# churchill-lab/gbrs

Hardware: AMD Instinct MI355X
Metric: EM iterations/s (EMASE Model 4, 40M reads x 8 haplotypes x 120k isoforms per GPU) (higher is better)
Workload: dtype f64

## Files before the change

### gbrs_amd/_lib.py

```python
from __future__ import annotations

import ctypes as C
import os

_HERE = os.path.dirname(os.path.abspath(__file__))
LIB_PATH = os.environ.get("GBRS_TUNING_LIB") or os.path.join(_HERE, "libgbrs_hip.so")

EXPORTS = [
    "gbrs_last_error", "gbrs_abi_version", "gbrs_device_count", "gbrs_warm_up",
    "gbrs_em_create", "gbrs_em_create_device", "gbrs_em_create_masked", "gbrs_em_create_masked_device", "gbrs_em_set_initial_values", "gbrs_em_prepare", "gbrs_em_step", "gbrs_em_run",
    "gbrs_em_set_groups", "gbrs_em_step_model", "gbrs_em_posterior",
    "gbrs_em_resample", "gbrs_em_weights", "gbrs_em_resample_info",
    "gbrs_em_bootstrap_begin", "gbrs_em_bootstrap_add", "gbrs_em_bootstrap_get",
    "gbrs_em_get", "gbrs_em_set_theta", "gbrs_em_group_sums", "gbrs_em_estep_partial",
    "gbrs_em_finish_step", "gbrs_em_prepare_partial", "gbrs_em_finish_prepare", "gbrs_em_stream",
    "gbrs_em_set_stream",
    "gbrs_em_sync", "gbrs_em_pair_begin", "gbrs_em_pair_check", "gbrs_em_pair_status", "gbrs_em_info", "gbrs_em_fold_counts", "gbrs_em_tile_cut", "gbrs_em_tile_shapes",
    "gbrs_alignment_counts",
    "gbrs_counts_create", "gbrs_counts_get", "gbrs_counts_destroy", "gbrs_em_destroy",
    "gbrs_shard_plan", "gbrs_shard_index", "gbrs_shard_gather",
    "gbrs_hmm_create", "gbrs_hmm_set_expression", "gbrs_hmm_set_eprob", "gbrs_hmm_run",
    "gbrs_hmm_get", "gbrs_hmm_info", "gbrs_hmm_destroy",
    "gbrs_grid_knots", "gbrs_hmm_set_grid", "gbrs_hmm_grid", "gbrs_hmm_grid_info", "gbrs_hmm_sample_paths", "gbrs_hmm_sample_info",
    "gbrs_hmm_diagnostics", "gbrs_hmm_pair_posterior", "gbrs_hmm_diagnostics_info",
    "gbrs_hmm_set_panel", "gbrs_hmm_match", "gbrs_hmm_match_info",
    "gbrs_hmm_set_snps", "gbrs_hmm_impute", "gbrs_hmm_impute_info", "gbrs_hmm_impute_times",
    "gbrs_hmm_loglik", "gbrs_hmm_loglik_tables", "gbrs_hmm_loglik_info", "gbrs_interpolate", "gbrs_genoprob_dosage",
    "gbrs_ri_transition_tables", "gbrs_alignment_spec",
    "gbrs_scan_create", "gbrs_scan_destroy", "gbrs_scan_append", "gbrs_scan_append_hmm", "gbrs_scan_prepare", "gbrs_scan_run",
    "gbrs_scan_info", "gbrs_scan_permute", "gbrs_scan_perm_info",
    "gbrs_scan_set_snps", "gbrs_scan_snp_dosage", "gbrs_scan_snps", "gbrs_scan_snp_info",
    "gbrs_compress_create", "gbrs_compress_get", "gbrs_compress_destroy",
    "gbrs_bam_open", "gbrs_bam_references", "gbrs_bam_set_reference_map", "gbrs_bam_convert", "gbrs_bam_get",
    "gbrs_bam_scan_records", "gbrs_bam_destroy",
    "gbrs_ecset_create", "gbrs_ecset_add_bam", "gbrs_ecset_add_bam_pair", "gbrs_ecset_sizes", "gbrs_ecset_get", "gbrs_ecset_destroy",
    "gbrs_matops_create", "gbrs_matops_intersect", "gbrs_matops_append_rows", "gbrs_matops_keep_unique_rows",
    "gbrs_matops_mask_columns", "gbrs_matops_sizes", "gbrs_matops_get", "gbrs_matops_destroy",
    "gbrs_matops_shared_counts", "gbrs_matops_shared_counts_get", "gbrs_matops_shared_counts_info",
    "gbrs_tensor_create", "gbrs_tensor_set_groups", "gbrs_tensor_reset", "gbrs_tensor_multiply",
    "gbrs_tensor_multiply_tensor", "gbrs_tensor_normalize", "gbrs_tensor_sum_reads", "gbrs_tensor_sum_loci",
    "gbrs_tensor_copy", "gbrs_tensor_values", "gbrs_tensor_set_values", "gbrs_tensor_nnz", "gbrs_tensor_destroy",
    "gbrs_format_double", "gbrs_write_locus_table", "gbrs_parse_length_table", "gbrs_parse_genotype_table",
    "gbrs_decode_chunks", "gbrs_inflate_backend", "gbrs_zip_directory", "gbrs_npz_stack", "gbrs_zip_read_members", "gbrs_parse_number_table",
]

GBRS_OK = 0
GBRS_ERR_INVALID = -1
GBRS_ERR_HIP = -2
GBRS_ERR_NO_DEVICE = -3
GBRS_ERR_FLOAT = -4
GBRS_ERR_UNSUPPORTED = -5
GBRS_ERR_STATE = -6

GBRS_EM_DEFAULT = 0
GBRS_EM_MERGE_IDENTICAL_ROWS = 1
GBRS_EM_LAYOUT_CSC = 2
GBRS_EM_NO_INTERLEAVE = 4
GBRS_EM_FORCE_INTERLEAVE = 8
GBRS_EM_NO_STREAMS = 16
GBRS_EM_DETERMINISTIC = 32
GBRS_EM_KEEP_CSC = 64
GBRS_EM_SIDE_BY_SIDE = 128
GBRS_EM_ONE_SHOT = 256
GBRS_EM_NO_LOCUS_SETS = 512
GBRS_EM_GROUPED_MODELS = 1024
GBRS_EM_POSTERIOR = 2048
GBRS_EM_RESAMPLE = 4096
GBRS_EM_NO_RUN_WORDS = 8192
GBRS_RESAMPLE_BASE = 0xFFFFFFFF


class EmInfo(C.Structure):
    _fields_ = [
        ("num_rows", C.c_uint64), ("num_entries", C.c_uint64), ("num_device_rows", C.c_uint64),
        ("num_device_words", C.c_uint64), ("bytes_per_iter", C.c_uint64),
        ("algorithmic_bytes", C.c_uint64), ("last_estep_ms", C.c_double),
        ("last_step_ms", C.c_double), ("num_loci", C.c_uint32), ("num_haps", C.c_uint32),
        ("layout", C.c_uint32), ("num_folded_rows", C.c_uint32),
        ("num_tiles", C.c_uint64), ("num_slots", C.c_uint64), ("num_long_rows", C.c_uint64),
        ("num_heavy_loci", C.c_uint64), ("num_light_loci", C.c_uint64), ("estep_bytes", C.c_uint64),
        ("retained_build_bytes", C.c_uint64),
        ("num_locus_sets", C.c_uint64),
    ]


class HmmInfo(C.Structure):
    _fields_ = [
        ("total_genes", C.c_uint64), ("algorithmic_bytes", C.c_uint64),
        ("last_emission_ms", C.c_double), ("last_forward_ms", C.c_double),
        ("last_backward_ms", C.c_double), ("last_backtrace_ms", C.c_double),
        ("num_states", C.c_int32), ("n_samples", C.c_int32),
        ("last_run_ms", C.c_double),
        ("last_delta_blocks", C.c_int32), ("last_delta_longest_fixup", C.c_int32),
        ("last_delta_fallbacks", C.c_int32), ("last_delta_tie_fallbacks", C.c_int32),
    ]


class ScanInfo(C.Structure):
    _fields_ = [
        ("n", C.c_int64), ("M", C.c_int64), ("H", C.c_int32), ("c", C.c_int32),
        ("last_prepare_ms", C.c_double), ("last_run_ms", C.c_double), ("last_product_ms", C.c_double),
        ("device_bytes", C.c_uint64),
    ]


class ScanPermInfo(C.Structure):
    _fields_ = [
        ("P", C.c_int64), ("B", C.c_int64), ("last_permute_ms", C.c_double), ("last_product_ms", C.c_double),
        ("peak_device_bytes", C.c_uint64),
    ]


class ScanSnpInfo(C.Structure):
    _fields_ = [
        ("M_snp", C.c_int64), ("chunk", C.c_int64), ("P", C.c_int64), ("last_pass_ms", C.c_double),
        ("last_row_ms", C.c_double), ("last_product_ms", C.c_double), ("device_bytes", C.c_uint64),
        ("peak_device_bytes", C.c_uint64), ("staged", C.c_int32), ("reserved", C.c_int32),
    ]


class GbrsHipError(RuntimeError):
    def __init__(self, status, message):
        super().__init__(message)
        self.status = status


_lib = None


def load():
    global _lib
    if _lib is not None:
        return _lib
    if not os.path.exists(LIB_PATH):
        raise ImportError(
            f"{LIB_PATH} is missing: the HIP library has not been built "
            "(run `python -c 'import __graft_entry__ as g; g.build()'`). "
            "gbrs_amd has no CPU fallback.")
    lib = C.CDLL(LIB_PATH)
    vp, i32, u32, u64, i64, dbl = C.c_void_p, C.c_int, C.c_uint32, C.c_uint64, C.c_int64, C.c_double
    pp = C.POINTER(C.c_void_p)
    lib.gbrs_last_error.restype = C.c_char_p
    lib.gbrs_last_error.argtypes = []
    lib.gbrs_abi_version.restype = i32
    lib.gbrs_device_count.restype = i32
    lib.gbrs_warm_up.restype = i32
    lib.gbrs_warm_up.argtypes = [i32]
    sigs = {
        "gbrs_em_create": [u64, u32, u32, pp, pp, vp, vp, i32, u32, pp],
        "gbrs_em_create_device": [u64, u32, u32, pp, pp, vp, vp, i32, u32, pp],
        "gbrs_em_create_masked": [u64, u32, u32, pp, pp, vp, vp, vp, i32, u32, pp],
        "gbrs_em_create_masked_device": [u64, u32, u32, pp, pp, vp, vp, vp, i32, u32, pp],
        "gbrs_em_set_initial_values": [vp, pp],
        "gbrs_em_prepare": [vp, dbl],
        "gbrs_em_step": [vp, i32, C.POINTER(dbl)],
        "gbrs_em_run": [vp, i32, dbl, i32, C.POINTER(i32), vp, i32, vp],
        "gbrs_em_set_groups": [vp, i64, vp, vp],
        "gbrs_em_step_model": [vp, i32, i32, C.POINTER(dbl)],
        "gbrs_em_posterior": [vp, u32, vp, u64],
        "gbrs_em_resample": [vp, u64, u32],
        "gbrs_em_weights": [vp, vp],
        "gbrs_em_resample_info": [vp, C.POINTER(u64), C.POINTER(u64), C.POINTER(u32)],
        "gbrs_em_bootstrap_begin": [vp, i64, vp, vp],
        "gbrs_em_bootstrap_add": [vp, vp, vp, vp, vp],
        "gbrs_em_bootstrap_get": [vp, i32, C.POINTER(u32), vp, vp, vp, vp, vp, vp, vp, vp],
        "gbrs_em_get": [vp, vp, vp],
        "gbrs_em_set_theta": [vp, vp],
        "gbrs_em_group_sums": [vp, i64, vp, vp, i32, vp],
        "gbrs_em_estep_partial": [vp, pp, C.POINTER(u64)],
        "gbrs_em_finish_step": [vp, C.POINTER(dbl)],
        "gbrs_em_prepare_partial": [vp, pp, C.POINTER(u64)],
        "gbrs_em_finish_prepare": [vp, dbl],
        "gbrs_em_sync": [vp],
        "gbrs_em_pair_begin": [vp, vp, i32],
        "gbrs_em_pair_check": [vp, vp, dbl],
        "gbrs_em_pair_status": [vp, vp, C.POINTER(i32), C.POINTER(i32), vp, i32],
        "gbrs_em_set_stream": [vp, vp],
        "gbrs_em_info": [vp, C.POINTER(EmInfo)],
        "gbrs_em_fold_counts": [vp, C.POINTER(u64), C.POINTER(u64)],
        "gbrs_em_tile_cut": [vp, C.POINTER(u32), C.POINTER(u32)],
        "gbrs_em_tile_shapes": [vp, vp, vp, u64],
        "gbrs_alignment_counts": [u64, u32, u32, pp, pp, vp, vp, u32, i32, vp, vp, vp],
        "gbrs_counts_create": [u64, u32, u32, pp, pp, vp, i32, pp],
        "gbrs_counts_get": [vp, vp, u32, vp, vp, vp],
        "gbrs_counts_destroy": [vp],
        "gbrs_em_destroy": [vp],
        "gbrs_shard_plan": [u64, u32, u32, pp, pp, i32, i32, vp],
        "gbrs_shard_index": [u64, u32, u32, pp, pp, u64, u64, i32, pp, vp],
        "gbrs_shard_gather": [u64, u32, u32, pp, pp, u64, u64, u32, pp, i32, vp, pp, pp, C.POINTER(u64)],
        "gbrs_hmm_create": [i32, i32, vp, vp, pp, i32, pp],
        "gbrs_hmm_set_expression": [vp, i32, pp, pp, pp, dbl, dbl],
        "gbrs_hmm_set_eprob": [vp, i32, pp],
        "gbrs_hmm_run": [vp],
        "gbrs_hmm_get": [vp, i32, i32, vp, vp, vp, vp, vp, vp, vp, vp],
        "gbrs_hmm_info": [vp, C.POINTER(HmmInfo)],
        "gbrs_hmm_destroy": [vp],
        "gbrs_grid_knots": [i32, vp, i32, vp, vp, vp],
        "gbrs_hmm_set_grid": [vp, vp, pp, vp, pp],
        "gbrs_hmm_grid": [vp, i32, vp, vp],
        "gbrs_hmm_grid_info": [vp, C.POINTER(i64), C.POINTER(dbl)],
        "gbrs_hmm_set_panel": [vp, i32, pp],
        "gbrs_hmm_match": [vp, i32, vp, vp],
        "gbrs_hmm_match_info": [vp, C.POINTER(i32), vp, C.POINTER(dbl), C.POINTER(u64)],
        "gbrs_hmm_set_snps": [vp, vp, pp, vp, pp, pp],
        "gbrs_hmm_impute": [vp, i32, i64, i64, vp],
        "gbrs_hmm_impute_info": [vp, C.POINTER(i64), C.POINTER(dbl), C.POINTER(u64)],
        "gbrs_hmm_impute_times": [vp, C.POINTER(dbl), C.POINTER(dbl), C.POINTER(dbl)],
        "gbrs_hmm_sample_paths": [vp, i32, i32, u64, vp, vp, vp, C.POINTER(u64)],
        "gbrs_hmm_sample_info": [vp, C.POINTER(dbl), C.POINTER(u64)],
        "gbrs_hmm_diagnostics": [vp, i32, vp, vp, vp, vp, vp],
        "gbrs_hmm_pair_posterior": [vp, i32, i32, vp],
        "gbrs_hmm_diagnostics_info": [vp, C.POINTER(dbl)],
        "gbrs_hmm_loglik": [vp, i32, vp],
        "gbrs_hmm_loglik_tables": [vp, i32, i32, vp, pp, i32, vp],
        "gbrs_hmm_loglik_info": [vp, C.POINTER(dbl), C.POINTER(u64)],
        "gbrs_interpolate": [i32, i32, vp, vp, i32, vp, vp, i32],
        "gbrs_genoprob_dosage": [i32, i64, vp, vp, i32],
        "gbrs_ri_transition_tables": [vp, vp, vp, i64, dbl, dbl, i32, vp],
        "gbrs_alignment_spec": [vp, vp, vp, i64, i32, dbl, i32, vp, vp, vp, vp],
        "gbrs_scan_create": [i32, i32, vp, i32, pp],
        "gbrs_scan_destroy": [vp],
        "gbrs_scan_append": [vp, i32, vp],
        "gbrs_scan_append_hmm": [vp, vp, i32],
        "gbrs_scan_prepare": [vp, i32, vp],
        "gbrs_scan_run": [vp, i64, vp, vp, vp, vp],
        "gbrs_scan_info": [vp, C.POINTER(ScanInfo), vp],
        "gbrs_scan_permute": [vp, i64, vp, i64, u64, vp, vp, vp],
        "gbrs_scan_perm_info": [vp, C.POINTER(ScanPermInfo)],
        "gbrs_scan_set_snps": [vp, pp, vp, pp, pp],
        "gbrs_scan_snp_dosage": [vp, i64, i64, vp],
        "gbrs_scan_snps": [vp, i64, vp, vp, vp, vp, vp],
        "gbrs_scan_snp_info": [vp, C.POINTER(ScanSnpInfo)],
        "gbrs_compress_create": [u64, u32, u32, pp, pp, vp, i32, pp, C.POINTER(u64), vp],
        "gbrs_compress_get": [vp, pp, pp, vp],
        "gbrs_compress_destroy": [vp],
        "gbrs_bam_convert": [vp, i32, C.POINTER(u64), C.POINTER(u32), vp, vp],
        "gbrs_bam_get": [vp, pp, pp, vp],
        "gbrs_ecset_create": [u32, u32, i32, C.POINTER(vp)],
        "gbrs_ecset_add_bam": [vp, vp, C.POINTER(u64), vp],
        "gbrs_ecset_add_bam_pair": [vp, vp, vp, C.POINTER(u64), vp],
        "gbrs_ecset_sizes": [vp, C.POINTER(u64), C.POINTER(u64), vp],
        "gbrs_ecset_get": [vp, pp, pp, vp],
        "gbrs_ecset_destroy": [vp],
        "gbrs_matops_create": [u64, u32, u32, pp, pp, i32, pp],
        "gbrs_matops_intersect": [vp, pp, pp],
        "gbrs_matops_append_rows": [vp, u64, pp, pp],
        "gbrs_matops_keep_unique_rows": [vp, vp, u32, i32, vp],
        "gbrs_matops_mask_columns": [vp, vp],
        "gbrs_matops_sizes": [vp, C.POINTER(u64), vp, C.POINTER(u32)],
        "gbrs_matops_get": [vp, pp, pp],
        "gbrs_matops_destroy": [vp],
        "gbrs_matops_shared_counts": [vp, vp, u32, C.POINTER(u64)],
        "gbrs_matops_shared_counts_get": [vp, vp, vp, vp],
        "gbrs_matops_shared_counts_info": [vp, C.POINTER(u64), C.POINTER(u64), C.POINTER(u64), C.POINTER(u32),
                                           C.POINTER(u64), C.POINTER(u64), C.POINTER(dbl)],
        "gbrs_tensor_create": [u64, u32, u32, pp, pp, pp, vp, i32, pp],
        "gbrs_tensor_set_groups": [vp, i64, vp, vp],
        "gbrs_tensor_reset": [vp],
        "gbrs_tensor_multiply": [vp, i32, vp, u64],
        "gbrs_tensor_multiply_tensor": [vp, vp],
        "gbrs_tensor_normalize": [vp, i32],
        "gbrs_tensor_sum_reads": [vp, vp],
        "gbrs_tensor_sum_loci": [vp, vp],
        "gbrs_tensor_copy": [vp, pp],
        "gbrs_tensor_values": [vp, u32, vp, vp, u64],
        "gbrs_tensor_set_values": [vp, u32, vp, u64],
        "gbrs_tensor_nnz": [vp, vp],
        "gbrs_tensor_destroy": [vp],
    }
    sigs.update(_host_signatures())
    for name, args in sigs.items():
        if name in ("gbrs_em_fold_counts", "gbrs_em_tile_cut", "gbrs_em_tile_shapes") and os.environ.get("GBRS_TUNING_LIB") and not hasattr(lib, name):
            continue
        fn = getattr(lib, name)
        fn.restype = i32
        fn.argtypes = args
    lib.gbrs_em_stream.restype = vp
    lib.gbrs_em_stream.argtypes = [vp]
    if lib.gbrs_abi_version() != 5:
        raise ImportError("libgbrs_hip.so ABI version mismatch")
    _lib = lib
    return lib


def _host_signatures():
    vp, i32, u32, u64, i64, dbl = C.c_void_p, C.c_int, C.c_uint32, C.c_uint64, C.c_int64, C.c_double
    return {
        "gbrs_format_double": [dbl, C.c_char_p],
        "gbrs_decode_chunks": [C.c_char_p, i64, vp, vp, vp, vp, u64, u32, u64, i32, i32, vp, i32],
        "gbrs_inflate_backend": [],
        "gbrs_zip_directory": [vp, u64, u64, vp, vp, vp, vp, vp, vp, u64, C.POINTER(u64), C.POINTER(u64)],
        "gbrs_npz_stack": [vp, u64, i64, vp, vp, vp, vp, vp, vp, u64, u64, vp, vp, i32],
        "gbrs_zip_read_members": [vp, u64, i64, vp, vp, vp, vp, vp, vp, i32],
        "gbrs_parse_number_table": [C.c_char_p, i64, i64, i32, vp],
        "gbrs_parse_length_table": [C.c_char_p, i64, C.c_char_p, vp, i64, C.c_char_p, vp, i32, dbl, vp],
        "gbrs_parse_genotype_table": [C.c_char_p, i64, C.c_char_p, vp, i64, C.c_char_p, vp, i32, vp, vp, i32, vp,
                                      C.POINTER(i64)],
        "gbrs_bam_open": [C.c_char_p, i32, C.POINTER(vp), C.POINTER(u64), C.POINTER(u64)],
        "gbrs_bam_references": [vp, vp, u64, vp, vp],
        "gbrs_bam_set_reference_map": [vp, u64, vp, vp, u32, u32],
        "gbrs_bam_scan_records": [vp, u64, vp, vp, vp, vp, u64, C.POINTER(u64), C.POINTER(u64)],
        "gbrs_bam_destroy": [vp],
        "gbrs_write_locus_table": [C.c_char_p, C.c_char_p, vp, i64, i32, i64, i64, vp, C.c_char_p, vp, C.c_char_p, vp, vp],
    }


def check(status):
    if status == GBRS_OK:
        return
    msg = load().gbrs_last_error().decode(errors="replace")
    if status == GBRS_ERR_FLOAT:
        raise FloatingPointError(msg)
    raise GbrsHipError(status, msg)


def ptr(a):
    if a is None:
        return None
    return a.ctypes.data_as(C.c_void_p)


def ptr_table(arrays):
    tab = (C.c_void_p * len(arrays))()
    for i, a in enumerate(arrays):
        tab[i] = None if a is None else a.ctypes.data
    return tab


def raw_table(addresses):
    tab = (C.c_void_p * len(addresses))()
    for i, a in enumerate(addresses):
        tab[i] = a
    return tab


def warm_up_device_async(device=0):
    import threading

    def _go():
        try:
            load().gbrs_warm_up(int(device))
        except Exception:
            pass
    t = threading.Thread(target=_go, name='gbrs-hip-init', daemon=True)
    t.start()
    return t
```

### gbrs_amd/csrc/em.hip

```cpp
#include "common.h"
#include "em_layout.h"
#include "em_step.h"

#include <algorithm>
#include <chrono>
#include <cmath>
#include <cstdlib>

namespace gbrs {


struct EmScalars {
    double s_prev, s_new;
    double err_sum;
    double pc_before, pc_after;
    int stop;
    int iters_done;
    int float_error;
    int ticket;
};

constexpr int RED_BLOCKS = 256;
constexpr int RED_THREADS = 256;

// ... 382 lines not shown
    else v = t * (fac[k] / (count ? count[r] : 1.0));
    out[k - k0] = v;
}

#include "em_tiles.inc"
#include "em_models.inc"
#include "em_resample.inc"

}

using namespace gbrs;


struct gbrs_em {
    int device = 0;
    hipStream_t stream = nullptr;
    bool own_stream = true;
    uint64_t R = 0, N = 0;
    uint32_t L = 0, H = 0;
    bool has_count = false, has_len = false, prepared = false;
    uint32_t flags = 0;

    int layout = 0;
    EmPlan plan;
    bool acc_external = false;
    TileLayout tl;

    DevBuf<uint32_t> ent_row;
    DevBuf<uint64_t> col_ptr;
    DevBuf<uint64_t> col_ptr_src;
    bool masked = false;
    DevBuf<double> den;

    DevBuf<double> count, eff_len;
    DevBuf<double> acc_init;
    bool has_init = false, keep_csc = false;
    bool stopped = false;
    DevBuf<double> theta, acc, counts;
    bool counts_stale = false;
    DevBuf<double> tot_prev, tot_new;
    DevBuf<double> partials;
    DevBuf<double> msums;
    uint32_t msum_cap = 0, msum_blocks = 0;
    DevBuf<double> scratch_hl;
    DevBuf<double> err_hist;
    DevBuf<EmScalars> scalars;
    int err_hist_cap = 0;
    double last_estep_ms = 0.0, last_step_ms = 0.0;
    bool time_steps = true;
    bool err_pending = false;
    double err_pending_target = -1.0;
    std::vector<hipEvent_t> ev_pool;

    struct PairScalars { int iters, stop; double err; };
    DevBuf<PairScalars> pair_sc;
    DevBuf<double> pair_hist;
    int pair_hist_cap = 0;
    hipEvent_t pair_ev_mstep = nullptr;
    hipEvent_t pair_ev_err = nullptr;

    bool grouped = false;
    uint32_t n_genes = 0;
    DevBuf<uint32_t> gene_ptr, gene_mem, locus_gene, row_ptr;
    DevBuf<uint32_t> rank_m1, inv_m1, rank_m23, inv_m23;
    GroupedOrder order_m1, order_m23;
    DevBuf<double> gene_tot, gene_hap_tot, locus_tot, fac;

    DevBuf<double> theta_kept, post_den, post_vals;
    int post_model = 0;
    bool post_den_valid = false;

    bool resample = false, has_base = false;
    DevBuf<uint32_t> base_count, big_rows;
    uint32_t n_big = 0;
    struct Stats {
        bool active = false;
        uint32_t n = 0;
        int64_t G = 0;
        DevBuf<int64_t> gptr, gmem;
        DevBuf<double> theta_sum;
        DevBuf<double> cur[2][2], mean[2][2], m2[2][2], tot_mean[2][2], tot_m2[2][2];
    } stats;

    int red_blocks() const { return (int)std::min<uint64_t>(RED_BLOCKS, (L + RED_THREADS - 1) / RED_THREADS); }
};

struct gbrs_counts {
    int device = 0;
    uint64_t R = 0, n = 0;
    uint32_t L = 0, H = 0;
    gbrs::DevBuf<uint32_t> ent_row;
    gbrs::DevBuf<uint64_t> col_ptr;
    gbrs::DevBuf<double> d_count;
    hipStream_t s = nullptr;
    gbrs::CountsWork *work = nullptr;
};

namespace {

ErrArgs em_err_args(gbrs_em *em, double target_err) {
    ErrArgs ea;
    ea.L = em->L;
    ea.nblocks = (int)em->msum_blocks;
    ea.cap = em->msum_cap;
    ea.tot_prev = em->tot_prev.p;
    ea.tot_new = em->tot_new.p;
    ea.partials = em->msums.p;
    ea.sc = em->scalars.p;
    ea.target_err = target_err;
    ea.err_hist = em->err_hist.p;
    ea.err_hist_cap = em->err_hist_cap;
    ea.n_err_blocks = (uint32_t)std::min<uint64_t>(ERR_BLOCKS, (em->L + RED_THREADS - 1) / RED_THREADS);
    return ea;
}

int em_launch_err(gbrs_em *em, double target_err) {
    const ErrArgs ea = em_err_args(em, target_err);
    hipLaunchKernelGGL(err_finish_kernel, dim3(ea.n_err_blocks), dim3(RED_THREADS), 0, em->stream, ea);
    GBRS_HIP_CHECK(hipGetLastError());
    return GBRS_OK;
}

int em_flush_err(gbrs_em *em) {
    if (!em->err_pending) return GBRS_OK;
    em->err_pending = false;
    return em_launch_err(em, em->err_pending_target);
}

int em_check_float(gbrs_em *em, EmScalars &host) {
    GBRS_TRY(em_flush_err(em));
    GBRS_HIP_CHECK(hipMemcpyAsync(&host, em->scalars.p, sizeof(EmScalars), hipMemcpyDeviceToHost, em->stream));
    GBRS_HIP_CHECK(hipStreamSynchronize(em->stream));
    em->stopped = host.stop != 0;
    if (host.float_error && !em->plan.no_float_check)
        return fail(GBRS_ERR_FLOAT, "invalid value encountered in divide (a read's alignments all have zero abundance)");
    return GBRS_OK;
}


EmStepRoute em_route(const gbrs_em *em, EmPass pass) {
    const TileLayout &tl = em->tl;
    EmStepShape s;
    s.tiled = em->layout == 1;
    s.H = em->H; s.tH = em->plan.tH; s.view = em->plan.view;
    s.no_tiles = tl.n_tiles == 0; s.no_long = tl.n_long == 0; s.no_entries = em->N == 0;
    s.weighted = tl.weighted; s.deterministic = tl.deterministic; s.all_one_word = tl.all_one_word;
    s.persist_groups = em->plan.persist_groups;
    s.acc_handed_out = em->acc_external;
    s.no_fused_mstep = em->plan.no_fused_mstep;
    return em_step_route(s, pass);
}

template <int HT, bool ONES>
int em_launch_tiles_h(gbrs_em *em, const EmStepRoute &r) {
    const TileLayout &tl = em->tl;
    const uint32_t tH = em->plan.tH;
    ErrArgs ea = em_err_args(em, em->err_pending_target);
    if (!r.err_rides || !em->err_pending) ea.n_err_blocks = 0;
    em->err_pending = false;
    const dim3 grid((unsigned)tl.n_tiles + ea.n_err_blocks), block(TILE_THREADS);
    const double *ww = tl.weighted ? tl.word_weight.p : (const double *)nullptr;
    const SetArgs sets{em->plan.tL, tl.n_sets ? tl.set_ptr.p : nullptr, tl.set_members.p, tl.dest_list.p, tl.dict_b.p, tl.dest_b.p,
                       em->resample ? 1u : 0u};
    const uint32_t lead_mask = em->plan.lead_mask;
#define GBRS_LAUNCH_TILES(W, D)                                                                                            \
    hipLaunchKernelGGL((tile_estep_kernel<HT, W, ONES, D>), grid, block, 0, em->stream, tH, tl.tiles.p, tl.words.p,        \
                       tl.dict.p, ww, em->theta.p, tl.partials.p, tl.slot_dest.p, em->acc.p, em->scalars.p,               \
                       (uint32_t)tl.n_tiles, ea, sets, lead_mask)
    switch (r.estep) {
        case EmEstep::Persistent:
        case EmEstep::PersistentOneWord: {
            const uint32_t G = std::min<uint32_t>(em->plan.persist_groups, (uint32_t)tl.n_tiles);
            const dim3 pgrid(G + ea.n_err_blocks);
#define GBRS_LAUNCH_PERSISTENT(HH, W, OW)                                                                                  \
            hipLaunchKernelGGL((tile_estep_persistent_kernel<HH, W, OW>), pgrid, block, 0, em->stream, tH, tl.tiles.p,     \
                               tl.words.p, tl.dict.p, ww, em->theta.p, tl.partials.p, tl.slot_dest.p,                      \
                               (int64_t)(em->acc.p - tl.partials.p), em->scalars.p, (uint32_t)tl.n_tiles, G, ea, sets)
            if (r.estep == EmEstep::PersistentOneWord) GBRS_LAUNCH_PERSISTENT(HT == 8 ? 8 : 1, false, HT == 8);
            else if (r.weighted) GBRS_LAUNCH_PERSISTENT(HT, true, false);
            else GBRS_LAUNCH_PERSISTENT(HT, false, false);
#undef GBRS_LAUNCH_PERSISTENT
            break;
        }
        case EmEstep::TilesDeterministic:
            if (r.weighted) GBRS_LAUNCH_TILES(true, true); else GBRS_LAUNCH_TILES(false, true);
            break;
#if !defined(GBRS_NO_ONEWORD)
        case EmEstep::TilesOneWord:
            hipLaunchKernelGGL((tile_estep_kernel<HT == 8 ? 8 : 1, false, ONES, false, HT == 8>), grid, block, 0, em->stream, tH,
                               tl.tiles.p, tl.words.p, tl.dict.p, ww, em->theta.p, tl.partials.p, tl.slot_dest.p, em->acc.p,
                               em->scalars.p, (uint32_t)tl.n_tiles, ea, sets, lead_mask);
            break;
#endif
        default:
            if (r.weighted) GBRS_LAUNCH_TILES(true, false); else GBRS_LAUNCH_TILES(false, false);
    }
#undef GBRS_LAUNCH_TILES
    return GBRS_OK;
}
int em_launch_tiles(gbrs_em *em, const EmStepRoute &r) {
#define GBRS_TILES_OF(HT) (r.pass == EmPass::Prepare ? em_launch_tiles_h<HT, true>(em, r) : em_launch_tiles_h<HT, false>(em, r))
    switch (r.width) {
        case 1: return GBRS_TILES_OF(1);
        case 2: return GBRS_TILES_OF(2);
        case 4: return GBRS_TILES_OF(4);
        case 8: return GBRS_TILES_OF(8);
        case 16: return GBRS_TILES_OF(16);
        default: return GBRS_TILES_OF(0);
    }
#undef GBRS_TILES_OF
}

int em_launch_long_rows(gbrs_em *em, const EmStepRoute &r) {
    const TileLayout &tl = em->tl;
    const bool ones = r.pass == EmPass::Prepare;
    GBRS_HIP_CHECK(hipMemsetAsync(tl.acc_extra.p, 0, tl.acc_extra.bytes(), em->stream));
#define GBRS_LAUNCH_LONG(KERNEL, GRID, BLOCK)                                                                              \
    hipLaunchKernelGGL(KERNEL, GRID, BLOCK, 0, em->stream, tl.n_long, em->plan.tH, tl.long_ptr.p, tl.long_loc.p,          \
                       tl.long_mask.p, tl.long_weight.p, em->theta.p, tl.acc_extra.p, em->scalars.p, em->resample ? 1u : 0u)
    const dim3 grid((unsigned)((tl.n_long + 3) / 4));
    if (r.long_rows == EmLongRows::Serial) {
        if (ones) GBRS_LAUNCH_LONG(long_rows_estep_serial_kernel<true>, dim3(1), dim3(64));
        else GBRS_LAUNCH_LONG(long_rows_estep_serial_kernel<false>, dim3(1), dim3(64));
    } else {
        if (ones) GBRS_LAUNCH_LONG(long_rows_estep_kernel<true>, grid, dim3(256));
        else GBRS_LAUNCH_LONG(long_rows_estep_kernel<false>, grid, dim3(256));
    }
#undef GBRS_LAUNCH_LONG
    return GBRS_OK;
}

int em_launch_gather(gbrs_em *em, const EmStepRoute &r) {
    const TileLayout &tl = em->tl;
    const uint32_t gH = em->plan.tH, gL = em->plan.tL;
    uint32_t HP = 1;
    while (HP < gH) HP <<= 1;
    const bool all = r.gather == EmGather::All;
    const uint64_t elems = all ? (uint64_t)gL * gH : (uint64_t)tl.n_light * gH;
    const unsigned light = (unsigned)((elems + 255) / 256);
    const unsigned heavy = (unsigned)((tl.n_heavy + 3) / 4);
    if (light + heavy > 0)
        hipLaunchKernelGGL(gather_kernel, dim3(light + heavy), dim3(256), 0, em->stream, gL, gH,
                           HP, light, heavy, (uint32_t)tl.n_heavy, all ? 1 : 0, (uint32_t)tl.n_light, tl.light_loci.p,
                           tl.slot_ptr.p, tl.heavy_loci.p, tl.locus_class.p, tl.partials.p,
                           (tl.n_long && all) ? tl.acc_extra.p : (const double *)nullptr, em->acc.p, em->scalars.p,
                           r.pass == EmPass::Prepare ? 0 : 1);
    return GBRS_OK;
}

template <bool ONES>
int em_launch_csc(gbrs_em *em, const EmStepRoute &r) {
    const uint64_t n = em->N;
    const uint32_t ncols = em->H * em->L;
    GBRS_HIP_CHECK(hipMemsetAsync(em->acc.p, 0, em->acc.bytes(), em->stream));
    if (r.estep != EmEstep::Csc) return GBRS_OK;
    GBRS_HIP_CHECK(hipMemsetAsync(em->den.p, 0, em->den.bytes(), em->stream));
    const unsigned grid = (unsigned)((n + 255) / 256);
    hipLaunchKernelGGL(csc_den_kernel<ONES>, dim3(grid), dim3(256), 0, em->stream, n, ncols, em->L,
                       em->H, em->col_ptr.p, em->ent_row.p, em->theta.p, em->den.p, em->scalars.p);
    hipLaunchKernelGGL(csc_acc_kernel<ONES>, dim3(grid), dim3(256), 0, em->stream, n, ncols, em->L,
                       em->H, em->col_ptr.p, em->ent_row.p, em->has_count ? em->count.p : nullptr,
                       em->den.p, em->acc.p, em->scalars.p, em->resample ? 1u : 0u);
    return GBRS_OK;
}

int em_launch_models(gbrs_em *em, int model) {
    const GroupedOrder &o = model == 1 ? em->order_m1 : em->order_m23;
    const uint32_t nt = std::max(em->L, em->n_genes);
    hipLaunchKernelGGL(model_totals_kernel, dim3((nt + 255) / 256), dim3(256), 0, em->stream, em->L, em->H, em->n_genes,
                       em->gene_ptr.p, em->gene_mem.p, em->theta.p, em->gene_tot.p, em->gene_hap_tot.p, em->locus_tot.p,
                       em->scalars.p);
    GBRS_HIP_CHECK(hipMemsetAsync(em->acc.p, 0, em->acc.bytes(), em->stream));
    if (em->N) {
        const dim3 rgrid((unsigned)((em->R + 255) / 256));
        const double *cnt = em->has_count ? em->count.p : (const double *)nullptr;
#define GBRS_LAUNCH_ROWS(M)                                                                                             \
        hipLaunchKernelGGL(model_row_kernel<M>, rgrid, dim3(256), 0, em->stream, em->R, em->H, em->row_ptr.p, o.lh.p,   \
                           o.src.p, em->locus_gene.p, em->theta.p, em->gene_tot.p, em->gene_hap_tot.p, em->locus_tot.p, \
                           cnt, em->fac.p, em->scalars.p)
        if (model == 1) GBRS_LAUNCH_ROWS(1);
        else if (model == 2) GBRS_LAUNCH_ROWS(2);
        else GBRS_LAUNCH_ROWS(3);
#undef GBRS_LAUNCH_ROWS
        hipLaunchKernelGGL(model_col_kernel, dim3((unsigned)((em->N + 255) / 256)), dim3(256), 0, em->stream, em->N,
                           em->H * em->L, em->L, em->H, em->col_ptr.p, em->fac.p, em->acc.p, em->scalars.p);
    }
    GBRS_HIP_CHECK(hipGetLastError());
    return GBRS_OK;
}

int em_estep(gbrs_em *em, const EmStepRoute &r, int model = 4, hipEvent_t after_kernels = nullptr) {
    if (!r.err_rides) GBRS_TRY(em_flush_err(em));
    if (r.estep == EmEstep::Models) GBRS_TRY(em_launch_models(em, model));
    else if (em->layout != 1) GBRS_TRY(r.pass == EmPass::Prepare ? em_launch_csc<true>(em, r) : em_launch_csc<false>(em, r));
    else if (r.estep != EmEstep::None) GBRS_TRY(em_launch_tiles(em, r));
    if (r.long_rows != EmLongRows::None) GBRS_TRY(em_launch_long_rows(em, r));
    if (after_kernels) GBRS_HIP_CHECK(hipEventRecord(after_kernels, em->stream));
    if (r.gather != EmGather::None) GBRS_TRY(em_launch_gather(em, r));
    GBRS_HIP_CHECK(hipGetLastError());
    return GBRS_OK;
}

template <int H, bool EXTRA, bool LEN>
void em_launch_mstep_gather_h(gbrs_em *em) {
    const TileLayout &tl = em->tl;
    const uint64_t npair = (uint64_t)em->L * MstepRow<H>::LANES, per = (uint64_t)RED_THREADS * MSTEP_EPT;
    const unsigned elem_blocks = (unsigned)((npair + per - 1) / per);
    const unsigned heavy_blocks = (unsigned)tl.n_heavy;
    const unsigned light_blocks = (unsigned)((tl.n_light * MstepRow<H>::LANES + RED_THREADS - 1) / RED_THREADS);
    em->msum_blocks = elem_blocks + heavy_blocks + light_blocks;
    hipLaunchKernelGGL((mstep_gather_kernel<H, EXTRA, LEN>), dim3(em->msum_blocks), dim3(RED_THREADS), 0, em->stream, em->L,
                       heavy_blocks, light_blocks, (uint32_t)tl.n_light, tl.heavy_range.p, tl.light_range.p,
                       tl.locus_class.p, tl.partials.p, em->acc.p, EXTRA ? tl.acc_extra.p : (const double *)nullptr,
                       em->theta.p, LEN ? em->eff_len.p : (const double *)nullptr, em->tot_prev.p, em->tot_new.p,
                       em->msums.p, em->msum_cap, em->scalars.p);
}
template <int H>
void em_launch_mstep_gather_opts(gbrs_em *em, bool extra) {
    if (extra) em->has_len ? em_launch_mstep_gather_h<H, true, true>(em) : em_launch_mstep_gather_h<H, true, false>(em);
    else em->has_len ? em_launch_mstep_gather_h<H, false, true>(em) : em_launch_mstep_gather_h<H, false, false>(em);
}
int em_launch_mstep_gather(gbrs_em *em, const EmStepRoute &r) {
    const bool extra = r.long_rows != EmLongRows::None;
    switch (em->H) {
    case 1: em_launch_mstep_gather_opts<1>(em, extra); break;
    case 2: em_launch_mstep_gather_opts<2>(em, extra); break;
    case 4: em_launch_mstep_gather_opts<4>(em, extra); break;
    case 8: em_launch_mstep_gather_opts<8>(em, extra); break;
    case 16: em_launch_mstep_gather_opts<16>(em, extra); break;
    default: return fail(GBRS_ERR_UNSUPPORTED, "the fused M-step has no instance for this haplotype count");
    }
    return GBRS_OK;
}

template <int MODE, int H>
void em_launch_mstep_elem(gbrs_em *em, const double *extra, const double *len) {
    const uint64_t npair = (uint64_t)em->L * MstepRow<H>::LANES;
    const unsigned nb = (unsigned)((npair + RED_THREADS - 1) / RED_THREADS);
    em->msum_blocks = nb;
    hipLaunchKernelGGL((mstep_elem_kernel<MODE, H>), dim3(nb), dim3(RED_THREADS), 0, em->stream, em->L, em->theta.p, em->acc.p,
                       extra, len, em->counts.p, em->tot_prev.p, em->tot_new.p, em->msums.p, em->msum_cap, em->scalars.p);
}
template <int MODE>
int em_launch_mstep_plain(gbrs_em *em, const EmStepRoute &r) {
    const double *len = em->has_len ? em->eff_len.p : nullptr;
    if (r.mstep == EmMstep::PerLocus) {
        const int nb = em->red_blocks();
        em->msum_blocks = nb;
        hipLaunchKernelGGL(mstep_kernel<MODE>, dim3(nb), dim3(RED_THREADS), 0, em->stream, em->L, em->H,
                           em->theta.p, em->acc.p, len, em->counts.p, em->tot_prev.p, em->tot_new.p,
                           em->msums.p, em->msum_cap, em->scalars.p);
        return GBRS_OK;
    }
    const double *extra = r.mstep_adds_extra ? em->tl.acc_extra.p : (const double *)nullptr;
    switch (em->H) {
    case 1: em_launch_mstep_elem<MODE, 1>(em, extra, len); break;
    case 2: em_launch_mstep_elem<MODE, 2>(em, extra, len); break;
    case 4: em_launch_mstep_elem<MODE, 4>(em, extra, len); break;
    case 8: em_launch_mstep_elem<MODE, 8>(em, extra, len); break;
    case 16: em_launch_mstep_elem<MODE, 16>(em, extra, len); break;
    case 32: em_launch_mstep_elem<MODE, 32>(em, extra, len); break;
    default: return fail(GBRS_ERR_UNSUPPORTED, "the element-parallel M-step has no instance for this haplotype count");
    }
    return GBRS_OK;
}
int em_launch_mstep(gbrs_em *em, const EmStepRoute &r) {
    if (r.mstep == EmMstep::Fused) return em_launch_mstep_gather(em, r);
    return r.pass == EmPass::Prepare ? em_launch_mstep_plain<1>(em, r) : em_launch_mstep_plain<0>(em, r);
}

__global__ void __launch_bounds__(256)
counts_from_theta_kernel(uint64_t n, const double *__restrict__ theta, const double *__restrict__ eff_len, double *__restrict__ counts) {
    const uint64_t i = (uint64_t)blockIdx.x * blockDim.x + threadIdx.x;
    if (i < n) counts[i] = eff_len ? theta[i] * eff_len[i] : theta[i];
}
int em_refresh_counts(gbrs_em *em) {
    if (!em->counts_stale) return GBRS_OK;
    const uint64_t n = (uint64_t)em->L * em->H;
    hipLaunchKernelGGL(counts_from_theta_kernel, dim3((unsigned)((n + 255) / 256)), dim3(256), 0, em->stream, n, em->theta.p,
                       em->has_len ? em->eff_len.p : (const double *)nullptr, em->counts.p);
    GBRS_HIP_CHECK(hipGetLastError());
    em->counts_stale = false;
    return GBRS_OK;
}

int em_finish_step(gbrs_em *em, const EmStepRoute &r, double target_err, bool defer_err) {
    GBRS_TRY(em_flush_err(em));
    GBRS_TRY(em_launch_mstep(em, r));
    em->counts_stale = r.counts_stale;
    if (defer_err && r.err_defer) {
        em->err_pending = true;
        em->err_pending_target = target_err;
        return GBRS_OK;
    }
    return em_launch_err(em, target_err);
}

int em_keep_theta(gbrs_em *em, int model) {
    if (!(em->flags & GBRS_EM_POSTERIOR)) return GBRS_OK;
    GBRS_TRY(em_flush_err(em));
    const uint64_t n = (uint64_t)em->L * em->H;
    hipLaunchKernelGGL(keep_theta_kernel, dim3((unsigned)((n + 255) / 256)), dim3(256), 0, em->stream, n, em->theta.p,
                       em->theta_kept.p, em->scalars.p);
    GBRS_HIP_CHECK(hipGetLastError());
    em->post_model = model;
    em->post_den_valid = false;
    return GBRS_OK;
}

constexpr int EM_TIME_STRIDE = 8, EM_TIME_SAMPLES = 16;
int em_one_step(gbrs_em *em, const EmStepRoute &r, int model, double target_err, hipEvent_t *ev, bool defer_err) {
    GBRS_TRY(em_keep_theta(em, model));
    if (!em->time_steps) ev = nullptr;
    if (ev) GBRS_HIP_CHECK(hipEventRecord(ev[0], em->stream));
    GBRS_TRY(em_estep(em, r, model, ev ? ev[1] : nullptr));
    GBRS_TRY(em_finish_step(em, r, target_err, defer_err));
    if (r.pass == EmPass::Model && em->layout == 1) GBRS_HIP_CHECK(hipMemsetAsync(em->acc.p, 0, em->acc.bytes(), em->stream));
    if (ev) GBRS_HIP_CHECK(hipEventRecord(ev[2], em->stream));
    return GBRS_OK;
}

void em_read_times(gbrs_em *em, int n) {
    if (!em->time_steps || n <= 0) return;
    double se = 0.0, ss = 0.0;
    for (int i = 0; i < n; ++i) {
        float a = 0.f, b = 0.f;
        if (hipEventElapsedTime(&a, em->ev_pool[3 * i], em->ev_pool[3 * i + 1]) != hipSuccess) return;
        if (hipEventElapsedTime(&b, em->ev_pool[3 * i], em->ev_pool[3 * i + 2]) != hipSuccess) return;
        se += a;
        ss += b;
    }
    em->last_estep_ms = se / n;
    em->last_step_ms = ss / n;
}

int em_finish_prepare(gbrs_em *em, double pseudocount) {
    GBRS_TRY(em_launch_mstep(em, em_route(em, EmPass::Prepare)));
    em->counts_stale = false;
    const int nb = em->red_blocks();
    if (pseudocount > 0.0) {
        hipLaunchKernelGGL(pseudo_add_kernel, dim3(nb), dim3(RED_THREADS), 0, em->stream, em->L,
                           em->H, pseudocount, em->theta.p, em->partials.p);
        hipLaunchKernelGGL(pseudo_scale_kernel, dim3(nb), dim3(RED_THREADS), 0, em->stream,
                           (uint64_t)em->L * em->H, nb, em->theta.p, em->partials.p, em->scalars.p);
    }
    GBRS_HIP_CHECK(hipMemsetAsync(em->partials.p, 0, em->partials.bytes(), em->stream));
    GBRS_HIP_CHECK(hipMemsetAsync(em->acc.p, 0, em->acc.bytes(), em->stream));
    GBRS_HIP_CHECK(hipGetLastError());
    em->prepared = true;
    return GBRS_OK;
}

int em_reset_scalars(gbrs_em *em, bool keep_iters) {
    GBRS_TRY(em_flush_err(em));
    EmScalars host;
    std::memset(&host, 0, sizeof(host));
    if (keep_iters) {
        EmScalars cur;
        GBRS_HIP_CHECK(hipMemcpyAsync(&cur, em->scalars.p, sizeof(cur), hipMemcpyDeviceToHost, em->stream));
        GBRS_HIP_CHECK(hipStreamSynchronize(em->stream));
        host.iters_done = cur.iters_done;
    }
    em->stopped = false;
    GBRS_HIP_CHECK(hipMemcpyAsync(em->scalars.p, &host, sizeof(host), hipMemcpyHostToDevice, em->stream));
    GBRS_HIP_CHECK(hipStreamSynchronize(em->stream));
    return GBRS_OK;
}

int em_ensure_hist(gbrs_em *em, int cap) {
    if (cap <= em->err_hist_cap) return GBRS_OK;
    GBRS_HIP_CHECK(hipStreamSynchronize(em->stream));
    GBRS_TRY(em->err_hist.alloc((size_t)cap));
    em->err_hist_cap = cap;
    return GBRS_OK;
}

int em_check_model(const gbrs_em *em, int model) {
    if (model < 1 || model > 4) return fail(GBRS_ERR_INVALID, "The read normalization model should be 1, 2, 3, or 4.");
    if (model == 4) return GBRS_OK;
    if (em->flags & GBRS_EM_DETERMINISTIC)
        return fail(GBRS_ERR_UNSUPPORTED, "multiread model %d has no bit-reproducible form (GBRS_EM_DETERMINISTIC)", model);
    if (!em->grouped)
        return fail(GBRS_ERR_UNSUPPORTED, "multiread model %d needs gene groups: create the handle with "
                                          "GBRS_EM_GROUPED_MODELS and call gbrs_em_set_groups", model);
    return GBRS_OK;
}

int em_ensure_order(gbrs_em *em, int model) {
    GroupedOrder &o = model == 1 ? em->order_m1 : em->order_m23;
    if (o.built) return GBRS_OK;
    GBRS_TRY(em_flush_err(em));
    return build_grouped_order(o, em->R, em->L, em->H, em->N, em->ent_row.p, em->col_ptr.p,
                               model == 1 ? em->rank_m1.p : em->rank_m23.p, model == 1 ? em->inv_m1.p : em->inv_m23.p,
                               em->stream);
}

int upload_csc(uint64_t R, uint32_t L, uint32_t H, const uint32_t *const *indptr,
               const uint32_t *const *indices, bool on_device, DevBuf<uint32_t> &ent_row,
               DevBuf<uint64_t> &col_ptr_dev, uint64_t &n_out, const uint32_t *allowed = nullptr,
               DevBuf<uint64_t> *src_ptr_dev = nullptr, hipStream_t stream = nullptr) {
    const hipMemcpyKind kind = on_device ? hipMemcpyDeviceToDevice : hipMemcpyHostToDevice;
    std::vector<uint64_t> col_ptr((size_t)H * L + 1), src_ptr;
    if (allowed) src_ptr.resize((size_t)H * L + 1);
    std::vector<uint32_t> tmp(L + 1);
    uint64_t n = 0, n_src = 0;
    std::vector<uint64_t> hap_off(H + 1);
    for (uint32_t h = 0; h < H; ++h) {
        if (!indptr[h]) return fail(GBRS_ERR_INVALID, "indptr[%u] is NULL", h);
        if (on_device) {
            GBRS_HIP_CHECK(hipMemcpy(tmp.data(), indptr[h], (L + 1) * sizeof(uint32_t), hipMemcpyDeviceToHost));
        } else {
            std::memcpy(tmp.data(), indptr[h], (L + 1) * sizeof(uint32_t));
        }
        if (tmp[0] != 0) return fail(GBRS_ERR_INVALID, "indptr[%u][0] != 0", h);
        hap_off[h] = n_src;
        for (uint32_t l = 0; l < L; ++l) {
            if (tmp[l + 1] < tmp[l]) return fail(GBRS_ERR_INVALID, "indptr[%u] is not non-decreasing at %u", h, l);
            col_ptr[(size_t)h * L + l] = n;
            if (allowed) {
                src_ptr[(size_t)h * L + l] = n_src + tmp[l];
                if ((allowed[l] >> h) & 1u) n += tmp[l + 1] - tmp[l];
            } else {
                n += tmp[l + 1] - tmp[l];
            }
        }
        n_src += tmp[L];
    }
    hap_off[H] = n_src;
    col_ptr[(size_t)H * L] = n;
    GBRS_TRY(col_ptr_dev.alloc(col_ptr.size()));
    GBRS_HIP_CHECK(hipMemcpy(col_ptr_dev.p, col_ptr.data(), col_ptr_dev.bytes(), hipMemcpyHostToDevice));
    GBRS_TRY(ent_row.alloc(std::max<uint64_t>(n, 1)));
// ... 333 lines not shown
        int hbad = 0;
        GBRS_HIP_CHECK(hipMemcpyAsync(&hbad, bad.p, sizeof(int), hipMemcpyDeviceToHost, em->stream));
        GBRS_HIP_CHECK(hipStreamSynchronize(em->stream));
        GBRS_HIP_CHECK(hipGetLastError());
        if (hbad) {
            em->acc_init.release();
            return fail(GBRS_ERR_FLOAT, "invalid value encountered in divide (a read's stored alignment values are "
                                        "negative or add up to zero)");
        }
    }
    em->has_init = true;
    if (em->layout == 1 && em->keep_csc) {
        if (!(em->flags & (GBRS_EM_GROUPED_MODELS | GBRS_EM_POSTERIOR))) em->ent_row.release();
        em->den.release();
        em->col_ptr_src.release();
        em->keep_csc = false;
    }
    return GBRS_OK;
}

int gbrs_em_prepare_partial(gbrs_em_t *em, void **partial_dev, uint64_t *n_elems) {
    if (!em) return fail(GBRS_ERR_INVALID, "handle is NULL");
    em->acc_external = true;
    GBRS_TRY(em_prepare_partial(em));
    if (partial_dev) *partial_dev = em->acc.p;
    if (n_elems) *n_elems = (uint64_t)em->L * em->H;
    return GBRS_OK;
}

int gbrs_em_finish_prepare(gbrs_em_t *em, double pseudocount) {
    if (!em) return fail(GBRS_ERR_INVALID, "handle is NULL");
    GBRS_TRY(select_device(em->device));
    GBRS_TRY(em_finish_prepare(em, pseudocount));
    EmScalars host;
    return em_check_float(em, host);
}

int gbrs_em_prepare(gbrs_em_t *em, double pseudocount) {
    RoctxRange roctx_range("gbrs_em_prepare");
    if (!em) return fail(GBRS_ERR_INVALID, "handle is NULL");
    GBRS_TRY(em_prepare_partial(em));
    return gbrs_em_finish_prepare(em, pseudocount);
}

int gbrs_em_estep_partial(gbrs_em_t *em, void **partial_dev, uint64_t *n_elems) {
    if (!em) return fail(GBRS_ERR_INVALID, "handle is NULL");
    if (!em->prepared) return fail(GBRS_ERR_STATE, "prepare() has not been called");
    GBRS_TRY(select_device(em->device));
    if (em->stopped) GBRS_TRY(em_reset_scalars(em, true));
    em->acc_external = true;
    GBRS_TRY(em_estep(em, em_route(em, EmPass::Partial)));
    if (partial_dev) *partial_dev = em->acc.p;
    if (n_elems) *n_elems = (uint64_t)em->L * em->H;
    return GBRS_OK;
}

int gbrs_em_finish_step(gbrs_em_t *em, double *err_sum_out) {
    if (!em) return fail(GBRS_ERR_INVALID, "handle is NULL");
    GBRS_TRY(select_device(em->device));
    GBRS_TRY(em_finish_step(em, em_route(em, EmPass::Partial), -1.0,  err_sum_out == nullptr));
    if (em->pair_ev_mstep) GBRS_HIP_CHECK(hipEventRecord(em->pair_ev_mstep, em->stream));
    if (err_sum_out) {
        EmScalars host;
        GBRS_TRY(em_check_float(em, host));
        *err_sum_out = host.err_sum;
    }
    return GBRS_OK;
}

int gbrs_em_step(gbrs_em_t *em, int n_iters, double *err_sum_out) {
    RoctxRange roctx_range("gbrs_em_step");
    if (!em) return fail(GBRS_ERR_INVALID, "handle is NULL");
    if (!em->prepared) return fail(GBRS_ERR_STATE, "prepare() has not been called");
    GBRS_TRY(select_device(em->device));
    if (em->stopped) GBRS_TRY(em_reset_scalars(em, true));
    const int stride = std::max(EM_TIME_STRIDE, (n_iters + EM_TIME_SAMPLES - 1) / EM_TIME_SAMPLES);
    const int timed = em->time_steps ? (n_iters + stride - 1) / stride : 0;
    while ((int)em->ev_pool.size() < 3 * timed) {
        hipEvent_t e;
        GBRS_HIP_CHECK(hipEventCreate(&e));
        em->ev_pool.push_back(e);
    }
    const EmStepRoute route = em_route(em, EmPass::Step);
    for (int i = 0; i < n_iters; ++i) {
        const int slot = i / stride;
        const bool t = i % stride == 0 && slot < timed;
        GBRS_TRY(em_one_step(em, route, 4, -1.0, t ? &em->ev_pool[3 * slot] : nullptr, i + 1 < n_iters));
    }
    EmScalars host;
    GBRS_TRY(em_check_float(em, host));
    em_read_times(em, timed);
    if (err_sum_out) *err_sum_out = host.err_sum;
    return GBRS_OK;
}

int gbrs_em_step_model(gbrs_em_t *em, int model, int n_iters, double *err_sum_out) {
    RoctxRange roctx_range("gbrs_em_step_model");
    if (!em) return fail(GBRS_ERR_INVALID, "handle is NULL");
    GBRS_TRY(em_check_model(em, model));
    if (model == 4) return gbrs_em_step(em, n_iters, err_sum_out);
    if (!em->prepared) return fail(GBRS_ERR_STATE, "prepare() has not been called");
    GBRS_TRY(select_device(em->device));
    if (em->stopped) GBRS_TRY(em_reset_scalars(em, true));
    GBRS_TRY(em_ensure_order(em, model));
    const EmStepRoute route = em_route(em, EmPass::Model);
    for (int i = 0; i < n_iters; ++i) GBRS_TRY(em_one_step(em, route, model, -1.0, i == 0 ? em->ev_pool.data() : nullptr, false));
    EmScalars host;
    GBRS_TRY(em_check_float(em, host));
    em_read_times(em, n_iters > 0 ? 1 : 0);
    if (err_sum_out) *err_sum_out = host.err_sum;
    return GBRS_OK;
}

int gbrs_em_set_groups(gbrs_em_t *em, int64_t G, const int64_t *group_ptr, const int64_t *members) {
    RoctxRange roctx_range("gbrs_em_set_groups");
    if (!em || G < 0 || (G > 0 && (!group_ptr || !members))) return fail(GBRS_ERR_INVALID, "bad argument");
    if (!(em->flags & GBRS_EM_GROUPED_MODELS))
        return fail(GBRS_ERR_STATE, "the handle was not created with GBRS_EM_GROUPED_MODELS");
    if (em->N && !em->ent_row.p) return fail(GBRS_ERR_STATE, "the handle no longer holds the CSC row ids");
    const uint32_t L = em->L, H = em->H;
    if (em->N >= 0xFFFFFFFFull || L >= (1u << 27))
        return fail(GBRS_ERR_UNSUPPORTED, "the grouped layout holds at most 2^32 - 1 entries of at most 2^27 loci");
    if (G > 0 && group_ptr[0] != 0) return fail(GBRS_ERR_INVALID, "group_ptr[0] != 0");
    for (int64_t g = 0; g < G; ++g)
        if (group_ptr[g + 1] < group_ptr[g]) return fail(GBRS_ERR_INVALID, "group_ptr not monotone");
    GBRS_TRY(select_device(em->device));
    std::vector<int64_t> gene(L, -1);
    std::vector<std::vector<uint32_t>> mem((size_t)G);
    for (int64_t g = 0; g < G; ++g)
        for (int64_t k = group_ptr[g]; k < group_ptr[g + 1]; ++k) {
            const int64_t l = members[k];
            if (l < 0 || l >= (int64_t)L) return fail(GBRS_ERR_INVALID, "group member %lld out of range", (long long)l);
            if (gene[l] == g) continue;
            if (gene[l] >= 0)
                return fail(GBRS_ERR_INVALID, "locus %lld is in two groups (%lld and %lld)", (long long)l,
                            (long long)gene[l], (long long)g);
            gene[l] = g;
            mem[g].push_back((uint32_t)l);
        }
    std::vector<uint32_t> gptr{0}, gmem, lgene(L), pos(L);
    gmem.reserve(L);
    for (int64_t g = 0; g < G; ++g) {
        std::sort(mem[g].begin(), mem[g].end());
        for (uint32_t l : mem[g]) { lgene[l] = (uint32_t)(gptr.size() - 1); pos[l] = (uint32_t)gmem.size(); gmem.push_back(l); }
        gptr.push_back((uint32_t)gmem.size());
    }
    for (uint32_t l = 0; l < L; ++l)
        if (gene[l] < 0) { lgene[l] = (uint32_t)(gptr.size() - 1); pos[l] = (uint32_t)gmem.size(); gmem.push_back(l); gptr.push_back((uint32_t)gmem.size()); }
    const uint32_t n_genes = (uint32_t)(gptr.size() - 1);
    const size_t HL = (size_t)H * L;
    std::vector<uint32_t> r23(HL), i23(HL), r1(HL), i1(HL);
    for (uint32_t l = 0; l < L; ++l) {
        const uint32_t g = lgene[l], start = gptr[g], size = gptr[g + 1] - start;
        for (uint32_t h = 0; h < H; ++h) {
            const uint32_t a = pos[l] * H + h, b = start * H + h * size + (pos[l] - start);
            r23[(size_t)h * L + l] = a;
            i23[a] = l * 32u + h;
            r1[(size_t)h * L + l] = b;
            i1[b] = l * 32u + h;
        }
    }
    em->grouped = false;
    em->order_m1.built = em->order_m23.built = false;
    auto up = [&](DevBuf<uint32_t> &d, const std::vector<uint32_t> &v) -> int {
        GBRS_TRY(d.alloc(std::max<size_t>(v.size(), 1)));
        if (!v.empty()) GBRS_HIP_CHECK(hipMemcpyAsync(d.p, v.data(), v.size() * 4, hipMemcpyHostToDevice, em->stream));
        return GBRS_OK;
    };
    GBRS_TRY(up(em->gene_ptr, gptr));
    GBRS_TRY(up(em->gene_mem, gmem));
    GBRS_TRY(up(em->locus_gene, lgene));
    GBRS_TRY(up(em->rank_m23, r23));
    GBRS_TRY(up(em->inv_m23, i23));
    GBRS_TRY(up(em->rank_m1, r1));
    GBRS_TRY(up(em->inv_m1, i1));
    GBRS_TRY(em->gene_tot.alloc(n_genes));
    GBRS_TRY(em->gene_hap_tot.alloc((size_t)n_genes * H));
    GBRS_TRY(em->locus_tot.alloc(L));
    GBRS_TRY(em->fac.alloc(std::max<uint64_t>(em->N, 1)));
    GBRS_HIP_CHECK(hipStreamSynchronize(em->stream));
    em->n_genes = n_genes;
    GBRS_TRY(build_row_ptr(em->row_ptr, em->R, em->N, em->ent_row.p, em->stream));
    GBRS_TRY(build_grouped_order(em->order_m23, em->R, L, H, em->N, em->ent_row.p, em->col_ptr.p, em->rank_m23.p,
                                 em->inv_m23.p, em->stream));
    em->grouped = true;
    return GBRS_OK;
}

int gbrs_em_run(gbrs_em_t *em, int model, double tol, int max_iters, int *n_iters_out,
                double *err_hist, int err_hist_cap, double *elapsed_s) {
    RoctxRange roctx_range("gbrs_em_run");
    if (!em) return fail(GBRS_ERR_INVALID, "handle is NULL");
    GBRS_TRY(em_check_model(em, model));
    if (!em->prepared) return fail(GBRS_ERR_STATE, "prepare() has not been called");
    GBRS_TRY(select_device(em->device));
    if (model != 4) GBRS_TRY(em_ensure_order(em, model));
    if (max_iters < 0) max_iters = 0;
    GBRS_TRY(em_ensure_hist(em, std::max(max_iters, 1)));
    GBRS_TRY(em_reset_scalars(em, false));
    const double target = 1000000.0 * tol;
    const EmStepRoute route = em_route(em, model == 4 ? EmPass::Step : EmPass::Model);
    int done = 0;
    EmScalars host;
    std::memset(&host, 0, sizeof(host));
    if (1000000.0 > target) {
        const int batch = 8;
        bool first = true;
        const auto t_start = std::chrono::steady_clock::now();
        while (done < max_iters) {
            const int nb = std::min(batch, max_iters - done);
            for (int i = 0; i < nb; ++i) {
                GBRS_TRY(em_one_step(em, route, model, target, first ? em->ev_pool.data() : nullptr, i + 1 < nb));
                first = false;
            }
            GBRS_TRY(em_check_float(em, host));
            if (elapsed_s) {
                const double t = std::chrono::duration<double>(std::chrono::steady_clock::now() - t_start).count();
                for (int i = done; i < host.iters_done && i < err_hist_cap; ++i) elapsed_s[i] = t;
            }
            done = host.iters_done;
            if (host.stop) break;
        }
    }
    em_read_times(em, 1);
    if (n_iters_out) *n_iters_out = done;
    if (err_hist && err_hist_cap > 0 && done > 0) {
        const int ncopy = std::min(done, err_hist_cap);
        GBRS_HIP_CHECK(hipMemcpy(err_hist, em->err_hist.p, ncopy * sizeof(double), hipMemcpyDeviceToHost));
    }
    return GBRS_OK;
}

int gbrs_em_get(gbrs_em_t *em, double *theta, double *expected_counts) {
    if (!em) return fail(GBRS_ERR_INVALID, "handle is NULL");
    GBRS_TRY(select_device(em->device));
    const size_t LH = (size_t)em->L * em->H;
    for (int which = 0; which < 2; ++which) {
        double *dst = which == 0 ? theta : expected_counts;
        if (!dst) continue;
        if (which == 1) GBRS_TRY(em_refresh_counts(em));
        hipLaunchKernelGGL(transpose_lh_to_hl, dim3(1024), dim3(256), 0, em->stream, em->L, em->H,
                           which == 0 ? em->theta.p : em->counts.p, em->scratch_hl.p);
        GBRS_HIP_CHECK(hipMemcpyAsync(dst, em->scratch_hl.p, LH * sizeof(double), hipMemcpyDeviceToHost, em->stream));
        GBRS_HIP_CHECK(hipStreamSynchronize(em->stream));
    }
    return GBRS_OK;
}

int gbrs_em_posterior(gbrs_em_t *em, uint32_t hap, double *out, uint64_t out_len) {
    RoctxRange roctx_range("gbrs_em_posterior");
    if (!em) return fail(GBRS_ERR_INVALID, "handle is NULL");
    if (!(em->flags & GBRS_EM_POSTERIOR))
        return fail(GBRS_ERR_STATE, "the handle was not created with GBRS_EM_POSTERIOR");
    if (em->post_model == 0) return fail(GBRS_ERR_STATE, "no EM step has run since prepare: there is no posterior yet");
    if (hap >= em->H) return fail(GBRS_ERR_INVALID, "haplotype %u >= num_haps %u", hap, em->H);
    GBRS_TRY(select_device(em->device));
    GBRS_TRY(em_flush_err(em));
    const uint32_t L = em->L, H = em->H, ncols = H * L;
    uint64_t k0 = 0, k1 = 0;
    GBRS_HIP_CHECK(hipMemcpyAsync(&k0, em->col_ptr.p + (size_t)hap * L, sizeof(k0), hipMemcpyDeviceToHost, em->stream));
    GBRS_HIP_CHECK(hipMemcpyAsync(&k1, em->col_ptr.p + (size_t)(hap + 1) * L, sizeof(k1), hipMemcpyDeviceToHost, em->stream));
    GBRS_HIP_CHECK(hipStreamSynchronize(em->stream));
    if (k1 < k0 || k1 > em->N) return fail(GBRS_ERR_STATE, "the kept column pointers are damaged");
    const uint64_t n_h = k1 - k0;
    if (out_len != n_h)
        return fail(GBRS_ERR_INVALID, "out_len is %llu, haplotype %u has %llu stored entries", (unsigned long long)out_len,
                    hap, (unsigned long long)n_h);
    if (n_h == 0) return GBRS_OK;
    if (!out) return fail(GBRS_ERR_INVALID, "out is NULL");
    if (!em->ent_row.p) return fail(GBRS_ERR_STATE, "the handle no longer holds the CSC row ids");
    const bool model4 = em->post_model == 4;
    if (!model4 && !em->fac.p) return fail(GBRS_ERR_STATE, "the handle holds no factors of a model %d step", em->post_model);
    if (model4 && !em->post_den_valid) {
        GBRS_HIP_CHECK(hipMemsetAsync(em->post_den.p, 0, em->post_den.bytes(), em->stream));
        hipLaunchKernelGGL(post_den_kernel, dim3((unsigned)((em->N + 255) / 256)), dim3(256), 0, em->stream, em->N, ncols,
                           L, H, em->col_ptr.p, em->ent_row.p, em->theta_kept.p, em->post_den.p);
        GBRS_HIP_CHECK(hipGetLastError());
        em->post_den_valid = true;
    }
    if (em->post_vals.n < n_h) {
        std::vector<uint64_t> cp((size_t)ncols + 1);
        GBRS_HIP_CHECK(hipMemcpy(cp.data(), em->col_ptr.p, cp.size() * 8, hipMemcpyDeviceToHost));
        uint64_t longest = 0;
        for (uint32_t h = 0; h < H; ++h) longest = std::max(longest, cp[(size_t)(h + 1) * L] - cp[(size_t)h * L]);
        GBRS_HIP_CHECK(hipStreamSynchronize(em->stream));
        GBRS_TRY(em->post_vals.alloc(longest));
    }
    const dim3 grid((unsigned)((n_h + 255) / 256));
    const double *cnt = em->has_count ? em->count.p : (const double *)nullptr;
    if (model4)
        hipLaunchKernelGGL(post_value_kernel<true>, grid, dim3(256), 0, em->stream, k0, k1, ncols, L, H, hap, em->col_ptr.p,
                           em->ent_row.p, em->theta_kept.p, em->post_den.p, (const double *)nullptr, cnt, em->post_vals.p);
    else
        hipLaunchKernelGGL(post_value_kernel<false>, grid, dim3(256), 0, em->stream, k0, k1, ncols, L, H, hap, em->col_ptr.p,
                           em->ent_row.p, em->theta_kept.p, (const double *)nullptr, em->fac.p, cnt, em->post_vals.p);
    GBRS_HIP_CHECK(hipGetLastError());
    GBRS_HIP_CHECK(hipMemcpyAsync(out, em->post_vals.p, n_h * sizeof(double), hipMemcpyDeviceToHost, em->stream));
    GBRS_HIP_CHECK(hipStreamSynchronize(em->stream));
    return GBRS_OK;
}

int gbrs_em_set_theta(gbrs_em_t *em, const double *theta) {
    if (!em || !theta) return fail(GBRS_ERR_INVALID, "NULL argument");
    GBRS_TRY(select_device(em->device));
    const size_t LH = (size_t)em->L * em->H;
    GBRS_TRY(em_refresh_counts(em));
    GBRS_HIP_CHECK(hipMemcpyAsync(em->scratch_hl.p, theta, LH * sizeof(double), hipMemcpyHostToDevice, em->stream));
    hipLaunchKernelGGL(transpose_hl_to_lh, dim3(1024), dim3(256), 0, em->stream, em->L, em->H,
                       em->scratch_hl.p, em->theta.p);
    GBRS_HIP_CHECK(hipStreamSynchronize(em->stream));
    em->prepared = true;
    return GBRS_OK;
}

int gbrs_em_group_sums(gbrs_em_t *em, int64_t G, const int64_t *group_ptr, const int64_t *members,
                       int which, double *out) {
    if (!em || !group_ptr || !out || G < 0) return fail(GBRS_ERR_INVALID, "bad argument");
    if (G == 0) return GBRS_OK;
    GBRS_TRY(select_device(em->device));
    const int64_t nm = group_ptr[G];
    for (int64_t g = 0; g < G; ++g)
        if (group_ptr[g + 1] < group_ptr[g]) return fail(GBRS_ERR_INVALID, "group_ptr not monotone");
    for (int64_t k = 0; k < nm; ++k)
        if (members[k] < 0 || members[k] >= (int64_t)em->L)
            return fail(GBRS_ERR_INVALID, "group member %lld out of range", (long long)members[k]);
    DevBuf<int64_t> d_ptr, d_mem;
    DevBuf<double> d_out;
    GBRS_TRY(d_ptr.alloc(G + 1));
    GBRS_TRY(d_mem.alloc(std::max<int64_t>(nm, 1)));
    GBRS_TRY(d_out.alloc((size_t)G * em->H));
    GBRS_HIP_CHECK(hipMemcpyAsync(d_ptr.p, group_ptr, (G + 1) * sizeof(int64_t), hipMemcpyHostToDevice, em->stream));
    if (nm) GBRS_HIP_CHECK(hipMemcpyAsync(d_mem.p, members, nm * sizeof(int64_t), hipMemcpyHostToDevice, em->stream));
    const int64_t total = G * (int64_t)em->H;
    if (which != 0) GBRS_TRY(em_refresh_counts(em));
    hipLaunchKernelGGL(group_sum_kernel, dim3((unsigned)((total + 255) / 256)), dim3(256), 0, em->stream,
                       em->H, G, d_ptr.p, d_mem.p, which == 0 ? em->theta.p : em->counts.p, d_out.p);
    GBRS_HIP_CHECK(hipMemcpyAsync(out, d_out.p, (size_t)G * em->H * sizeof(double), hipMemcpyDeviceToHost, em->stream));
    GBRS_HIP_CHECK(hipStreamSynchronize(em->stream));
    return GBRS_OK;
}

void *gbrs_em_stream(gbrs_em_t *em) { return em ? (void *)em->stream : nullptr; }

#if defined(GBRS_DIAG_TILE_TIMES)
int gbrs_debug_set_tile_stamps(void *device_ptr) {
    unsigned long long *p = static_cast<unsigned long long *>(device_ptr);
    GBRS_HIP_CHECK(hipMemcpyToSymbol(HIP_SYMBOL(g_tile_stamps), &p, sizeof(p)));
    return GBRS_OK;
}
#endif

int gbrs_em_set_stream(gbrs_em_t *em, void *stream) {
    if (!em) return fail(GBRS_ERR_INVALID, "handle is NULL");
    GBRS_TRY(select_device(em->device));
    GBRS_HIP_CHECK(hipStreamSynchronize(em->stream));
    if (em->own_stream && em->stream) (void)hipStreamDestroy(em->stream);
    em->stream = (hipStream_t)stream;
    em->own_stream = false;
    return GBRS_OK;
}

int gbrs_em_sync(gbrs_em_t *em) {
    if (!em) return fail(GBRS_ERR_INVALID, "handle is NULL");
    GBRS_TRY(em_flush_err(em));
    GBRS_HIP_CHECK(hipStreamSynchronize(em->stream));
    return GBRS_OK;
}

int gbrs_em_pair_begin(gbrs_em_t *a, gbrs_em_t *b, int max_iters) {
    if (!a || !b || a == b) return fail(GBRS_ERR_INVALID, "two distinct handles are needed");
    if (a->device != b->device) return fail(GBRS_ERR_INVALID, "the two handles of a pair live on one device");
    GBRS_TRY(select_device(a->device));
    for (gbrs_em *em : {a, b}) {
        GBRS_TRY(em_reset_scalars(em, false));
        if (!em->pair_ev_mstep) GBRS_HIP_CHECK(hipEventCreateWithFlags(&em->pair_ev_mstep, hipEventDisableTiming));
    }
    if (!a->pair_ev_err) GBRS_HIP_CHECK(hipEventCreateWithFlags(&a->pair_ev_err, hipEventDisableTiming));
    const int cap = std::max(max_iters, 1);
    if (!a->pair_sc.p) GBRS_TRY(a->pair_sc.alloc(1));
    if (cap > a->pair_hist_cap) {
        GBRS_TRY(a->pair_hist.alloc((size_t)cap));
        a->pair_hist_cap = cap;
    }
    GBRS_HIP_CHECK(hipMemset(a->pair_sc.p, 0, sizeof(gbrs_em::PairScalars)));
    return GBRS_OK;
}

int gbrs_em_pair_check(gbrs_em_t *a, gbrs_em_t *b, double tol) {
    if (!a || !b || !a->pair_sc.p || !a->pair_ev_err || !a->pair_ev_mstep || !b->pair_ev_mstep)
        return fail(GBRS_ERR_STATE, "gbrs_em_pair_begin has not been called on this pair");
    GBRS_TRY(select_device(a->device));
    GBRS_HIP_CHECK(hipStreamWaitEvent(b->stream, a->pair_ev_mstep, 0));
    static_assert(sizeof(PairState) == sizeof(gbrs_em::PairScalars), "one struct, two names");
    const PairSide sa{a->L, (int)a->msum_blocks, a->msum_cap, a->tot_prev.p, a->tot_new.p, a->msums.p, a->scalars.p};
    const PairSide sb{b->L, (int)b->msum_blocks, b->msum_cap, b->tot_prev.p, b->tot_new.p, b->msums.p, b->scalars.p};
    hipLaunchKernelGGL(pair_err_kernel, dim3(1), dim3(1024), 0, b->stream, sa, sb, 1000000.0 * tol,
                       reinterpret_cast<PairState *>(a->pair_sc.p), a->pair_hist.p, a->pair_hist_cap);
    GBRS_HIP_CHECK(hipGetLastError());
    GBRS_HIP_CHECK(hipEventRecord(a->pair_ev_err, b->stream));
    GBRS_HIP_CHECK(hipStreamWaitEvent(a->stream, a->pair_ev_err, 0));
    return GBRS_OK;
}

int gbrs_em_pair_status(gbrs_em_t *a, gbrs_em_t *b, int *iters_done, int *stopped, double *err_hist, int err_hist_cap) {
    if (!a || !b || !a->pair_sc.p) return fail(GBRS_ERR_STATE, "gbrs_em_pair_begin has not been called on this pair");
    GBRS_TRY(select_device(a->device));
    EmScalars ha, hb;
    GBRS_TRY(em_check_float(a, ha));
    GBRS_TRY(em_check_float(b, hb));
    gbrs_em::PairScalars ps;
    GBRS_HIP_CHECK(hipMemcpy(&ps, a->pair_sc.p, sizeof(ps), hipMemcpyDeviceToHost));
    if (iters_done) *iters_done = ps.iters;
    if (stopped) *stopped = ps.stop;
    if (err_hist && err_hist_cap > 0 && ps.iters > 0)
        GBRS_HIP_CHECK(hipMemcpy(err_hist, a->pair_hist.p, std::min(ps.iters, std::min(err_hist_cap, a->pair_hist_cap)) * sizeof(double),
                                 hipMemcpyDeviceToHost));
    return GBRS_OK;
}

int gbrs_em_info(gbrs_em_t *em, gbrs_em_info_t *info) {
    if (!em || !info) return fail(GBRS_ERR_INVALID, "NULL argument");
    std::memset(info, 0, sizeof(*info));
    const uint64_t HL = (uint64_t)em->H * em->L;
    info->num_rows = em->R;
    info->num_entries = em->N;
    info->num_device_rows = em->R;
    info->num_device_words = em->N;
    info->algorithmic_bytes = 4 * em->N + 4 * (em->R + 1) + (em->has_count ? 8 * em->R : 0) +
                              16 * HL + (em->has_len ? 8 * HL : 0);
    info->bytes_per_iter = 8 * em->N + 8 * em->R * 3 + 8 * HL * 4;
    info->estep_bytes = 8 * em->N + 8 * em->R * 3 + 8 * HL * 2;
    if (em->layout == 1) {
        const TileLayout &tl = em->tl;
        info->num_device_rows = tl.n_rows + tl.n_folded + tl.n_folded_two + tl.n_long;
        info->num_folded_rows = (uint32_t)tl.n_folded;
        info->num_tiles = tl.n_tiles;
        info->num_slots = tl.n_slots;
        info->num_long_rows = tl.n_long;
        info->num_device_words = tl.n_batches * 64;
        const uint64_t rows = tl.n_dest_rows ? tl.n_dest_rows : tl.n_slots;
        info->bytes_per_iter = 4 * tl.n_batches * 64 + 16 * tl.n_tiles + 4 * tl.n_slots +
                               8 * rows * em->plan.tH * 3 + 4 * rows + 4 * ((uint64_t)em->plan.tL + 1) +
                               (tl.weighted ? 8 * tl.n_batches * 64 : 0) + 8 * HL * 6;
        info->num_heavy_loci = tl.n_heavy;
        info->num_light_loci = tl.n_light;
        info->estep_bytes = 4 * tl.n_batches * 64 + 16 * tl.n_tiles + 4 * tl.n_slots + 4 * rows +
                            8 * rows * em->plan.tH * 2 + (tl.weighted ? 8 * tl.n_batches * 64 : 0) +
                            (tl.n_sets ? 8 * tl.n_slots : 0);
        if (tl.n_sets) info->bytes_per_iter += 8 * tl.n_slots;
    }
    info->last_estep_ms = em->last_estep_ms;
    info->last_step_ms = em->last_step_ms;
    info->num_loci = em->L;
    info->num_haps = em->H;
    info->layout = em->layout;
    info->retained_build_bytes = em->tl.retired_bytes;
    info->num_locus_sets = em->layout == 1 ? em->tl.n_sets : 0;
    return GBRS_OK;
}

int gbrs_em_fold_counts(gbrs_em_t *em, uint64_t *one_word_reads, uint64_t *two_word_reads) {
    if (!em || !one_word_reads || !two_word_reads) return fail(GBRS_ERR_INVALID, "NULL argument");
    *one_word_reads = em->layout == 1 ? em->tl.n_folded : 0;
    *two_word_reads = em->layout == 1 ? em->tl.n_folded_two : 0;
    return GBRS_OK;
}

int gbrs_em_tile_cut(gbrs_em_t *em, uint32_t *passes, uint32_t *tile_words) {
    if (!em || !passes || !tile_words) return fail(GBRS_ERR_INVALID, "NULL argument");
    *passes = em->layout == 1 ? em->tl.cut_passes : 0;
    *tile_words = em->layout == 1 ? em->tl.cut_tile_words : 0;
    return GBRS_OK;
}

int gbrs_em_tile_shapes(gbrs_em_t *em, uint32_t *n_batches, uint32_t *dict_entries, uint64_t n) {
    if (!em || !n_batches || !dict_entries) return fail(GBRS_ERR_INVALID, "NULL argument");
    if (em->layout != 1 || n != em->tl.n_tiles) return fail(GBRS_ERR_INVALID, "n is not the handle's number of tiles");
    (void)hipSetDevice(em->device);
    std::vector<TileHdr> hdr(n);
    if (n) GBRS_HIP_CHECK(hipMemcpy(hdr.data(), em->tl.tiles.p, n * sizeof(TileHdr), hipMemcpyDeviceToHost));
    for (uint64_t t = 0; t < n; ++t) {
        n_batches[t] = hdr[t].n_batches;
        dict_entries[t] = hdr[t].dict_count();
    }
    return GBRS_OK;
}

int gbrs_counts_create(uint64_t R, uint32_t L, uint32_t H, const uint32_t *const *indptr,
                       const uint32_t *const *indices, const double *count, int device, gbrs_counts_t **out) {
    if (!out) return fail(GBRS_ERR_INVALID, "out is NULL");
    *out = nullptr;
    if (H < 1 || H > 32 || L < 1 || R < 1 || R > 0xFFFFFFFFull || !indptr || !indices)
        return fail(GBRS_ERR_INVALID, "The shape must be a tuple of three positive integers (H <= 32, R < 2^32).");
    GBRS_TRY(select_device(device));
    gbrs_counts *c = new gbrs_counts();
    struct Guard { gbrs_counts *p; ~Guard() { if (p) gbrs_counts_destroy(p); } } guard{c};
    c->device = device;
    c->R = R; c->L = L; c->H = H;
    GBRS_HIP_CHECK(hipStreamCreateWithFlags(&c->s, hipStreamDefault));
    GBRS_TRY(upload_csc(R, L, H, indptr, indices, false, c->ent_row, c->col_ptr, c->n));
    if (count) {
        GBRS_TRY(c->d_count.alloc(R));
        GBRS_HIP_CHECK(hipMemcpy(c->d_count.p, count, R * sizeof(double), hipMemcpyHostToDevice));
    }
    GBRS_HIP_CHECK(hipDeviceSynchronize());
    GBRS_TRY(check_row_ids(c->n, c->ent_row.p, R, c->s));
    c->work = counts_work_new();
    guard.p = nullptr;
    *out = c;
    return GBRS_OK;
}

int gbrs_counts_get(gbrs_counts_t *c, const int32_t *locus_group, uint32_t num_out_loci, double *aln_counts,
                    double *allele_unique, double *locus_unique) {
    RoctxRange roctx_range("gbrs_counts_get");
    if (!c) return fail(GBRS_ERR_INVALID, "handle is NULL");
    const uint32_t L = c->L, H = c->H;
    const uint32_t Lout = locus_group ? num_out_loci : L;
    if (Lout < 1 || Lout >= (1u << 27)) return fail(GBRS_ERR_INVALID, "bad number of output loci");
    if (locus_group)
        for (uint32_t l = 0; l < L; ++l)
            if (locus_group[l] < -1 || (locus_group[l] >= 0 && (uint32_t)locus_group[l] >= Lout))
                return fail(GBRS_ERR_INVALID, "locus_group[%u] out of range", l);
    GBRS_TRY(select_device(c->device));
    DevBuf<double> d_aln, d_uniq, d_lu;
    DevBuf<int32_t> d_group;
    if (locus_group) {
        GBRS_TRY(d_group.alloc(L));
        GBRS_HIP_CHECK(hipMemcpy(d_group.p, locus_group, L * sizeof(int32_t), hipMemcpyHostToDevice));
    }
    GBRS_TRY(d_aln.alloc((size_t)H * Lout));
    GBRS_TRY(d_uniq.alloc((size_t)H * Lout));
    GBRS_TRY(d_lu.alloc(Lout));
    GBRS_TRY(alignment_counts_device(c->R, L, H, c->n, c->ent_row.p, c->col_ptr.p, c->d_count.p,
                                     locus_group ? d_group.p : nullptr, Lout, d_aln.p, d_uniq.p, d_lu.p, c->s, c->work));
    if (aln_counts) GBRS_HIP_CHECK(hipMemcpy(aln_counts, d_aln.p, d_aln.bytes(), hipMemcpyDeviceToHost));
    if (allele_unique) GBRS_HIP_CHECK(hipMemcpy(allele_unique, d_uniq.p, d_uniq.bytes(), hipMemcpyDeviceToHost));
    if (locus_unique) GBRS_HIP_CHECK(hipMemcpy(locus_unique, d_lu.p, d_lu.bytes(), hipMemcpyDeviceToHost));
    return GBRS_OK;
}

int gbrs_counts_destroy(gbrs_counts_t *c) {
    if (!c) return GBRS_OK;
    (void)hipSetDevice(c->device);
    if (c->s) {
        (void)hipStreamSynchronize(c->s);
        (void)hipStreamDestroy(c->s);
    }
    if (c->work) counts_work_free(c->work);
    delete c;
    return GBRS_OK;
}

int gbrs_alignment_counts(uint64_t R, uint32_t L, uint32_t H, const uint32_t *const *indptr,
// ... 182 lines not shown
```

### gbrs_amd/csrc/em_layout.h

```cpp
#pragma once
#include "common.h"
#include "em_plan.h"

#include <vector>

namespace gbrs {

#ifndef GBRS_TILE_THREADS
#define GBRS_TILE_THREADS 512
#endif
constexpr int TILE_THREADS = GBRS_TILE_THREADS;
constexpr int TILE_WAVES = TILE_THREADS / 64;
#ifndef GBRS_TILE_CAP
#define GBRS_TILE_CAP 32768
#endif
#ifndef GBRS_TILE_WORDS
#define GBRS_TILE_WORDS 2048
#endif
constexpr int TILE_WORDS = GBRS_TILE_WORDS, TILE_WORDS_MAX = GBRS_TILE_CAP - 64, TILE_ROUNDS_MIN = 1;
static_assert(TILE_WORDS <= TILE_WORDS_MAX, "a tile's padded words must fit the dictionary sort");
__host__ __device__ constexpr int pos_bits(int H) { return H <= 8 ? 5 : 3; }
__host__ __device__ constexpr int max_row_words(int H) { return 1 << pos_bits(H); }
#ifndef GBRS_LDS_DOUBLES
#define GBRS_LDS_DOUBLES 3072
#endif
#ifndef GBRS_LDS_DOUBLES_WEIGHTED
#define GBRS_LDS_DOUBLES_WEIGHTED 4608
#endif
#ifndef GBRS_LDS_DOUBLES_H16
#define GBRS_LDS_DOUBLES_H16 4800
#endif
__host__ __device__ constexpr uint32_t dict_index_limit(int H) { return 1u << (32 - H - 2 * pos_bits(H)); }
__host__ __device__ constexpr int lds_theta_doubles(bool weighted, int H) {
    return weighted ? GBRS_LDS_DOUBLES_WEIGHTED : (H == 16 ? GBRS_LDS_DOUBLES_H16 : GBRS_LDS_DOUBLES);
}
__host__ __device__ constexpr int lds_acc_doubles(bool weighted, int H) { return lds_theta_doubles(weighted, H) + 64; }
__host__ __device__ constexpr uint32_t det_dict_cap(int H, bool weighted) { return (lds_acc_doubles(weighted, H) / TILE_WAVES - 1) / H; }
constexpr uint32_t SLOT_DIRECT = 0x80000000u;
constexpr uint32_t SLOT_SET = 0x40000000u;
constexpr uint32_t SLOT_PAIR = 0x20000000u;
constexpr uint32_t DICT_PAIR = 0x80000000u, DICT_SET = 0x40000000u;
constexpr int HEAVY_SLOTS = 16;

struct TileHdr {
    uint32_t batch_base;
    uint16_t n_batches;
    uint16_t n_one;
    uint32_t dict_base;
    uint32_t dict_n_two;
    __host__ __device__ uint32_t dict_count() const { return dict_n_two & 0xFFFFu; }
    __host__ __device__ uint32_t n_two() const { return dict_n_two >> 16; }
    template <bool COUNTED> __host__ __device__ uint32_t dict_count_of() const { return COUNTED ? dict_count() : dict_n_two; }
};
static_assert(sizeof(TileHdr) == 16, "a tile header is one 16-byte scalar load");
static_assert(GBRS_LDS_DOUBLES < 65536 && GBRS_LDS_DOUBLES_WEIGHTED < 65536 && GBRS_LDS_DOUBLES_H16 < 65536,
              "TileHdr::dict_count is 16 bits");
static_assert(2 * (GBRS_TILE_CAP / 64) < 65536, "TileHdr::n_batches is 16 bits");

struct SetArgs {
    uint32_t n_loci;
    const uint32_t *set_ptr, *set_members, *dest_list;
    const uint32_t *dict_b, *dest_b;
    uint32_t relax_zero_weight;
};

struct TileLayout {
    uint64_t n_pairs = 0;
    uint64_t n_rows_in = 0;
    uint64_t n_rows = 0;
    uint64_t n_folded = 0;
    uint64_t n_folded_two = 0;
    uint64_t n_long = 0;
    uint64_t n_tiles = 0, n_batches = 0, n_slots = 0, n_heavy = 0, n_light = 0;
    uint32_t d_max = 0;
    uint32_t cut_passes = 0;
    uint32_t cut_tile_words = 0;
    bool weighted = false;
    bool deterministic = false;
    bool all_one_word = false;

    DevBuf<uint32_t> words;
    DevBuf<TileHdr> tiles;
    DevBuf<uint32_t> dict;
    DevBuf<double> word_weight;
    DevBuf<double> row_weight;
    DevBuf<uint32_t> slot_ptr;
    DevBuf<uint32_t> slot_list;
    DevBuf<uint32_t> heavy_loci;
    DevBuf<uint32_t> light_loci;
    DevBuf<uint32_t> heavy_range, light_range;
    DevBuf<uint32_t> slot_dest;
    DevBuf<uint8_t> locus_class;
    DevBuf<double> partials;
    DevBuf<uint64_t> long_ptr;
    DevBuf<uint32_t> long_loc, long_mask;
    DevBuf<double> long_weight;
    DevBuf<double> acc_extra;
    bool keep_row_ids = false;
    DevBuf<uint32_t> word_row;
    DevBuf<uint32_t> long_row;
    uint32_t n_sets = 0;
    uint64_t n_dest_rows = 0;
    DevBuf<uint32_t> set_ptr, set_members;
    DevBuf<uint32_t> dest_list;
    DevBuf<uint32_t> dict_b, dest_b;
    bool retain_temporaries = false;
    std::vector<void *> retired;
    size_t retired_bytes = 0;
    TileLayout() = default;
    TileLayout(const TileLayout &) = delete;
    TileLayout &operator=(const TileLayout &) = delete;
    ~TileLayout() {
        for (void *p : retired) (void)hipFree(p);
    }
};

inline EmDictLimits dict_limits(bool weighted, int H) {
    return {(uint32_t)max_row_words(H), dict_index_limit(H), (uint32_t)lds_theta_doubles(weighted, H), det_dict_cap(H, weighted)};
}

int build_tile_layout(TileLayout &out, uint64_t R, uint64_t N, const uint32_t *ent_row, const uint64_t *col_ptr,
                      const double *count, hipStream_t stream, const EmPlan &plan);

struct GroupedOrder {
    DevBuf<uint32_t> lh;
    DevBuf<uint32_t> src;
    bool built = false;
};
int build_row_ptr(DevBuf<uint32_t> &row_ptr, uint64_t R, uint64_t N, const uint32_t *ent_row, hipStream_t s);
int build_grouped_order(GroupedOrder &out, uint64_t R, uint32_t L, uint32_t H, uint64_t N, const uint32_t *ent_row,
                        const uint64_t *col_ptr, const uint32_t *rank, const uint32_t *rank_lh, hipStream_t s);

struct CompressResult {
    uint64_t num_ecs = 0, n_entries = 0;
    DevBuf<uint64_t> col_ptr;
    DevBuf<uint32_t> indices;
    DevBuf<double> count;
};
int compress_device(CompressResult &out, uint64_t R, uint32_t L, uint32_t H, uint64_t N, const uint32_t *ent_row,
                    const uint64_t *col_ptr, const double *count, hipStream_t s);

struct CountsWork;
CountsWork *counts_work_new();
void counts_work_free(CountsWork *w);
int alignment_counts_device(uint64_t R, uint32_t L, uint32_t H, uint64_t N, const uint32_t *ent_row,
                            const uint64_t *col_ptr, const double *count, const int32_t *locus_group,
                            uint32_t Lout, double *aln, double *uniq, double *locus_uniq, hipStream_t s,
                            CountsWork *work = nullptr);

__device__ __forceinline__ uint32_t find_column(const uint64_t *__restrict__ col_ptr, uint32_t lo,
                                                uint32_t hi, uint64_t k) {
    while (lo < hi) {
        const uint32_t mid = lo + ((hi - lo + 1) >> 1);
        if (col_ptr[mid] <= k) lo = mid; else hi = mid - 1;
    }
    return lo;
}

__device__ __forceinline__ uint32_t find_column_from(const uint64_t *__restrict__ col_ptr, uint32_t c0,
                                                     uint32_t ncols, uint64_t k) {
    uint32_t lo = c0, step = 1;
    while (lo + step < ncols && col_ptr[lo + step] <= k) {
        lo += step;
        step <<= 1;
    }
    const uint32_t hi = min(lo + step, ncols) - 1;
    return find_column(col_ptr, lo, hi, k);
}

__device__ __forceinline__ uint32_t entry_column(const uint64_t *__restrict__ col_ptr, uint32_t ncols,
                                                 uint64_t k, uint64_t n) {
    const uint64_t kbase = k - (threadIdx.x & 63);
    const uint64_t klast = min(kbase + 63, n - 1);
    uint32_t c_first = 0, c_last = 0;
    if ((threadIdx.x & 63) == 0) {
        c_first = find_column(col_ptr, 0, ncols - 1, kbase);
        c_last = find_column(col_ptr, c_first, ncols - 1, klast);
    }
    c_first = __shfl(c_first, 0, WAVE);
    c_last = __shfl(c_last, 0, WAVE);
    if (c_first == c_last) return c_first;
    return find_column(col_ptr, c_first, c_last, k);
}

}
```

### gbrs_amd/csrc/em_layout.hip

```cpp
#include "em_layout.h"
#include "prim.h"

#include <algorithm>

namespace gbrs {
namespace {



struct BuildFlags {
    unsigned int duplicate;
    unsigned int dict_overflow;
    unsigned int bad_row;
    unsigned int n_long;
    unsigned int long_pairs;
};

constexpr int KEY_ITERS = 32, KEY_SPAN = 64 * KEY_ITERS;
__global__ void __launch_bounds__(256)
make_keys_kernel(uint64_t n, uint32_t ncols, uint32_t L, uint64_t R, unsigned row_shift,
                 const uint64_t *__restrict__ col_ptr, const uint32_t *__restrict__ ent_row,
                 uint64_t *__restrict__ keys, BuildFlags *flags, uint32_t view_h = 0) {
    const int lane = threadIdx.x & 63;
    const uint64_t base = ((uint64_t)blockIdx.x * 4 + (threadIdx.x >> 6)) * KEY_SPAN;
// ... 1642 lines not shown
    std::vector<TileHdr> hdr(T);
    GBRS_HIP_CHECK(hipMemcpy(hdr.data(), out.tiles.p, T * sizeof(TileHdr), hipMemcpyDeviceToHost));
    std::stable_sort(hdr.begin(), hdr.end(), [](const TileHdr &a, const TileHdr &b) { return a.n_batches > b.n_batches; });
    GBRS_HIP_CHECK(hipMemcpy(out.tiles.p, hdr.data(), T * sizeof(TileHdr), hipMemcpyHostToDevice));
    return GBRS_OK;
}

int inverted_index(Build &b, TileLayout &out, uint32_t NS, uint32_t L_in, uint32_t H) {
    hipStream_t s = b.s;
    GBRS_TRY(out.slot_dest.alloc(std::max<uint32_t>(NS, 1)));
    uint32_t NE = 0, n_rows_real = 0;
    if (NS) {
        DevBuf<uint32_t> ecnt, eoff;
        GBRS_TRY(ecnt.alloc(NS)); GBRS_TRY(eoff.alloc(NS));
        hipLaunchKernelGGL(dest_count_kernel, dim3(grid_for(NS)), dim3(256), 0, s, (uint64_t)NS, L_in, out.dict.p,
                           out.n_sets ? out.set_ptr.p : (const uint32_t *)nullptr, ecnt.p);
        GBRS_TRY(scan_total(b.sc, ecnt.p, eoff.p, NS, NE, s));
        if (NE >= SLOT_PAIR) return fail(GBRS_ERR_INVALID, "the tiled layout needs fewer than 2^29 destination rows");
        DevBuf<uint32_t> eloc, eidx, sloc;
        GBRS_TRY(eloc.alloc(NE)); GBRS_TRY(eidx.alloc(NE)); GBRS_TRY(sloc.alloc(NE));
        GBRS_TRY(out.slot_list.alloc(NE));
        GBRS_TRY(out.dest_list.alloc(NE));
        hipLaunchKernelGGL(dest_emit_kernel, dim3(grid_for(NS)), dim3(256), 0, s, (uint64_t)NS, L_in, out.dict.p,
                           out.n_sets ? out.set_ptr.p : (const uint32_t *)nullptr, out.set_members.p, eoff.p, eloc.p, eidx.p,
                           out.slot_dest.p, out.dest_list.p);
        GBRS_TRY(sort_pairs<uint32_t>(b.sc, eloc.p, sloc.p, eidx.p, out.slot_list.p, NE, bits_for(L_in), s));
        hipLaunchKernelGGL(slot_ptr_kernel, dim3(grid_for((uint64_t)L_in + 1)), dim3(256), 0, s, L_in, (uint64_t)NE, sloc.p,
                           out.slot_ptr.p);
        GBRS_HIP_CHECK(hipMemcpyAsync(&n_rows_real, out.slot_ptr.p + L_in, 4, hipMemcpyDeviceToHost, s));
        GBRS_HIP_CHECK(hipStreamSynchronize(s));
    } else {
        GBRS_TRY(out.slot_list.alloc(1));
        GBRS_TRY(out.dest_list.alloc(1));
    }
    out.n_dest_rows = n_rows_real;
    GBRS_TRY(out.partials.alloc(std::max<size_t>((size_t)n_rows_real * H, 1)));
    hipLaunchKernelGGL(locus_class_kernel, dim3(grid_for(L_in)), dim3(256), 0, s, L_in, out.slot_ptr.p, out.slot_list.p,
                       out.locus_class.p, out.dest_list.p);
    if (NS) hipLaunchKernelGGL(dest_route_kernel, dim3(grid_for(NS)), dim3(256), 0, s, (uint64_t)NS, out.dest_list.p, out.slot_dest.p);
    if (out.n_sets && NS) {
        GBRS_TRY(out.dict_b.alloc(NS));
        GBRS_TRY(out.dest_b.alloc(NS));
        hipLaunchKernelGGL(encode_sets_kernel, dim3(grid_for(NS)), dim3(256), 0, s, (uint64_t)NS, L_in, out.set_ptr.p,
                           out.set_members.p, out.dest_list.p, out.dict.p, out.dict_b.p, out.slot_dest.p, out.dest_b.p);
    }
    return GBRS_OK;
}

int heavy_light_lists(TileLayout &out, uint32_t L_in, hipStream_t s) {
    std::vector<uint32_t> sp((size_t)L_in + 1), heavy, lightv;
    GBRS_HIP_CHECK(hipMemcpyAsync(sp.data(), out.slot_ptr.p, sp.size() * 4, hipMemcpyDeviceToHost, s));
    GBRS_HIP_CHECK(hipStreamSynchronize(s));
    for (uint32_t l = 0; l < L_in; ++l)
        if (sp[l + 1] - sp[l] > (uint32_t)HEAVY_SLOTS) heavy.push_back(l);
        else if (sp[l + 1] - sp[l] >= 2) lightv.push_back(l);
    out.n_heavy = heavy.size();
    out.n_light = lightv.size();
    for (int which = 0; which < 2; ++which) {
        const std::vector<uint32_t> &loci = which == 0 ? heavy : lightv;
        DevBuf<uint32_t> &dst = which == 0 ? out.heavy_range : out.light_range;
        std::vector<uint32_t> rng;
        rng.reserve(loci.size() * 3);
        for (uint32_t l : loci) {
            rng.push_back(l);
            rng.push_back(sp[l]);
            rng.push_back(sp[l + 1]);
        }
        GBRS_TRY(dst.alloc(std::max<size_t>(rng.size(), 3)));
        if (!rng.empty()) GBRS_HIP_CHECK(hipMemcpyAsync(dst.p, rng.data(), rng.size() * 4, hipMemcpyHostToDevice, s));
        GBRS_HIP_CHECK(hipStreamSynchronize(s));
    }
    GBRS_TRY(out.light_loci.alloc(std::max<size_t>(lightv.size(), 1)));
    if (!lightv.empty())
        GBRS_HIP_CHECK(hipMemcpyAsync(out.light_loci.p, lightv.data(), lightv.size() * 4, hipMemcpyHostToDevice, s));
    GBRS_TRY(out.heavy_loci.alloc(std::max<size_t>(heavy.size(), 1)));
    if (!heavy.empty())
        GBRS_HIP_CHECK(hipMemcpyAsync(out.heavy_loci.p, heavy.data(), heavy.size() * 4, hipMemcpyHostToDevice, s));
    GBRS_HIP_CHECK(hipStreamSynchronize(s));
    return GBRS_OK;
}

}

int build_tile_layout(TileLayout &out, uint64_t R, uint64_t N, const uint32_t *ent_row, const uint64_t *col_ptr,
                      const double *count, hipStream_t s, const EmPlan &plan) {
    const uint32_t L_in = plan.tL, H = plan.tH;
    out.n_sets = 0;
    out.n_dest_rows = 0;
    const bool keep_row_ids = out.keep_row_ids && !plan.merge;
    if (H > 16) return fail(GBRS_ERR_INVALID, "the tiled layout packs the haplotype mask in 16 bits (H <= 16)");
    if (N >= 0xFFFFFFFFull || L_in >= (1u << 27))
        return fail(GBRS_ERR_INVALID, "the tiled layout needs N < 2^32 entries and L < 2^27 loci per handle");
    DeferFrees park_temporaries(out.retain_temporaries ? &out.retired : nullptr, &out.retired_bytes);
    StageTimer stg("layout");
    Build b(s, &stg);
    GBRS_TRY(b.init());
    out.d_max = plan.d_max;
    out.deterministic = plan.deterministic;
    if (!plan.dict_room)
        return fail(GBRS_ERR_UNSUPPORTED, "the deterministic tile layout has no room for a row's loci at H = %u", H);
    out.weighted = plan.weighted;
    out.n_pairs = out.n_rows = out.n_rows_in = out.n_long = out.n_tiles = out.n_batches = out.n_slots = out.n_folded = out.n_folded_two = 0;
    GBRS_TRY(out.slot_ptr.alloc((size_t)L_in + 1));
    GBRS_HIP_CHECK(hipMemsetAsync(out.slot_ptr.p, 0, out.slot_ptr.bytes(), s));
    GBRS_TRY(out.locus_class.alloc(L_in));
    GBRS_HIP_CHECK(hipMemsetAsync(out.locus_class.p, 0, out.locus_class.bytes(), s));
    if (N == 0) { GBRS_HIP_CHECK(hipStreamSynchronize(s)); return GBRS_OK; }

    RowPairs rp;
    stg.mark("0 setup");
    GBRS_TRY(build_row_pairs(b, rp, R, L_in, H, N, ent_row, col_ptr, 5 + bits_for(L_in - 1) , plan.view));
    out.n_pairs = rp.P;
    out.n_rows_in = rp.R1;
    stg.mark("3 rows");
    if (plan.whole_row_sets && rp.R1 > 0) {
        GBRS_TRY(whole_row_sets(b, out, rp, plan));
        stg.mark("3b locus sets");
    }
    if (plan.locus_sets && rp.R1 > 0 && out.n_sets == 0) {
        if (plan.group_sets) GBRS_TRY(mask_group_sets(b, out, rp, plan));
        stg.mark("3c mask-group sets");
    }
    SortedRows rows;
    LayoutRows lr;
    GBRS_TRY(order_rows(b, out, rp, rows, L_in + out.n_sets, H));
    stg.mark("4 order rows");
    GBRS_TRY(merge_rows(b, out, rp, rows, lr, count, plan));
    out.all_one_word = false;
    stg.mark("5 merge");
    if (rows.n_long) GBRS_TRY(long_rows(b, out, rp, rows, count, keep_row_ids, plan));
    rows.srow.release();
    if (!keep_row_ids) rp.row_orig.release();
    if (lr.M == 0) { GBRS_HIP_CHECK(hipStreamSynchronize(s)); return GBRS_OK; }
    stg.mark("6 long rows");
    Tiles tiles;
    TileParts parts;
    GBRS_TRY(cut_tiles(b, out, rp, lr, tiles, plan));
    stg.mark("7 tiles");
    if (plan.row_order != 0) GBRS_TRY(order_rows_in_tiles(b, out, lr, tiles, plan.row_order == 1));
    tiles.dnew.release();
    tiles.tflag.release();
    stg.mark("7b row order");
    GBRS_TRY(pad_rows(b, out, tiles, parts, lr.M, plan));
    stg.mark("8 padding");
    GBRS_TRY(tile_dictionaries(b, out, rp, lr, tiles, parts));
    stg.mark("9 dictionaries");
    GBRS_TRY(emit_words(b, out, rp, lr, tiles, parts, keep_row_ids, plan));
    parts.release(); tiles.release(); lr.release(); rp.release();
    out.row_weight.release();
    if (plan.reorder_tiles && tiles.T > 1) GBRS_TRY(reorder_tiles(out, tiles.T));
    stg.mark("10 words");
    GBRS_TRY(inverted_index(b, out, parts.NS, L_in, H));
    stg.mark("11 inverted index");
    GBRS_TRY(heavy_light_lists(out, L_in, s));
    stg.mark("12 heavy / light lists");
    GBRS_HIP_CHECK(hipGetLastError());
    return GBRS_OK;
}

}

namespace gbrs {
namespace {

__global__ void __launch_bounds__(256)
row_hist_kernel(uint64_t n, const uint32_t *__restrict__ ent_row, uint32_t *__restrict__ cnt) {
// ... 78 lines not shown
```

### gbrs_amd/csrc/em_plan.h

```cpp
#pragma once

#include <algorithm>
#include <cstdint>
#include <cstdlib>

#include "../../include/gbrs_hip.h"

namespace gbrs {


struct EmTuning {
    struct Int {
        bool set = false;
        int v = 0;
        bool is(int x) const { return set && v == x; }
        bool nonzero() const { return set && v != 0; }
    };
    int dict_cap = 0;
    Int locus_sets;
    Int group_sets;
    uint32_t set_min_rows = 192;
    Int run_words;
    int tile_words = 0;
    bool tile_cut = true;
    int tile_target = 0;
    bool tile_order = true;
    bool half_loci = false;
    bool persistent = false;
    unsigned persistent_groups = 0;
    bool no_phase_split = false;
    uint32_t resample_cut = 256;
    bool no_fused_mstep = false;
    bool no_float_check = false;
};

namespace em_env {
inline EmTuning::Int integer(const char *name) {
    EmTuning::Int i;
    if (const char *e = std::getenv(name); e) { i.set = true; i.v = std::atoi(e); }
    return i;
}
template <typename T>
inline void at_least(const char *name, int lo, T &v) {
    if (const char *e = std::getenv(name); e && std::atoi(e) >= lo) v = (T)std::atoi(e);
}
}

inline EmTuning em_tuning_from_env() {
    using namespace em_env;
    EmTuning t;
    at_least("GBRS_TUNING_DICT_CAP", 1, t.dict_cap);
    t.locus_sets = integer("GBRS_TUNING_LOCUS_SETS");
    t.group_sets = integer("GBRS_TUNING_GROUP_SETS");
    at_least("GBRS_TUNING_SET_MIN_ROWS", 1, t.set_min_rows);
    t.run_words = integer("GBRS_TUNING_RUN_WORDS");
    at_least("GBRS_TUNING_TILE_WORDS", 64, t.tile_words);
    t.tile_cut = !integer("GBRS_TUNING_TILE_CUT").is(0);
    at_least("GBRS_TUNING_TILE_TARGET", 1, t.tile_target);
    t.tile_order = !integer("GBRS_TUNING_TILE_ORDER").is(0);
    t.half_loci = integer("GBRS_TUNING_HALF_LOCI").nonzero();
    t.persistent = integer("GBRS_TUNING_PERSISTENT").nonzero();
    at_least("GBRS_TUNING_PERSISTENT_GROUPS", 1, t.persistent_groups);
    t.no_phase_split = integer("GBRS_TUNING_NO_PHASE_SPLIT").nonzero();
    at_least("GBRS_TUNING_RESAMPLE_CUT", 1, t.resample_cut);
    t.no_fused_mstep = integer("GBRS_TUNING_NO_FUSED_MSTEP").nonzero();
    t.no_float_check = integer("GBRS_TUNING_NO_FLOAT_CHECK").set;
    return t;
}


struct EmDictLimits {
    uint32_t max_row_words = 0;
    uint32_t index_limit = 0;
    uint32_t lds_doubles = 0;
    uint32_t det_cap = 0;
};

struct EmShape {
    uint32_t H = 0, L = 0;
    uint64_t R = 0, N = 0;
    uint32_t flags = 0;
    bool counts_given = false;
    int n_cu = 0;
    uint32_t tile_words = 0, tile_words_max = 0, tile_rounds_min = 1;
    uint32_t err_blocks = 0;
    EmDictLimits dict;
    EmDictLimits dict_half;
};

inline bool em_weighted(uint32_t flags, bool counts_given) {
    return counts_given || (flags & (GBRS_EM_RESAMPLE | GBRS_EM_MERGE_IDENTICAL_ROWS)) != 0;
}


struct EmPlan {
    bool tiled = false;
    uint32_t view = 1;
    uint32_t tH = 0, tL = 0;
    int row_order = 2;
    bool merge = false, deterministic = false, weighted = false;
    unsigned side_by_side = 1;
    bool locus_sets = false;
    bool whole_row_sets = false;
    bool group_sets = false;
    bool group_sets_forced = false;
    int sets_forced = -1;
    uint32_t set_min_rows = 192;
    bool counted_pairs = false;
    bool fold = false;
    int fold_mode = 3;
    bool fold_forced = false;
    unsigned per_cu = 3;
    uint64_t places = 0;
    uint32_t tile_words = 0, tile_words_cap = 0;
    uint32_t tile_words_forced = 0;
    bool exact_cut = false;
    uint64_t tile_target = 0;
    bool tile_target_forced = false;
    bool reorder_tiles = true;
    uint32_t d_max = 0, dseg = 0;
    bool dict_room = false;
    uint32_t persist_groups = 0;
    uint32_t lead_mask = ~0u;
    uint32_t resample_cut = 256;
    bool no_fused_mstep = false, no_float_check = false;
};

inline uint64_t em_tile_target(uint64_t places, unsigned side_by_side, uint32_t err_blocks, int forced) {
    if (forced > 0) return (uint64_t)forced;
    const uint64_t n = std::max<uint64_t>(places / std::max(side_by_side, 1u), 1);
    return n > err_blocks ? n - err_blocks : n;
}

inline EmPlan em_plan(const EmShape &s, const EmTuning &t) {
    EmPlan p;
    const uint32_t f = s.flags;
    p.merge = (f & GBRS_EM_MERGE_IDENTICAL_ROWS) != 0;
    p.deterministic = (f & GBRS_EM_DETERMINISTIC) != 0;
    p.weighted = em_weighted(f, s.counts_given);
    p.side_by_side = (f & GBRS_EM_SIDE_BY_SIDE) ? 2u : 1u;
    p.no_fused_mstep = t.no_fused_mstep;
    p.no_float_check = t.no_float_check;
    if ((f & GBRS_EM_RESAMPLE) && s.counts_given) p.resample_cut = t.resample_cut;
    p.tiled = !(f & GBRS_EM_LAYOUT_CSC) && s.H <= 16 && s.N < 0xFFFFFFFFull;
    p.tH = s.H;
    p.tL = s.L;
    if (!p.tiled) return p;

    if (f & GBRS_EM_FORCE_INTERLEAVE) p.row_order = 1;
    else if (f & GBRS_EM_NO_STREAMS) p.row_order = (p.weighted && !(f & GBRS_EM_NO_INTERLEAVE)) ? 1 : 0;
    if (s.H == 16 && t.half_loci && !p.weighted && !p.deterministic && (uint64_t)s.L * 2 < (1u << 27)) p.view = 2;
    p.tH = s.H / p.view;
    p.tL = s.L * p.view;
    const EmDictLimits &d = p.view == 2 ? s.dict_half : s.dict;

    p.locus_sets = !(f & GBRS_EM_NO_LOCUS_SETS) && !p.weighted;
    p.whole_row_sets = p.locus_sets && t.locus_sets.is(1);
    if (t.locus_sets.set) p.sets_forced = t.locus_sets.v != 0;
    p.group_sets = p.locus_sets && !t.group_sets.is(0);
    p.group_sets_forced = t.group_sets.is(1);
    p.set_min_rows = t.set_min_rows;

    p.counted_pairs = p.row_order == 2 && !p.weighted && !p.deterministic && p.view == 1 &&
                      (p.tH == 1 || p.tH == 2 || p.tH == 4 || p.tH == 8);
    p.fold = !(f & GBRS_EM_NO_RUN_WORDS) && p.counted_pairs && !t.run_words.is(0);
    p.fold_mode = t.run_words.is(1) ? 2 : 3;
    p.fold_forced = t.run_words.set;

    p.per_cu = (p.weighted || p.tH > 8) ? 2u : 3u;
    const unsigned n_cu = (unsigned)std::max(s.n_cu, 1);
    p.places = (uint64_t)s.tile_rounds_min * p.per_cu * n_cu;
    p.tile_words = s.tile_words;
    p.tile_words_cap = p.weighted ? std::min<uint32_t>(s.tile_words_max, 16320) : s.tile_words_max;
    if (t.tile_words) p.tile_words_forced = std::min<uint32_t>((uint32_t)t.tile_words, s.tile_words_max);
    p.exact_cut = t.tile_cut && !p.tile_words_forced;
    p.tile_target = em_tile_target(p.places, p.side_by_side, s.err_blocks, t.tile_target);
    p.tile_target_forced = t.tile_target > 0;
    p.reorder_tiles = t.tile_order;

    p.d_max = std::min<uint32_t>(1024, d.lds_doubles / p.tH);
    p.d_max = std::min(p.d_max, d.index_limit);
    if (p.deterministic) p.d_max = std::min(p.d_max, d.det_cap);
    if (t.dict_cap > (int)d.max_row_words) p.d_max = std::min(p.d_max, (uint32_t)t.dict_cap);
    p.dict_room = p.d_max > d.max_row_words;
    p.dseg = p.dict_room ? p.d_max - d.max_row_words : 0;

    unsigned groups = p.per_cu * n_cu / p.side_by_side;
    if (t.persistent_groups) groups = t.persistent_groups;
    p.persist_groups = t.persistent ? std::max(groups, 1u) : 0u;
    p.lead_mask = t.no_phase_split ? 0u : ~0u;
    return p;
}


inline uint32_t em_tile_words(const EmPlan &p, uint64_t total_words) {
    if (p.tile_words_forced) return p.tile_words_forced;
    const uint64_t fit = total_words * p.side_by_side / p.places;
    return (uint32_t)std::min<uint64_t>(std::max<uint64_t>(fit, p.tile_words), p.tile_words_cap) & ~63u;
}

constexpr int TILE_CUT_PASSES = 3;
inline bool em_take_exact_cut(const EmPlan &p, uint64_t total_words) {
    if (!p.exact_cut) return false;
    return p.tile_target_forced || (total_words + p.tile_target - 1) / p.tile_target <= p.tile_words_cap;
}
inline uint32_t em_cut_clamp(const EmPlan &p, uint64_t words) {
    return (uint32_t)std::min<uint64_t>(std::max<uint64_t>((words + 63) & ~63ull, p.tile_words), p.tile_words_cap);
}
inline uint32_t em_cut_tile_words(const EmPlan &p, uint64_t total_words) {
    return em_cut_clamp(p, (total_words + p.tile_target - 1) / p.tile_target);
}
inline uint32_t em_cut_rescale(const EmPlan &p, uint32_t tile_words, uint64_t tiles) {
    if (tiles <= p.tile_target) return tile_words;
    return std::max(tile_words, em_cut_clamp(p, ((uint64_t)tile_words * tiles + p.tile_target - 1) / p.tile_target));
}

inline bool em_take_fold(const EmPlan &p, uint64_t words_in, uint64_t folded) {
    if (p.fold_forced) return true;
    return folded * 100 >= words_in * 15 && (words_in - folded) * p.side_by_side / p.places >= (uint64_t)p.tile_words;
}

inline bool em_use_whole_row_sets(const EmPlan &p, uint64_t P, uint64_t P2, uint64_t L, uint64_t V) {
    if (p.sets_forced >= 0) return p.sets_forced != 0;
    return P2 * 100 <= P * 85 && P2 >= 100 * (L + V) && V <= 2 * L;
}
// ... 6 lines not shown
```

### gbrs_amd/csrc/em_step.h

```cpp
#pragma once

#include "em_plan.h"

namespace gbrs {

struct EmStepShape {
    bool tiled = false;
    uint32_t H = 0;
    uint32_t tH = 0, view = 1;
    bool no_tiles = true, no_long = true, no_entries = true;
    bool weighted = false, deterministic = false, all_one_word = false;
    uint32_t persist_groups = 0;
    bool acc_handed_out = false;
    bool no_fused_mstep = false;
};

enum class EmPass {
    Prepare,
    Step,
    Partial,
    Model,
};
enum class EmEstep { None, Csc, Tiles, TilesOneWord, TilesDeterministic, Persistent, PersistentOneWord, Models };
enum class EmLongRows { None, Atomic, Serial };
enum class EmGather { None, Written, All };
enum class EmMstep { Fused, Elem, PerLocus };

struct EmStepRoute {
    EmPass pass = EmPass::Step;
    EmEstep estep = EmEstep::None;
    int width = 0;
    bool weighted = false;
    EmLongRows long_rows = EmLongRows::None;
    EmGather gather = EmGather::None;
    EmMstep mstep = EmMstep::PerLocus;
    bool mstep_adds_extra = false;
    bool counts_stale = false;
    bool err_rides = false;
    bool err_defer = false;
};

#if defined(GBRS_NO_ONEWORD)
constexpr bool EM_ONEWORD_TILES = false;
#else
constexpr bool EM_ONEWORD_TILES = true;
#endif

inline EmStepRoute em_step_route(const EmStepShape &s, EmPass pass) {
    EmStepRoute r;
    r.pass = pass;
    const bool ones = pass == EmPass::Prepare;
    r.mstep = (s.H & (s.H - 1)) == 0 ? EmMstep::Elem : EmMstep::PerLocus;
    if (pass == EmPass::Model) {
        r.estep = EmEstep::Models;
        return r;
    }
    if (!s.tiled) {
        r.estep = s.no_entries ? EmEstep::None : EmEstep::Csc;
        return r;
    }
    const uint32_t tH = s.tH;
    r.width = (tH == 1 || tH == 2 || tH == 4 || tH == 8 || tH == 16) ? (int)tH : 0;
    r.weighted = s.weighted;
    const bool one_word = r.width == 8 && !s.weighted && s.all_one_word;
    if (s.no_tiles) r.estep = EmEstep::None;
    else if (!ones && !s.deterministic && s.persist_groups > 0 && r.width >= 1 && r.width <= 8)
        r.estep = one_word ? EmEstep::PersistentOneWord : EmEstep::Persistent;
    else if (s.deterministic) r.estep = EmEstep::TilesDeterministic;
    else if (EM_ONEWORD_TILES && one_word) r.estep = EmEstep::TilesOneWord;
    else r.estep = EmEstep::Tiles;
    r.err_rides = !ones && !s.no_tiles;
    if (!s.no_long) r.long_rows = s.deterministic ? EmLongRows::Serial : EmLongRows::Atomic;
    const bool fused = pass == EmPass::Step && r.mstep == EmMstep::Elem && !s.acc_handed_out && s.view == 1 && !s.no_fused_mstep;
    const bool all = pass != EmPass::Step || s.acc_handed_out || (tH & (tH - 1)) != 0 || s.view > 1;
    r.gather = fused ? EmGather::None : all ? EmGather::All : EmGather::Written;
    if (fused) r.mstep = EmMstep::Fused;
    r.mstep_adds_extra = r.gather == EmGather::Written && !s.no_long;
    r.counts_stale = fused;
    r.err_defer = !ones;
    return r;
}

}
```

### gbrs_amd/csrc/em_tiles.inc

```


#ifndef GBRS_ESTEP_WAVES16
#define GBRS_ESTEP_WAVES16 4
#endif
#ifndef GBRS_ESTEP_WAVES
#define GBRS_ESTEP_WAVES 6
#endif
#if !defined(GBRS_NO_MASK_ZLO) && !defined(GBRS_MASK_ZLO)
#define GBRS_MASK_ZLO 1
#endif
__host__ __device__ constexpr int estep_batches(bool weighted, int ht) { return (weighted && ht <= 8) ? 2 : 1; }
#ifndef GBRS_FTAB
#define GBRS_FTAB 1
#endif
__host__ __device__ constexpr bool estep_uses_ftab(int ub, int ht) { return GBRS_FTAB && ub == 1 && ht == 8; }
#ifndef GBRS_THETA_REGS
#define GBRS_THETA_REGS 1
#endif
__host__ __device__ constexpr bool estep_theta_regs(int ub, int ht, bool det) { return GBRS_THETA_REGS && ub == 1 && ht == 8 && !det; }
#ifndef GBRS_THETA_PLANES
#define GBRS_THETA_PLANES 1
#endif
__host__ __device__ constexpr bool theta_planar(int ht) { return GBRS_THETA_PLANES && (ht == 8 || ht == 16); }
__host__ __device__ constexpr bool estep_uses_zlo(int ub) {
// ... 298 lines not shown
#pragma unroll
                    for (int h = 0; h < HC; ++h)
                        if (h < H) atomicAdd(ap + h, st.pc[h]);
                    st.pidx = 0xFFFFFFFFu;
                }
            }
            if (miss) {
#pragma unroll
                for (int h = 0; h < HC; ++h) {
                    asm volatile("v_mov_b64 %0, %1" : "+v"(st.pc[h]) : "v"(st.c[h]));
                    asm volatile("v_mov_b64 %0, 0" : "+v"(st.c[h]));
                }
                st.pidx = st.cidx;
                st.cidx = idx[u];
            }
        }
#else
        if (miss) st.cidx = idx[u];
#endif
        if (HT > 0) {
#pragma unroll
            for (int h = 0; h < HT; ++h) {
                if ((ZLO || FTAB) && HT == 8) { st.c[h] = fma(f8[u][h & 7], v[u], st.c[h]); continue; }
                if (ZLO && HT == 16) { st.c[h] = fma(f16[u][h & 15], v[u], st.c[h]); continue; }
                st.c[h] = fma(bit_as_double(mask[u], h), v[u], st.c[h]);
            }
        } else {
#pragma unroll
            for (int h = 0; h < HC; ++h)
                if (h < H) st.c[h] = fma(bit_as_double(mask[u], h), v[u], st.c[h]);
        }
    }
}

template <bool ZERO>
__device__ __forceinline__ double sum_copies(double *__restrict__ s_acc, uint32_t i, uint32_t K, uint32_t stride) {
    double a = 0.0;
    if (K >= 8) {
        for (uint32_t c = 0; c < K; c += 8) {
            double v[8];
#pragma unroll
            for (int q = 0; q < 8; ++q) v[q] = s_acc[(c + q) * stride + i];
            if (ZERO) {
#pragma unroll
                for (int q = 0; q < 8; ++q) s_acc[(c + q) * stride + i] = 0.0;
            }
#pragma unroll
            for (int q = 0; q < 8; ++q) a += v[q];
        }
    } else {
        double v[4];
#pragma unroll
        for (int q = 0; q < 4; ++q) v[q] = s_acc[min((uint32_t)q, K - 1u) * stride + i];
        if (ZERO) {
#pragma unroll
            for (int q = 0; q < 4; ++q)
                if ((uint32_t)q < K) s_acc[q * stride + i] = 0.0;
        }
#pragma unroll
        for (int q = 0; q < 4; ++q) a += (uint32_t)q < K ? v[q] : 0.0;
    }
    return a;
}

#if defined(GBRS_DIAG_TILE_TIMES)
__device__ unsigned long long *g_tile_stamps = nullptr;
__device__ __forceinline__ void diag_stamp(int slot, unsigned long long extra = 0) {
    if (g_tile_stamps && threadIdx.x == 0) {
        g_tile_stamps[(size_t)blockIdx.x * 8 + slot] = __builtin_amdgcn_s_memrealtime();
        if (slot == 0) {
            g_tile_stamps[(size_t)blockIdx.x * 8 + 4] = __builtin_amdgcn_s_getreg((31 << 11) | (0 << 6) | 4);
            g_tile_stamps[(size_t)blockIdx.x * 8 + 5] = __builtin_amdgcn_s_getreg((3 << 11) | (0 << 6) | 20);
            g_tile_stamps[(size_t)blockIdx.x * 8 + 5] |= extra << 8;
        }
    }
}
#define GBRS_DIAG_STAMP(...) do { if (!ONES) diag_stamp(__VA_ARGS__); } while (0)
#define GBRS_DIAG_PSTAMP(t, slot) do { if (g_tile_stamps && threadIdx.x == 0) g_tile_stamps[(size_t)(t) * 8 + (slot)] = __builtin_amdgcn_s_memrealtime(); } while (0)
#else
#define GBRS_DIAG_STAMP(...) do { } while (0)
#define GBRS_DIAG_PSTAMP(t, slot) do { } while (0)
#endif

template <int HT, bool WEIGHTED, bool ONES, bool DET = false, bool ONEWORD = false>
#if defined(GBRS_ESTEP_VGPR_CAP)
__attribute__((amdgpu_num_vgpr(GBRS_ESTEP_VGPR_CAP)))
#endif
__global__ void __launch_bounds__(TILE_THREADS, (HT > 0 && HT <= 8) ? (WEIGHTED ? 4 : GBRS_ESTEP_WAVES) : (WEIGHTED ? 3 : GBRS_ESTEP_WAVES16))
tile_estep_kernel(uint32_t Hrt, const TileHdr *__restrict__ tiles, const uint32_t *__restrict__ words,
                  const uint32_t *__restrict__ dict, const double *__restrict__ word_weight,
                  const double *__restrict__ theta, double *__restrict__ partials,
                  const uint32_t *__restrict__ slot_dest, double *__restrict__ acc_direct,
                  EmScalars *__restrict__ sc, uint32_t n_tiles, ErrArgs ea, SetArgs sets,
                  uint32_t lead_mask ) {
    constexpr int LDS_ACC_DOUBLES = lds_acc_doubles(WEIGHTED, HT);
    __shared__ __attribute__((aligned(16))) double s_theta[lds_theta_doubles(WEIGHTED, HT)];
    __shared__ __attribute__((aligned(16))) double2 s_ftab[32];
    if (estep_uses_ftab(estep_batches(WEIGHTED, HT), HT) && threadIdx.x < 32) {
        const uint32_t k = threadIdx.x & 15u, sh = (threadIdx.x >> 4) * 2;
        s_ftab[threadIdx.x] = make_double2((double)((k >> sh) & 1u), (double)((k >> (sh + 1)) & 1u));
    }
    __shared__ __attribute__((aligned(16))) double s_acc[LDS_ACC_DOUBLES];
    __shared__ uint32_t s_stop;
    if (blockIdx.x >= n_tiles) {
        if (!ONES) err_finish_body(ea, blockIdx.x - n_tiles);
        return;
    }
    const uint32_t stop_flag = ONES ? 0u : sc->stop;
    const int H = HT > 0 ? HT : (int)Hrt;
    const int PB = pos_bits(H);
#if defined(GBRS_ESTEP_PRIO)
    __builtin_amdgcn_s_setprio(GBRS_ESTEP_PRIO);
#endif
    const TileHdr th = tiles[blockIdx.x];
    GBRS_DIAG_STAMP(0, th.n_batches);
    const int lane = threadIdx.x & 63, wave = __builtin_amdgcn_readfirstlane(threadIdx.x >> 6);
#ifndef GBRS_WEIGHTED_PD
#define GBRS_WEIGHTED_PD 4
#endif
#ifndef GBRS_RAW_PD
#define GBRS_RAW_PD 4
#endif
#ifndef GBRS_H16_PD
#define GBRS_H16_PD 8
#endif
    constexpr int UB = estep_batches(WEIGHTED, HT), PD = WEIGHTED ? GBRS_WEIGHTED_PD : (HT == 16 ? GBRS_H16_PD : GBRS_RAW_PD);
    const uint32_t b0 = (uint32_t)(((uint64_t)th.n_batches * wave) / TILE_WAVES);
    const uint32_t b1 = (uint32_t)(((uint64_t)th.n_batches * (wave + 1)) / TILE_WAVES);
    constexpr bool SPLIT = HT > 0 && HT <= 8 && !WEIGHTED && !DET;
    const uint32_t n_one = SPLIT ? (uint32_t)th.n_one : 0u;
    const uint32_t n_lead = SPLIT ? ((n_one + (ONEWORD ? 0u : th.n_two())) & lead_mask) : 0u;
    uint32_t bm = b0;
    if (SPLIT && n_lead > b0) bm = b0 + ((min(b1, n_lead) - b0) / PD) * PD;
    const uint32_t *wp = words + (size_t)th.batch_base * 64;
    const double *wtp = WEIGHTED ? word_weight + (size_t)th.batch_base * 64 : nullptr;
    const __amdgpu_buffer_rsrc_t wres = __builtin_amdgcn_make_buffer_rsrc(const_cast<uint32_t *>(wp), 0, (int)(b1 * 256u), 0x00020000);
    const __amdgpu_buffer_rsrc_t wtres = __builtin_amdgcn_make_buffer_rsrc(const_cast<double *>(WEIGHTED ? wtp : (const double *)wp), 0,
                                                                          WEIGHTED ? (int)(b1 * 512u) : 0, 0x00020000);
    int voff = (int)(b0 * 256u) + lane * 4;
    auto load_word = [&](int ahead) -> uint32_t {
        return (uint32_t)__builtin_amdgcn_raw_buffer_load_b32(wres, voff + ahead * 256, 0, 0);
    };
    auto load_weight = [&](int ahead) -> double {
        const auto q = __builtin_amdgcn_raw_buffer_load_b64(wtres, 2 * voff + ahead * 512, 0, 0);
        return __hiloint2double((int)q[1], (int)q[0]);
    };
    uint32_t ring[PD];
    double wring[WEIGHTED ? PD : 1];
#pragma unroll
    for (int u = 0; u < PD; ++u) {
        ring[u] = load_word(u);
        if (WEIGHTED) wring[u] = load_weight(u);
    }
    const uint32_t DH = th.template dict_count_of<SPLIT>() * H;
    const uint32_t stride = DH | 1u;
    uint32_t K = LDS_ACC_DOUBLES / stride;
    K = K >= 64 ? 64u : (1u << (31 - __clz((int)K)));
#if defined(GBRS_ABLATE_PROLOGUE)
    constexpr bool gather_ones = true;
#else
    constexpr bool gather_ones = ONES;
#endif
    for (uint32_t i = threadIdx.x; i < K * stride; i += TILE_THREADS) s_acc[i] = 0.0;
    GBRS_DIAG_STAMP(7);
    for (uint32_t i = threadIdx.x; i < DH; i += TILE_THREADS) {
        const uint32_t j = i / H, h = i - j * H;
        constexpr uint32_t DP = theta_planar(HT) ? lds_theta_doubles(WEIGHTED, HT) / (HT > 0 ? HT : 1) : 0;
        const uint32_t at = theta_planar(HT) ? (((h >> 1) * DP + j) << 1) + (h & 1u) : i;
        double tv;
#if defined(GBRS_ABLATE_PROLOGUE_FULL)
        if (true) {
            tv = 1.0;
        } else
#endif
        if (sets.set_ptr == nullptr) {
            tv = gather_ones ? 1.0 : theta[(size_t)dict[th.dict_base + j] * H + h];
        } else {
            const uint32_t e = dict[th.dict_base + j], e2 = sets.dict_b[th.dict_base + j];
            if (!(e & (DICT_PAIR | DICT_SET))) {
                tv = gather_ones ? 1.0 : theta[(size_t)e * H + h];
            } else if (e & DICT_PAIR) {
                if (gather_ones) {
                    tv = 2.0;
                } else {
                    const double t0 = theta[(size_t)(e & ~DICT_PAIR) * H + h], t1 = theta[(size_t)e2 * H + h];
                    tv = t0 + t1;
                }
            } else {
                const uint32_t k = e & ~DICT_SET;
                const uint32_t m0 = sets.set_ptr[k], m1 = sets.set_ptr[k + 1];
                tv = 0.0;
                if (gather_ones) {
                    tv = (double)(m1 - m0);
                } else {
                    constexpr int SETB = (HT == 16 && !WEIGHTED) ? 1 : 4;
                    for (uint32_t m = m0; m < m1; m += SETB) {
                        uint32_t mem[SETB];
                        double tm[SETB];
#pragma unroll
                        for (int q = 0; q < SETB; ++q) mem[q] = sets.set_members[min(m + q, m1 - 1)];
#pragma unroll
                        for (int q = 0; q < SETB; ++q) tm[q] = theta[(size_t)mem[q] * H + h];
#pragma unroll
                        for (int q = 0; q < SETB; ++q) tv += m + q < m1 ? tm[q] : 0.0;
                    }
                }
            }
        }
        s_theta[at] = tv;
    }
    GBRS_DIAG_STAMP(6);
    if (threadIdx.x == 0) s_stop = stop_flag;
    __syncthreads();
    if (s_stop) return;
    GBRS_DIAG_STAMP(1);
#if defined(GBRS_ESTEP_PRIO)
    __builtin_amdgcn_s_setprio(0);
#endif
    double *my_acc = s_acc + (DET ? (uint32_t)wave : (lane & (K - 1))) * stride;
    constexpr int HC = HT > 0 ? HT : 16;
    int zlo[32];
#pragma unroll
    for (int k = 0; k < 32; ++k) {
        if constexpr (estep_uses_zlo(estep_batches(WEIGHTED, HT))) asm volatile("v_mov_b32 %0, 0" : "=v"(zlo[k]));
        else zlo[k] = 0;
    }
    LaneAcc<HC> st;
#pragma unroll
    for (int h = 0; h < HC; ++h) st.c[h] = st.pc[h] = 0.0;
    if constexpr (estep_theta_regs(UB, HT, DET)) {
#pragma unroll
        for (int h = 0; h < HC / 2; ++h) st.th[h] = theta_pair_t{0.0, 0.0};
    }
    st.cidx = st.pidx = 0xFFFFFFFFu;
    st.bad = 0;
    if constexpr (SPLIT) {
        for (uint32_t b = b0; b < bm; b += PD) {
#pragma unroll
            for (int tt = 0; tt < PD; ++tt) {
                const uint32_t w[1] = {ring[tt]};
                const double wt[1] = {1.0};
                ring[tt] = load_word(PD + tt);
                tile_batches<HT, false, HC, false, 1, ONEWORD, true>(w, wt, H, PB, lane, s_theta, my_acc, st, zlo, s_ftab, 0u, 0u, 0,
                                                                     !ONEWORD && b + tt >= n_one);
            }
            voff += PD * 256;
            asm volatile("" : "+v"(voff));
        }
        if constexpr (estep_theta_regs(UB, HT, DET)) {
#pragma unroll
            for (int h = 0; h < HC / 2; ++h) asm volatile("" : "+v"(st.th[h]));
        }
    }
    int lane_g = lane;
    if constexpr (SPLIT) asm volatile("" : "+v"(lane_g));
    const uint32_t misfit_bits = pair_misfit_bits(H, PB, lane_g);
#if defined(GBRS_ABLATE_BATCHES)
    for (uint32_t b = bm; b < bm; b += PD) {
#else
    for (uint32_t b = bm; b < b1; b += PD) {
#endif
#pragma unroll
        for (int tt = 0; tt < PD / UB; ++tt) {
            uint32_t w[UB];
            double wt[UB];
#pragma unroll
            for (int u = 0; u < UB; ++u) {
                const int slot = tt * UB + u;
                w[u] = ring[slot];
                wt[u] = WEIGHTED ? wring[slot] : 1.0;
                ring[slot] = load_word(PD + slot);
                if (WEIGHTED) wring[slot] = load_weight(PD + slot);
            }
            if (b + tt * UB < b1) tile_batches<HT, WEIGHTED, HC, DET, UB, ONEWORD>(w, wt, H, PB, lane, s_theta, my_acc, st, zlo, s_ftab, misfit_bits, WEIGHTED ? sets.relax_zero_weight : 0u,
                                                                                   !SPLIT ? 0 : (b + tt * UB < n_one ? 1 : (!ONEWORD && b + tt * UB < n_one + th.n_two() ? 2 : 0)));
        }
        voff += PD * 256;
        asm volatile("" : "+v"(voff));
    }
#if defined(GBRS_ABLATE_ATOMICS)
    asm volatile("" ::"v"(st.c[0]), "v"(st.pc[0]));
    st.cidx = st.pidx = 0xFFFFFFFFu;
#endif
    if (DET) {
        if (K < (uint32_t)TILE_WAVES) sc->float_error = 1;
        det_flush<HC>(my_acc, H, lane, st.pidx, st.pc);
        det_flush<HC>(my_acc, H, lane, st.cidx, st.c);
    }
    constexpr int FIRST_FLUSH = 0;
#if defined(GBRS_ABLATE_FLUSH)
    asm volatile("" ::"v"(st.c[0]), "v"(st.pc[0]));
    for (int which = 2; which < 2; ++which) {
#else
    for (int which = FIRST_FLUSH; which < 2 && !DET; ++which) {
#endif
        const uint32_t fidx = which == 0 ? st.pidx : st.cidx;
        if (fidx != 0xFFFFFFFFu) {
            double *ap = my_acc + fidx * H;
#pragma unroll
            for (int h = 0; h < HC; ++h)
                if (h < H) atomicAdd(ap + h, which == 0 ? st.pc[h] : st.c[h]);
        }
    }
    if (st.bad != 0) sc->float_error = 1;
#if defined(GBRS_ESTEP_PRIO)
    __builtin_amdgcn_s_setprio(GBRS_ESTEP_PRIO);
#endif
    __syncthreads();
    GBRS_DIAG_STAMP(2);
    uint32_t tix = threadIdx.x;
    asm volatile("" : "+v"(tix));
    for (uint32_t i = tix; i < DH; i += TILE_THREADS) {
        double a = sum_copies<false>(s_acc, i, K, stride);
        if (SPLIT && estep_theta_regs(UB, HT, DET) && n_lead != 0 && !(a < 4e307)) sc->float_error = 1;
#if defined(GBRS_ABLATE_ATOMICS) || defined(GBRS_ABLATE_BATCHES)
        a = 1.0;
#endif
        const uint32_t j = i / H, h = i - j * H;
        const uint32_t d = slot_dest[th.dict_base + j];
        const uint32_t d2 = sets.set_ptr ? sets.dest_b[th.dict_base + j] : 0u;
        auto put = [&](uint32_t dq) {
            if (dq & SLOT_DIRECT) acc_direct[(size_t)(dq & ~SLOT_DIRECT) * H + h] = a;
            else partials[(size_t)dq * H + h] = a;
        };
        if (sets.set_ptr == nullptr || !(d & (SLOT_SET | SLOT_PAIR))) {
            put(d);
        } else if (d & SLOT_PAIR) {
            put(d & ~SLOT_PAIR);
            put(d2);
        } else {
            const uint32_t *dl = sets.dest_list + (d & ~SLOT_SET);
            const uint32_t n = dl[0];
            for (uint32_t q = 1; q <= n; ++q) put(dl[q]);
        }
    }
    GBRS_DIAG_STAMP(3);
}

template <int HT, bool WEIGHTED>
__device__ __forceinline__ double dict_entry_theta(const double *__restrict__ theta, const SetArgs &sets, uint32_t e, uint32_t e2,
                                                   uint32_t H, uint32_t h) {
    if (sets.set_ptr == nullptr || !(e & (DICT_PAIR | DICT_SET))) return theta[(size_t)e * H + h];
    if (e & DICT_PAIR) {
        const double t0 = theta[(size_t)(e & ~DICT_PAIR) * H + h], t1 = theta[(size_t)e2 * H + h];
        return t0 + t1;
    }
    const uint32_t k = e & ~DICT_SET;
    const uint32_t m0 = sets.set_ptr[k], m1 = sets.set_ptr[k + 1];
    double tv = 0.0;
    constexpr int SETB = (HT == 16 && !WEIGHTED) ? 1 : 4;
    for (uint32_t m = m0; m < m1; m += SETB) {
        uint32_t mem[SETB];
        double tm[SETB];
#pragma unroll
        for (int q = 0; q < SETB; ++q) mem[q] = sets.set_members[min(m + q, m1 - 1)];
#pragma unroll
        for (int q = 0; q < SETB; ++q) tm[q] = theta[(size_t)mem[q] * H + h];
#pragma unroll
        for (int q = 0; q < SETB; ++q) tv += m + q < m1 ? tm[q] : 0.0;
    }
    return tv;
}

template <int HT, bool WEIGHTED>
__device__ __forceinline__ uint32_t theta_lds_index(uint32_t i, uint32_t j, uint32_t h) {
    constexpr uint32_t DP = theta_planar(HT) ? lds_theta_doubles(WEIGHTED, HT) / (HT > 0 ? HT : 1) : 0;
    return theta_planar(HT) ? (((h >> 1) * DP + j) << 1) + (h & 1u) : i;
}

template <int HT, bool WEIGHTED, bool ONEWORD = false>
__global__ void __launch_bounds__(TILE_THREADS, (HT > 0 && HT <= 8) ? (WEIGHTED ? 4 : GBRS_ESTEP_WAVES) : (WEIGHTED ? 3 : GBRS_ESTEP_WAVES16))
tile_estep_persistent_kernel(uint32_t Hrt, const TileHdr *__restrict__ tiles, const uint32_t *__restrict__ words,
                             const uint32_t *__restrict__ dict, const double *__restrict__ word_weight,
                             const double *__restrict__ theta, double *__restrict__ partials,
                             const uint32_t *__restrict__ slot_dest, int64_t direct_delta ,
                             EmScalars *__restrict__ sc, uint32_t n_tiles, uint32_t n_groups, ErrArgs ea, SetArgs sets) {
    constexpr int LDS_ACC_DOUBLES = lds_acc_doubles(WEIGHTED, HT);
    constexpr bool PF = HT > 0 && HT <= 8;
    constexpr bool EPF = PF && !(HT == 8 && !WEIGHTED && !ONEWORD);
    __shared__ __attribute__((aligned(16))) double s_theta[lds_theta_doubles(WEIGHTED, HT)];
    __shared__ __attribute__((aligned(16))) double2 s_ftab[32];
    __shared__ __attribute__((aligned(16))) double s_acc[LDS_ACC_DOUBLES];
    __shared__ uint32_t s_stop;
    if (estep_uses_ftab(estep_batches(WEIGHTED, HT), HT) && threadIdx.x < 32) {
        const uint32_t k = threadIdx.x & 15u, sh = (threadIdx.x >> 4) * 2;
        s_ftab[threadIdx.x] = make_double2((double)((k >> sh) & 1u), (double)((k >> (sh + 1)) & 1u));
    }
    if (blockIdx.x >= n_groups) {
        err_finish_body(ea, blockIdx.x - n_groups);
        return;
    }
    const uint32_t stop_flag = sc->stop;
    const int H = HT > 0 ? HT : (int)Hrt;
    const int PB = pos_bits(H);
    const int lane = threadIdx.x & 63, wave = __builtin_amdgcn_readfirstlane(threadIdx.x >> 6);
    constexpr int UB = estep_batches(WEIGHTED, HT), PD = WEIGHTED ? GBRS_WEIGHTED_PD : (HT == 16 ? GBRS_H16_PD : GBRS_RAW_PD);
    constexpr int HC = HT > 0 ? HT : 16;
    const uint32_t G = n_groups, me = blockIdx.x;
    uint32_t round = 0, t = me;
    TileHdr th = tiles[t];
    uint32_t b0, b1;
    __amdgpu_buffer_rsrc_t wres, wtres;
    int voff;
// ... 323 lines not shown
```

### gbrs_amd/engine.py

```python
from __future__ import annotations

import ctypes as C

import numpy as np

from . import _lib


def _allowed_array(allowed, L):
    al = np.ascontiguousarray(allowed, dtype=np.uint32)
    if al.shape != (L,):
        raise RuntimeError('allowed must hold one haplotype bit mask per locus')
    return al


class EmEngine:
    def __init__(self, handle, shape, keepalive=None):
        self._h = handle
        self.shape = shape
        self._keep = keepalive

    @classmethod
    def from_host(cls, R, L, H, indptr, indices, count=None, eff_len=None, device=0, flags=0, allowed=None):
        lib = _lib.load()
# ... 26 lines not shown
        if allowed is not None:
            al = _allowed_array(allowed, L)
            _lib.check(lib.gbrs_em_create_masked_device(R, L, H, _lib.raw_table(indptr_ptrs),
                                                        _lib.raw_table(indices_ptrs), count_ptr, eff_len_ptr,
                                                        _lib.ptr(al), device, flags, C.byref(h)))
        else:
            _lib.check(lib.gbrs_em_create_device(R, L, H, _lib.raw_table(indptr_ptrs),
                                                 _lib.raw_table(indices_ptrs), count_ptr, eff_len_ptr,
                                                 device, flags, C.byref(h)))
        return cls(h, (L, H, R))

    def set_initial_values(self, values):
        vals = [np.ascontiguousarray(v, dtype=np.float64) for v in values]
        _lib.check(_lib.load().gbrs_em_set_initial_values(self._h, _lib.ptr_table(vals)))

    def close(self):
        if self._h is not None:
            _lib.load().gbrs_em_destroy(self._h)
            self._h = None

    def __del__(self):
        try:
            self.close()
        except Exception:
            pass

    def prepare(self, pseudocount=0.0):
        _lib.check(_lib.load().gbrs_em_prepare(self._h, float(pseudocount)))

    def step(self, n=1, want_err=False):
        err = C.c_double(0.0)
        _lib.check(_lib.load().gbrs_em_step(self._h, int(n), C.byref(err) if want_err else None))
        return err.value

    def run(self, model=4, tol=0.001, max_iters=999):
        n_it = C.c_int(0)
        cap = max(int(max_iters), 1)
        hist = np.zeros(cap, dtype=np.float64)
        _lib.check(_lib.load().gbrs_em_run(self._h, int(model), float(tol), int(max_iters), C.byref(n_it),
                                           _lib.ptr(hist), cap, None))
        return int(n_it.value), hist[:n_it.value].copy()

    def theta(self):
        L, H, R = self.shape
        out = np.empty((H, L), dtype=np.float64)
        _lib.check(_lib.load().gbrs_em_get(self._h, _lib.ptr(out), None))
        return out

    def expected_counts(self):
        L, H, R = self.shape
        out = np.empty((H, L), dtype=np.float64)
        _lib.check(_lib.load().gbrs_em_get(self._h, None, _lib.ptr(out)))
        return out

    def set_theta(self, theta):
        L, H, R = self.shape
        t = np.ascontiguousarray(theta, dtype=np.float64).reshape(H, L)
        _lib.check(_lib.load().gbrs_em_set_theta(self._h, _lib.ptr(t)))

    def group_sums(self, group_ptr, members, which=0):
        L, H, R = self.shape
        gp = np.ascontiguousarray(group_ptr, dtype=np.int64)
        mem = np.ascontiguousarray(members, dtype=np.int64)
        G = len(gp) - 1
        out = np.empty((H, G), dtype=np.float64)
        _lib.check(_lib.load().gbrs_em_group_sums(self._h, G, _lib.ptr(gp), _lib.ptr(mem), which, _lib.ptr(out)))
        return out

    def info(self):
        inf = _lib.EmInfo()
        _lib.check(_lib.load().gbrs_em_info(self._h, C.byref(inf)))
        return inf

    def fold_counts(self):
        one, two = C.c_uint64(0), C.c_uint64(0)
        _lib.check(_lib.load().gbrs_em_fold_counts(self._h, C.byref(one), C.byref(two)))
        return int(one.value), int(two.value)

    def tile_cut(self):
        passes, words = C.c_uint32(0), C.c_uint32(0)
        _lib.check(_lib.load().gbrs_em_tile_cut(self._h, C.byref(passes), C.byref(words)))
        return int(passes.value), int(words.value)

    def tile_shapes(self):
        n = int(self.info().num_tiles)
        batches, entries = np.zeros(n, np.uint32), np.zeros(n, np.uint32)
        _lib.check(_lib.load().gbrs_em_tile_shapes(self._h, batches.ctypes.data, entries.ctypes.data, n))
        return batches, entries

    def _partial(self, fn):
        p = C.c_void_p()
        n = C.c_uint64(0)
        _lib.check(fn(self._h, C.byref(p), C.byref(n)))
        return p.value, int(n.value)

    def estep_partial(self):
        return self._partial(_lib.load().gbrs_em_estep_partial)

    def prepare_partial(self):
        return self._partial(_lib.load().gbrs_em_prepare_partial)

    def finish_step(self, want_err=True):
        err = C.c_double(0.0)
        _lib.check(_lib.load().gbrs_em_finish_step(self._h, C.byref(err) if want_err else None))
        return err.value

    def finish_prepare(self, pseudocount=0.0):
        _lib.check(_lib.load().gbrs_em_finish_prepare(self._h, float(pseudocount)))

    def sync(self):
        _lib.check(_lib.load().gbrs_em_sync(self._h))

    def pair_begin(self, other, max_iters):
        _lib.check(_lib.load().gbrs_em_pair_begin(self._h, other._h, int(max_iters)))

    def pair_check(self, other, tol):
        _lib.check(_lib.load().gbrs_em_pair_check(self._h, other._h, float(tol)))

    def pair_status(self, other, cap):
        it, st = C.c_int(0), C.c_int(0)
        hist = np.zeros(max(int(cap), 1), dtype=np.float64)
        _lib.check(_lib.load().gbrs_em_pair_status(self._h, other._h, C.byref(it), C.byref(st), _lib.ptr(hist), len(hist)))
        return int(it.value), bool(st.value), hist[:min(int(it.value), len(hist))].copy()

    def stream(self):
        return _lib.load().gbrs_em_stream(self._h)

    def set_stream(self, stream_ptr):
        _lib.check(_lib.load().gbrs_em_set_stream(self._h, stream_ptr))
```

### include/gbrs_hip.h

```cpp
#ifndef GBRS_HIP_H
#define GBRS_HIP_H

#include <stdint.h>

#ifdef __cplusplus
extern "C" {
#endif

#define GBRS_ABI_VERSION 5

enum gbrs_status {
    GBRS_OK = 0,
    GBRS_ERR_INVALID = -1,
    GBRS_ERR_HIP = -2,
    GBRS_ERR_NO_DEVICE = -3,
    GBRS_ERR_FLOAT = -4,
    GBRS_ERR_UNSUPPORTED = -5,
    GBRS_ERR_STATE = -6
};

const char *gbrs_last_error(void);
int gbrs_abi_version(void);
int gbrs_device_count(void);
int gbrs_warm_up(int device);
// ... 25 lines not shown

int gbrs_em_create_device(uint64_t num_rows, uint32_t num_loci, uint32_t num_haps,
                          const uint32_t *const *indptr, const uint32_t *const *indices,
                          const double *count, const double *eff_len,
                          int device, uint32_t flags, gbrs_em_t **out);

int gbrs_em_create_masked(uint64_t num_rows, uint32_t num_loci, uint32_t num_haps,
                          const uint32_t *const *indptr, const uint32_t *const *indices,
                          const double *count, const double *eff_len, const uint32_t *allowed,
                          int device, uint32_t flags, gbrs_em_t **out);
int gbrs_em_create_masked_device(uint64_t num_rows, uint32_t num_loci, uint32_t num_haps,
                                 const uint32_t *const *indptr, const uint32_t *const *indices,
                                 const double *count, const double *eff_len, const uint32_t *allowed,
                                 int device, uint32_t flags, gbrs_em_t **out);

int gbrs_em_set_initial_values(gbrs_em_t *em, const double *const *values);

int gbrs_em_prepare(gbrs_em_t *em, double pseudocount);

int gbrs_em_step(gbrs_em_t *em, int n_iters, double *err_sum_out);

int gbrs_em_set_groups(gbrs_em_t *em, int64_t num_groups, const int64_t *group_ptr, const int64_t *members);

int gbrs_em_step_model(gbrs_em_t *em, int model, int n_iters, double *err_sum_out);

int gbrs_em_run(gbrs_em_t *em, int model, double tol, int max_iters,
                int *n_iters_out, double *err_hist, int err_hist_cap, double *elapsed_s);

int gbrs_em_get(gbrs_em_t *em, double *theta, double *expected_counts);

int gbrs_em_posterior(gbrs_em_t *em, uint32_t hap, double *out, uint64_t out_len);

int gbrs_em_resample(gbrs_em_t *em, uint64_t seed, uint32_t replicate);
int gbrs_em_weights(gbrs_em_t *em, double *out);
int gbrs_em_resample_info(gbrs_em_t *em, uint64_t *extra_device_bytes, uint64_t *num_big_rows, uint32_t *cut);

int gbrs_em_bootstrap_begin(gbrs_em_t *em, int64_t num_groups, const int64_t *group_ptr, const int64_t *members);
int gbrs_em_bootstrap_add(gbrs_em_t *em, double *tpm, double *counts, double *gene_tpm, double *gene_counts);
int gbrs_em_bootstrap_get(gbrs_em_t *em, int level, uint32_t *num_replicates, double *tpm_mean, double *tpm_sd,
                          double *count_mean, double *count_sd, double *tpm_total_mean, double *tpm_total_sd,
                          double *count_total_mean, double *count_total_sd);

int gbrs_em_set_theta(gbrs_em_t *em, const double *theta);

int gbrs_em_group_sums(gbrs_em_t *em, int64_t num_groups, const int64_t *group_ptr,
                       const int64_t *members, int which, double *out);

int gbrs_em_estep_partial(gbrs_em_t *em, void **partial_dev, uint64_t *n_elems);
int gbrs_em_finish_step(gbrs_em_t *em, double *err_sum_out);
int gbrs_em_prepare_partial(gbrs_em_t *em, void **partial_dev, uint64_t *n_elems);
int gbrs_em_finish_prepare(gbrs_em_t *em, double pseudocount);
void *gbrs_em_stream(gbrs_em_t *em);
int gbrs_em_set_stream(gbrs_em_t *em, void *stream);
int gbrs_em_sync(gbrs_em_t *em);

int gbrs_em_pair_begin(gbrs_em_t *a, gbrs_em_t *b, int max_iters);
int gbrs_em_pair_check(gbrs_em_t *a, gbrs_em_t *b, double tol);
int gbrs_em_pair_status(gbrs_em_t *a, gbrs_em_t *b, int *iters_done, int *stopped, double *err_hist, int err_hist_cap);

typedef struct gbrs_em_info {
    uint64_t num_rows;
    uint64_t num_entries;
    uint64_t num_device_rows;
    uint64_t num_device_words;
    uint64_t bytes_per_iter;
    uint64_t algorithmic_bytes;
    double   last_estep_ms;
    double   last_step_ms;
    uint32_t num_loci, num_haps;
    uint32_t layout;
    uint32_t num_folded_rows;
    uint64_t num_tiles;
    uint64_t num_slots;
    uint64_t num_long_rows;
    uint64_t num_heavy_loci;
    uint64_t num_light_loci;
    uint64_t estep_bytes;
    uint64_t retained_build_bytes;
    uint64_t num_locus_sets;
} gbrs_em_info_t;
int gbrs_em_info(gbrs_em_t *em, gbrs_em_info_t *info);
int gbrs_em_fold_counts(gbrs_em_t *em, uint64_t *one_word_reads, uint64_t *two_word_reads);
int gbrs_em_tile_cut(gbrs_em_t *em, uint32_t *passes, uint32_t *tile_words);
int gbrs_em_tile_shapes(gbrs_em_t *em, uint32_t *n_batches, uint32_t *dict_entries, uint64_t n);

int gbrs_alignment_counts(uint64_t num_rows, uint32_t num_loci, uint32_t num_haps,
                          const uint32_t *const *indptr, const uint32_t *const *indices,
                          const double *count, const int32_t *locus_group, uint32_t num_out_loci,
                          int device, double *aln_counts, double *allele_unique, double *locus_unique);

typedef struct gbrs_counts gbrs_counts_t;
int gbrs_counts_create(uint64_t num_rows, uint32_t num_loci, uint32_t num_haps,
                       const uint32_t *const *indptr, const uint32_t *const *indices,
                       const double *count, int device, gbrs_counts_t **out);
int gbrs_counts_get(gbrs_counts_t *c, const int32_t *locus_group, uint32_t num_out_loci,
                    double *aln_counts, double *allele_unique, double *locus_unique);
int gbrs_counts_destroy(gbrs_counts_t *c);

int gbrs_shard_plan(uint64_t num_rows, uint32_t num_loci, uint32_t num_haps,
                    const uint32_t *const *indptr, const uint32_t *const *indices,
                    int world, int device, uint64_t *bounds);
int gbrs_shard_index(uint64_t num_rows, uint32_t num_loci, uint32_t num_haps,
                     const uint32_t *const *indptr, const uint32_t *const *indices,
                     uint64_t r0, uint64_t r1, int device,
                     uint32_t *const *indptr_out, uint64_t *nnz_out);
int gbrs_shard_gather(uint64_t num_rows, uint32_t num_loci, uint32_t num_haps,
                      const uint32_t *const *indptr, const uint32_t *const *indices,
                      uint64_t r0, uint64_t r1, uint32_t l_split, const double *const *values,
                      int device, const uint64_t *nnz_local, uint32_t *const *indices_out,
                      double *const *values_out, uint64_t *straddling);

int gbrs_em_destroy(gbrs_em_t *em);

typedef struct gbrs_compress gbrs_compress_t;
int gbrs_compress_create(uint64_t num_rows, uint32_t num_loci, uint32_t num_haps,
                         const uint32_t *const *indptr, const uint32_t *const *indices,
                         const double *count, int device, gbrs_compress_t **out,
                         uint64_t *num_ecs, uint64_t *nnz_per_hap);
int gbrs_compress_get(gbrs_compress_t *c, uint32_t *const *indptr_out, uint32_t *const *indices_out,
                      double *count_out);
int gbrs_compress_destroy(gbrs_compress_t *c);

typedef struct gbrs_matops gbrs_matops_t;
int gbrs_matops_create(uint64_t num_rows, uint32_t num_loci, uint32_t num_haps, const uint32_t *const *indptr,
                       const uint32_t *const *indices, int device, gbrs_matops_t **out);
int gbrs_matops_intersect(gbrs_matops_t *m, const uint32_t *const *indptr_b, const uint32_t *const *indices_b);
int gbrs_matops_append_rows(gbrs_matops_t *m, uint64_t num_rows_b, const uint32_t *const *indptr_b,
                            const uint32_t *const *indices_b);
int gbrs_matops_keep_unique_rows(gbrs_matops_t *m, const int32_t *locus_group, uint32_t num_groups,
                                 int ignore_haplotype, uint8_t *keep_out);
int gbrs_matops_mask_columns(gbrs_matops_t *m, const uint32_t *allowed);
int gbrs_matops_sizes(gbrs_matops_t *m, uint64_t *num_rows, uint64_t *nnz_per_hap, uint32_t *sorted_inputs);
int gbrs_matops_get(gbrs_matops_t *m, uint32_t *const *indptr_out, uint32_t *const *indices_out);
int gbrs_matops_shared_counts(gbrs_matops_t *m, const int32_t *locus_group, uint32_t num_groups, uint64_t *nnz_out);
int gbrs_matops_shared_counts_get(gbrs_matops_t *m, uint64_t *indptr_out, uint32_t *indices_out, double *data_out);
int gbrs_matops_shared_counts_info(gbrs_matops_t *m, uint64_t *num_columns, uint64_t *pattern_entries,
                                   uint64_t *pairs_emitted, uint32_t *batches, uint64_t *pair_budget,
                                   uint64_t *peak_device_bytes, double *device_ms);
int gbrs_matops_destroy(gbrs_matops_t *m);

typedef struct gbrs_tensor gbrs_tensor_t;
int gbrs_tensor_create(uint64_t num_rows, uint32_t num_loci, uint32_t num_haps, const uint32_t *const *indptr,
                       const uint32_t *const *indices, const double *const *values ,
                       const double *count , int device, gbrs_tensor_t **out);
int gbrs_tensor_set_groups(gbrs_tensor_t *t, int64_t num_groups, const int64_t *group_ptr, const int64_t *members);
int gbrs_tensor_reset(gbrs_tensor_t *t);
int gbrs_tensor_multiply(gbrs_tensor_t *t, int form, const double *m, uint64_t m_len);
int gbrs_tensor_multiply_tensor(gbrs_tensor_t *t, const gbrs_tensor_t *other);
int gbrs_tensor_normalize(gbrs_tensor_t *t, int axis);
int gbrs_tensor_sum_reads(gbrs_tensor_t *t, double *out_HxL);
int gbrs_tensor_sum_loci(gbrs_tensor_t *t, double *out_RxH);
int gbrs_tensor_copy(gbrs_tensor_t *t, gbrs_tensor_t **out);
int gbrs_tensor_values(gbrs_tensor_t *t, uint32_t hap, double *out, uint8_t *live , uint64_t len);
int gbrs_tensor_set_values(gbrs_tensor_t *t, uint32_t hap, const double *v, uint64_t len);
int gbrs_tensor_nnz(gbrs_tensor_t *t, uint64_t *per_hap);
int gbrs_tensor_destroy(gbrs_tensor_t *t);

typedef struct gbrs_bam gbrs_bam_t;
int gbrs_bam_open(const char *path, int32_t threads, gbrs_bam_t **out, uint64_t *n_ref, uint64_t *ref_names_len);
int gbrs_bam_references(gbrs_bam_t *b, char *names, uint64_t names_cap, uint64_t *name_off, uint32_t *ref_len);
int gbrs_bam_set_reference_map(gbrs_bam_t *b, uint64_t n_ref, const uint32_t *hap, const uint32_t *locus,
                               uint32_t num_haps, uint32_t num_loci);
int gbrs_bam_convert(gbrs_bam_t *b, int device, uint64_t *num_reads, uint32_t *name_width, uint64_t *nnz_per_hap,
                     double *stage_seconds);
int gbrs_bam_get(gbrs_bam_t *b, uint32_t *const *indptr_out, uint32_t *const *indices_out, char *rname_out);
int gbrs_bam_scan_records(gbrs_bam_t *b, uint64_t cap, int32_t *refid, uint32_t *flag, uint64_t *name_off, char *names,
// ... 196 lines not shown
```

Before: 24300.

## Fuse the model-4 M-step into the next E-step tile prologue via gather slots

For unweighted tiled layouts with 1-8 haplotypes, each E-step tile now applies the previous iteration's M-step (theta*acc/len, per-locus totals, error partial sums) while loading theta into LDS. It accumulates directly into a triple-rotated acc buffer through new gather slots instead of writing partials for a separate reduction. This removes the standalone M-step kernel, the partial-reduction pass and the acc memset from each iteration, at the cost of extra buffers and rotated state. It also needs settle logic to recover the right theta when convergence stops mid-batch. Owner-only writes keep duplicated loci consistent, but atomics on acc may change reduction order.

```diff
diff --git a/gbrs_amd/_lib.py b/gbrs_amd/_lib.py
--- a/gbrs_amd/_lib.py
+++ b/gbrs_amd/_lib.py
@@ -15,7 +15,7 @@
     "gbrs_em_get", "gbrs_em_set_theta", "gbrs_em_group_sums", "gbrs_em_estep_partial",
     "gbrs_em_finish_step", "gbrs_em_prepare_partial", "gbrs_em_finish_prepare", "gbrs_em_stream",
     "gbrs_em_set_stream",
-    "gbrs_em_sync", "gbrs_em_pair_begin", "gbrs_em_pair_check", "gbrs_em_pair_status", "gbrs_em_info", "gbrs_em_fold_counts", "gbrs_em_tile_cut", "gbrs_em_tile_shapes",
+    "gbrs_em_sync", "gbrs_em_pair_begin", "gbrs_em_pair_check", "gbrs_em_pair_status", "gbrs_em_info", "gbrs_em_fold_counts", "gbrs_em_tile_cut", "gbrs_em_gather_mstep", "gbrs_em_tile_shapes",
     "gbrs_alignment_counts",
     "gbrs_counts_create", "gbrs_counts_get", "gbrs_counts_destroy", "gbrs_em_destroy",
     "gbrs_shard_plan", "gbrs_shard_index", "gbrs_shard_gather",
@@ -179,6 +179,7 @@
         "gbrs_em_info": [vp, C.POINTER(EmInfo)],
         "gbrs_em_fold_counts": [vp, C.POINTER(u64), C.POINTER(u64)],
         "gbrs_em_tile_cut": [vp, C.POINTER(u32), C.POINTER(u32)],
+        "gbrs_em_gather_mstep": [vp, C.POINTER(u32)],
         "gbrs_em_tile_shapes": [vp, vp, vp, u64],
         "gbrs_alignment_counts": [u64, u32, u32, pp, pp, vp, vp, u32, i32, vp, vp, vp],
         "gbrs_counts_create": [u64, u32, u32, pp, pp, vp, i32, pp],
@@ -270,7 +271,7 @@
     }
     sigs.update(_host_signatures())
     for name, args in sigs.items():
-        if name in ("gbrs_em_fold_counts", "gbrs_em_tile_cut", "gbrs_em_tile_shapes") and os.environ.get("GBRS_TUNING_LIB") and not hasattr(lib, name):
+        if name in ("gbrs_em_fold_counts", "gbrs_em_tile_cut", "gbrs_em_gather_mstep", "gbrs_em_tile_shapes") and os.environ.get("GBRS_TUNING_LIB") and not hasattr(lib, name):
             continue
         fn = getattr(lib, name)
         fn.restype = i32
diff --git a/gbrs_amd/csrc/em.hip b/gbrs_amd/csrc/em.hip
--- a/gbrs_amd/csrc/em.hip
+++ b/gbrs_amd/csrc/em.hip
@@ -488,6 +488,15 @@
         DevBuf<double> cur[2][2], mean[2][2], m2[2][2], tot_mean[2][2], tot_m2[2][2];
     } stats;
 
+    struct Gather {
+        bool ready = false;
+        DevBuf<double> acc_b[2], theta_b, tot_prev_b, tot_new_b, msums_b;
+        int rot = 0;
+        bool clean = false;
+        bool primed = false;
+        std::vector<const double *> wrote;
+    } gm;
+
     int red_blocks() const { return (int)std::min<uint64_t>(RED_BLOCKS, (L + RED_THREADS - 1) / RED_THREADS); }
 };
 
@@ -544,7 +553,7 @@
 }
 
 
-EmStepRoute em_route(const gbrs_em *em, EmPass pass) {
+EmStepShape em_step_shape(const gbrs_em *em) {
     const TileLayout &tl = em->tl;
     EmStepShape s;
     s.tiled = em->layout == 1;
@@ -554,8 +563,9 @@
     s.persist_groups = em->plan.persist_groups;
     s.acc_handed_out = em->acc_external;
     s.no_fused_mstep = em->plan.no_fused_mstep;
-    return em_step_route(s, pass);
-}
+    return s;
+}
+EmStepRoute em_route(const gbrs_em *em, EmPass pass) { return em_step_route(em_step_shape(em), pass); }
 
 template <int HT, bool ONES>
 int em_launch_tiles_h(gbrs_em *em, const EmStepRoute &r) {
@@ -572,7 +582,7 @@
 #define GBRS_LAUNCH_TILES(W, D)                                                                                            \
     hipLaunchKernelGGL((tile_estep_kernel<HT, W, ONES, D>), grid, block, 0, em->stream, tH, tl.tiles.p, tl.words.p,        \
                        tl.dict.p, ww, em->theta.p, tl.partials.p, tl.slot_dest.p, em->acc.p, em->scalars.p,               \
-                       (uint32_t)tl.n_tiles, ea, sets, lead_mask)
+                       (uint32_t)tl.n_tiles, ea, sets, lead_mask, GatherArgs{})
     switch (r.estep) {
         case EmEstep::Persistent:
         case EmEstep::PersistentOneWord: {
@@ -595,7 +605,7 @@
         case EmEstep::TilesOneWord:
             hipLaunchKernelGGL((tile_estep_kernel<HT == 8 ? 8 : 1, false, ONES, false, HT == 8>), grid, block, 0, em->stream, tH,
                                tl.tiles.p, tl.words.p, tl.dict.p, ww, em->theta.p, tl.partials.p, tl.slot_dest.p, em->acc.p,
-                               em->scalars.p, (uint32_t)tl.n_tiles, ea, sets, lead_mask);
+                               em->scalars.p, (uint32_t)tl.n_tiles, ea, sets, lead_mask, GatherArgs{});
             break;
 #endif
         default:
@@ -740,11 +750,11 @@
 }
 
 template <int MODE, int H>
-void em_launch_mstep_elem(gbrs_em *em, const double *extra, const double *len) {
+void em_launch_mstep_elem(gbrs_em *em, double *theta, const double *acc, const double *extra, const double *len) {
     const uint64_t npair = (uint64_t)em->L * MstepRow<H>::LANES;
     const unsigned nb = (unsigned)((npair + RED_THREADS - 1) / RED_THREADS);
     em->msum_blocks = nb;
-    hipLaunchKernelGGL((mstep_elem_kernel<MODE, H>), dim3(nb), dim3(RED_THREADS), 0, em->stream, em->L, em->theta.p, em->acc.p,
+    hipLaunchKernelGGL((mstep_elem_kernel<MODE, H>), dim3(nb), dim3(RED_THREADS), 0, em->stream, em->L, theta, acc,
                        extra, len, em->counts.p, em->tot_prev.p, em->tot_new.p, em->msums.p, em->msum_cap, em->scalars.p);
 }
 template <int MODE>
@@ -760,12 +770,12 @@
     }
     const double *extra = r.mstep_adds_extra ? em->tl.acc_extra.p : (const double *)nullptr;
     switch (em->H) {
-    case 1: em_launch_mstep_elem<MODE, 1>(em, extra, len); break;
-    case 2: em_launch_mstep_elem<MODE, 2>(em, extra, len); break;
-    case 4: em_launch_mstep_elem<MODE, 4>(em, extra, len); break;
-    case 8: em_launch_mstep_elem<MODE, 8>(em, extra, len); break;
-    case 16: em_launch_mstep_elem<MODE, 16>(em, extra, len); break;
-    case 32: em_launch_mstep_elem<MODE, 32>(em, extra, len); break;
+    case 1: em_launch_mstep_elem<MODE, 1>(em, em->theta.p, em->acc.p, extra, len); break;
+    case 2: em_launch_mstep_elem<MODE, 2>(em, em->theta.p, em->acc.p, extra, len); break;
+    case 4: em_launch_mstep_elem<MODE, 4>(em, em->theta.p, em->acc.p, extra, len); break;
+    case 8: em_launch_mstep_elem<MODE, 8>(em, em->theta.p, em->acc.p, extra, len); break;
+    case 16: em_launch_mstep_elem<MODE, 16>(em, em->theta.p, em->acc.p, extra, len); break;
+    case 32: em_launch_mstep_elem<MODE, 32>(em, em->theta.p, em->acc.p, extra, len); break;
     default: return fail(GBRS_ERR_UNSUPPORTED, "the element-parallel M-step has no instance for this haplotype count");
     }
     return GBRS_OK;
@@ -794,6 +804,8 @@
     GBRS_TRY(em_flush_err(em));
     GBRS_TRY(em_launch_mstep(em, r));
     em->counts_stale = r.counts_stale;
+    em->gm.primed = true;
+    em->gm.clean = false;
     if (defer_err && r.err_defer) {
         em->err_pending = true;
         em->err_pending_target = target_err;
@@ -840,6 +852,149 @@
     em->last_step_ms = ss / n;
 }
 
+
+bool em_gather_route(const gbrs_em *em) {
+    if (em->layout != 1 || em->N == 0) return false;
+    const TileLayout &tl = em->tl;
+    const EmStepShape s = em_step_shape(em);
+    EmGatherShape g;
+    g.no_heavy = tl.n_heavy == 0;
+    g.n_tiles = (uint32_t)tl.n_tiles; g.tile_waves = TILE_WAVES; g.msum_cap = em->msum_cap;
+    g.posterior = (em->flags & GBRS_EM_POSTERIOR) != 0;
+    g.resample = em->resample;
+    g.pair_mode = em->pair_ev_mstep != nullptr;
+    EmTuning t;
+    t.no_gather_mstep = em->plan.no_gather_mstep;
+    return em_gather_mstep(s, g, EmPass::Step, t);
+}
+
+int em_gather_setup(gbrs_em *em) {
+    gbrs_em::Gather &gm = em->gm;
+    const size_t LH = (size_t)em->L * em->H;
+    if (!gm.ready) {
+        GBRS_TRY(build_gather_slots(em->tl, em->plan.tL, em->stream));
+        for (DevBuf<double> *b : {&gm.acc_b[0], &gm.acc_b[1], &gm.theta_b}) {
+            GBRS_TRY(b->alloc(LH));
+            GBRS_HIP_CHECK(hipMemsetAsync(b->p, 0, b->bytes(), em->stream));
+        }
+        GBRS_TRY(gm.tot_prev_b.alloc(em->L));
+        GBRS_TRY(gm.tot_new_b.alloc(em->L));
+        GBRS_TRY(gm.msums_b.alloc(em->msums.n));
+        GBRS_HIP_CHECK(hipMemsetAsync(gm.msums_b.p, 0, gm.msums_b.bytes(), em->stream));
+        gm.ready = true;
+        gm.clean = false;
+    }
+    if (!gm.clean) {
+        for (double *p : {em->acc.p, gm.acc_b[0].p, gm.acc_b[1].p}) GBRS_HIP_CHECK(hipMemsetAsync(p, 0, LH * sizeof(double), em->stream));
+        for (double *p : {em->tot_prev.p, em->tot_new.p, gm.tot_prev_b.p, gm.tot_new_b.p})
+            GBRS_HIP_CHECK(hipMemsetAsync(p, 0, (size_t)em->L * sizeof(double), em->stream));
+        gm.rot = 0;
+        gm.clean = true;
+    }
+    return GBRS_OK;
+}
+
+template <int HT>
+void em_launch_gather_tiles(gbrs_em *em, bool one_word, const double *theta, const ErrArgs &ea, const GatherArgs &ga) {
+    const TileLayout &tl = em->tl;
+    const dim3 grid((unsigned)tl.n_tiles + ea.n_err_blocks), block(TILE_THREADS);
+    const SetArgs sets{em->plan.tL, tl.n_sets ? tl.set_ptr.p : nullptr, tl.set_members.p, tl.dest_list.p, tl.dict_b.p, tl.dest_b.p, 0u};
+#define GBRS_LAUNCH_GATHER(OW)                                                                                             \
+    hipLaunchKernelGGL((tile_estep_kernel<HT, false, false, false, OW, true>), grid, block, 0, em->stream, em->plan.tH,    \
+                       tl.tiles.p, tl.words.p, tl.dict.p, (const double *)nullptr, theta, (double *)nullptr, tl.slot_dest.p, \
+                       (double *)nullptr, em->scalars.p, (uint32_t)tl.n_tiles, ea, sets, em->plan.lead_mask, ga)
+    if constexpr (HT == 8) {
+        if (one_word) { GBRS_LAUNCH_GATHER(true); return; }
+    }
+    GBRS_LAUNCH_GATHER(false);
+#undef GBRS_LAUNCH_GATHER
+}
+
+int em_gather_steps(gbrs_em *em, int k, double target_err, int stride, int timed) {
+    GBRS_TRY(em_flush_err(em));
+    GBRS_TRY(em_gather_setup(em));
+    gbrs_em::Gather &gm = em->gm;
+    const TileLayout &tl = em->tl;
+    const EmStepRoute route = em_route(em, EmPass::Step);
+    const bool one_word = route.estep == EmEstep::TilesOneWord;
+    double *accs[3] = {em->acc.p, gm.acc_b[0].p, gm.acc_b[1].p};
+    double *thetas[2] = {em->theta.p, gm.theta_b.p};
+    double *tps[2] = {em->tot_prev.p, gm.tot_prev_b.p}, *tns[2] = {em->tot_new.p, gm.tot_new_b.p}, *mss[2] = {em->msums.p, gm.msums_b.p};
+    gm.wrote.assign((size_t)k + 1, nullptr);
+    gm.wrote[0] = em->theta.p;
+    ErrArgs waiting = em_err_args(em, target_err);
+    waiting.nblocks = (int)(tl.n_tiles * TILE_WAVES);
+    const uint32_t n_err = waiting.n_err_blocks;
+    bool have_waiting = false;
+    int src = 0;
+    if (!em->time_steps) timed = 0;
+    for (int j = 1; j <= k; ++j) {
+        const bool pending = j > 1;
+        const int set = j & 1, dst = src ^ 1;
+        GatherArgs ga;
+        ga.acc_old = accs[(gm.rot + 2) % 3];
+        ga.eff_len = em->has_len ? em->eff_len.p : nullptr;
+        ga.theta_new = thetas[dst];
+        ga.tot_prev = tps[set]; ga.tot_new = tns[set]; ga.msums = mss[set]; ga.cap = em->msum_cap;
+        ga.acc_cur = accs[gm.rot]; ga.acc_next = accs[(gm.rot + 1) % 3];
+        ga.gdest = tl.gdest.p; ga.gdest_b = tl.gdest_b.p; ga.gdest_list = tl.gdest_list.p;
+        ga.pending = pending ? 1u : 0u;
+        ErrArgs ea = waiting;
+        ea.n_err_blocks = have_waiting ? n_err : 0u;
+        const int slot = (j - 1) / stride;
+        hipEvent_t *ev = ((j - 1) % stride == 0 && slot < timed) ? &em->ev_pool[3 * slot] : nullptr;
+        if (ev) GBRS_HIP_CHECK(hipEventRecord(ev[0], em->stream));
+        switch (em->H) {
+        case 1: em_launch_gather_tiles<1>(em, one_word, thetas[src], ea, ga); break;
+        case 2: em_launch_gather_tiles<2>(em, one_word, thetas[src], ea, ga); break;
+        case 4: em_launch_gather_tiles<4>(em, one_word, thetas[src], ea, ga); break;
+        case 8: em_launch_gather_tiles<8>(em, one_word, thetas[src], ea, ga); break;
+        default: return fail(GBRS_ERR_UNSUPPORTED, "the gather-side M-step has no instance for this haplotype count");
+        }
+        if (ev) {
+            GBRS_HIP_CHECK(hipEventRecord(ev[1], em->stream));
+            GBRS_HIP_CHECK(hipEventRecord(ev[2], em->stream));
+        }
+        if (pending) {
+            gm.wrote[j - 1] = thetas[dst];
+            waiting.tot_prev = tps[set]; waiting.tot_new = tns[set]; waiting.partials = mss[set];
+            have_waiting = true;
+            src = dst;
+        }
+        gm.rot = (gm.rot + 1) % 3;
+    }
+    GBRS_HIP_CHECK(hipGetLastError());
+    if (have_waiting) {
+        waiting.n_err_blocks = n_err;
+        hipLaunchKernelGGL(err_finish_kernel, dim3(n_err), dim3(RED_THREADS), 0, em->stream, waiting);
+    }
+    {
+        double *theta = thetas[src];
+        const double *acc = accs[(gm.rot + 2) % 3], *len = em->has_len ? em->eff_len.p : nullptr;
+        switch (em->H) {
+        case 1: em_launch_mstep_elem<0, 1>(em, theta, acc, nullptr, len); break;
+        case 2: em_launch_mstep_elem<0, 2>(em, theta, acc, nullptr, len); break;
+        case 4: em_launch_mstep_elem<0, 4>(em, theta, acc, nullptr, len); break;
+        default: em_launch_mstep_elem<0, 8>(em, theta, acc, nullptr, len); break;
+        }
+    }
+    gm.wrote[k] = thetas[src];
+    if (src == 1) em->theta.swap(gm.theta_b);
+    em->counts_stale = false;
+    GBRS_TRY(em_launch_err(em, target_err));
+    GBRS_HIP_CHECK(hipGetLastError());
+    return GBRS_OK;
+}
+
+void em_gather_settle(gbrs_em *em, int it0, int done) {
+    gbrs_em::Gather &gm = em->gm;
+    const int k = (int)gm.wrote.size() - 1, m = done - it0;
+    if (k < 1 || m < 0 || m >= k) return;
+    if (gm.wrote[m] != em->theta.p) em->theta.swap(gm.theta_b);
+    em->counts_stale = true;
+    gm.clean = false;
+}
+
 int em_finish_prepare(gbrs_em *em, double pseudocount) {
     GBRS_TRY(em_launch_mstep(em, em_route(em, EmPass::Prepare)));
     em->counts_stale = false;
@@ -854,6 +1009,7 @@
     GBRS_HIP_CHECK(hipMemsetAsync(em->acc.p, 0, em->acc.bytes(), em->stream));
     GBRS_HIP_CHECK(hipGetLastError());
     em->prepared = true;
+    em->gm.primed = em->gm.clean = false;
     return GBRS_OK;
 }
 
@@ -1353,6 +1509,23 @@
         em->ev_pool.push_back(e);
     }
     const EmStepRoute route = em_route(em, EmPass::Step);
+    if (em_gather_route(em) && n_iters > 0) {
+        int left = n_iters;
+        if (!em->gm.primed) {
+            GBRS_TRY(em_one_step(em, route, 4, -1.0, left == 1 ? em->ev_pool.data() : nullptr, false));
+            --left;
+        }
+        const int gtimed = left == 0 ? 1 : std::min(timed, (left + stride - 1) / stride);
+        if (left > 0) GBRS_TRY(em_gather_steps(em, left, -1.0, stride, gtimed));
+        EmScalars host;
+        std::memset(&host, 0, sizeof(host));
+        const int float_rc = em_check_float(em, host);
+        if (host.stop || float_rc != GBRS_OK) em->gm.clean = em->gm.primed = false;
+        GBRS_TRY(float_rc);
+        em_read_times(em, gtimed);
+        if (err_sum_out) *err_sum_out = host.err_sum;
+        return GBRS_OK;
+    }
     for (int i = 0; i < n_iters; ++i) {
         const int slot = i / stride;
         const bool t = i % stride == 0 && slot < timed;
@@ -1480,11 +1653,26 @@
         const auto t_start = std::chrono::steady_clock::now();
         while (done < max_iters) {
             const int nb = std::min(batch, max_iters - done);
-            for (int i = 0; i < nb; ++i) {
+            const bool gather = model == 4 && em_gather_route(em);
+            int left = nb;
+            if (gather && !em->gm.primed) {
+                GBRS_TRY(em_one_step(em, route, model, target, first ? em->ev_pool.data() : nullptr, false));
+                first = false;
+                --left;
+            }
+            const int gk = gather ? left : 0, g_it0 = done + (nb - left);
+            if (gk > 0) {
+                GBRS_TRY(em_gather_steps(em, gk, target, gk, first ? 1 : 0));
+                first = false;
+                left = 0;
+            }
+            for (int i = 0; i < left; ++i) {
                 GBRS_TRY(em_one_step(em, route, model, target, first ? em->ev_pool.data() : nullptr, i + 1 < nb));
                 first = false;
             }
-            GBRS_TRY(em_check_float(em, host));
+            const int float_rc = em_check_float(em, host);
+            if (gk > 0 && host.stop) em_gather_settle(em, g_it0, host.iters_done);
+            GBRS_TRY(float_rc);
             if (elapsed_s) {
                 const double t = std::chrono::duration<double>(std::chrono::steady_clock::now() - t_start).count();
                 for (int i = done; i < host.iters_done && i < err_hist_cap; ++i) elapsed_s[i] = t;
@@ -1581,6 +1769,7 @@
                        em->scratch_hl.p, em->theta.p);
     GBRS_HIP_CHECK(hipStreamSynchronize(em->stream));
     em->prepared = true;
+    em->gm.primed = false;
     return GBRS_OK;
 }
 
@@ -1719,6 +1908,15 @@
                             8 * rows * em->plan.tH * 2 + (tl.weighted ? 8 * tl.n_batches * 64 : 0) +
                             (tl.n_sets ? 8 * tl.n_slots : 0);
         if (tl.n_sets) info->bytes_per_iter += 8 * tl.n_slots;
+        if (em_gather_route(em)) {
+            const uint64_t tH = em->plan.tH;
+            const uint64_t with_slot = tl.n_dest_rows ? std::min<uint64_t>(rows, em->L) : std::min<uint64_t>(tl.n_slots, em->L);
+            info->estep_bytes = 4 * tl.n_batches * 64 + 16 * tl.n_tiles + 4 * tl.n_slots * 3 + 4 * rows * 2 +
+                                8 * rows * tH * ((em->has_len ? 3 : 2) + 1) + 8 * with_slot * tH + 16 * with_slot +
+                                8 * (tl.n_light) * tH + 16 * tl.n_tiles * TILE_WAVES +
+                                (tl.n_sets ? 8 * tl.n_slots : 0);
+            info->bytes_per_iter = info->estep_bytes;
+        }
     }
     info->last_estep_ms = em->last_estep_ms;
     info->last_step_ms = em->last_step_ms;
@@ -1741,6 +1939,12 @@
     if (!em || !passes || !tile_words) return fail(GBRS_ERR_INVALID, "NULL argument");
     *passes = em->layout == 1 ? em->tl.cut_passes : 0;
     *tile_words = em->layout == 1 ? em->tl.cut_tile_words : 0;
+    return GBRS_OK;
+}
+
+int gbrs_em_gather_mstep(gbrs_em_t *em, uint32_t *taken) {
+    if (!em || !taken) return fail(GBRS_ERR_INVALID, "NULL argument");
+    *taken = em_gather_route(em) ? 1u : 0u;
     return GBRS_OK;
 }
 
diff --git a/gbrs_amd/csrc/em_layout.h b/gbrs_amd/csrc/em_layout.h
--- a/gbrs_amd/csrc/em_layout.h
+++ b/gbrs_amd/csrc/em_layout.h
@@ -62,6 +62,19 @@
     const uint32_t *set_ptr, *set_members, *dest_list;
     const uint32_t *dict_b, *dest_b;
     uint32_t relax_zero_weight;
+};
+
+constexpr uint32_t GSLOT_OWNER = 0x80000000u, GSLOT_DIRECT = 0x40000000u, GSLOT_LOCUS = 0x3FFFFFFFu;
+struct GatherArgs {
+    const double *acc_old;
+    const double *eff_len;
+    double *theta_new;
+    double *tot_prev, *tot_new;
+    double *msums;
+    uint32_t cap;
+    double *acc_cur, *acc_next;
+    const uint32_t *gdest, *gdest_b, *gdest_list;
+    uint32_t pending;
 };
 
 struct TileLayout {
@@ -104,6 +117,8 @@
     DevBuf<uint32_t> set_ptr, set_members;
     DevBuf<uint32_t> dest_list;
     DevBuf<uint32_t> dict_b, dest_b;
+    bool gather_slots = false;
+    DevBuf<uint32_t> gdest, gdest_b, gdest_list;
     bool retain_temporaries = false;
     std::vector<void *> retired;
     size_t retired_bytes = 0;
@@ -121,6 +136,7 @@
 
 int build_tile_layout(TileLayout &out, uint64_t R, uint64_t N, const uint32_t *ent_row, const uint64_t *col_ptr,
                       const double *count, hipStream_t stream, const EmPlan &plan);
+int build_gather_slots(TileLayout &tl, uint32_t L, hipStream_t stream);
 
 struct GroupedOrder {
     DevBuf<uint32_t> lh;
diff --git a/gbrs_amd/csrc/em_layout.hip b/gbrs_amd/csrc/em_layout.hip
--- a/gbrs_amd/csrc/em_layout.hip
+++ b/gbrs_amd/csrc/em_layout.hip
@@ -1748,6 +1748,64 @@
 
 }
 
+int build_gather_slots(TileLayout &tl, uint32_t L, hipStream_t s) {
+    if (tl.gather_slots) return GBRS_OK;
+    const size_t NS = tl.n_slots;
+    const bool sets = tl.n_sets != 0;
+    std::vector<uint32_t> dict(NS), dict_b, sdest, set_ptr, members;
+    std::vector<uint32_t> gdest(std::max<size_t>(NS, 1), 0u), gdest_b, glist(std::max<size_t>(tl.dest_list.n, 1), 0u);
+    GBRS_HIP_CHECK(hipStreamSynchronize(s));
+    if (NS) GBRS_HIP_CHECK(hipMemcpy(dict.data(), tl.dict.p, NS * 4, hipMemcpyDeviceToHost));
+    if (sets && NS) {
+        dict_b.resize(NS); sdest.resize(NS); gdest_b.assign(NS, 0u);
+        set_ptr.resize((size_t)tl.n_sets + 1); members.resize(tl.set_members.n);
+        GBRS_HIP_CHECK(hipMemcpy(dict_b.data(), tl.dict_b.p, NS * 4, hipMemcpyDeviceToHost));
+        GBRS_HIP_CHECK(hipMemcpy(sdest.data(), tl.slot_dest.p, NS * 4, hipMemcpyDeviceToHost));
+        GBRS_HIP_CHECK(hipMemcpy(set_ptr.data(), tl.set_ptr.p, set_ptr.size() * 4, hipMemcpyDeviceToHost));
+        if (!members.empty()) GBRS_HIP_CHECK(hipMemcpy(members.data(), tl.set_members.p, members.size() * 4, hipMemcpyDeviceToHost));
+    }
+    auto walk = [&](auto &&fn) -> int {
+        for (size_t p = 0; p < NS; ++p) {
+            const uint32_t e = dict[p];
+            if (!sets || !(e & (DICT_PAIR | DICT_SET))) {
+                if (e >= L) return fail(GBRS_ERR_STATE, "a dictionary entry is no locus");
+                fn(e, gdest[p]);
+            } else if (e & DICT_PAIR) {
+                const uint32_t a = e & ~DICT_PAIR, b2 = dict_b[p];
+                if (a >= L || b2 >= L) return fail(GBRS_ERR_STATE, "a two-member set's entry is no locus");
+                fn(a, gdest[p]);
+                fn(b2, gdest_b[p]);
+            } else {
+                const uint32_t k = e & ~DICT_SET;
+                if (k >= tl.n_sets || !(sdest[p] & SLOT_SET)) return fail(GBRS_ERR_STATE, "a set entry without a destination list");
+                const size_t off = sdest[p] & ~SLOT_SET, m0 = set_ptr[k], n = set_ptr[k + 1] - m0;
+                if (off + n >= glist.size() || m0 + n > members.size()) return fail(GBRS_ERR_STATE, "a set's destination list is out of range");
+                glist[off] = (uint32_t)n;
+                for (size_t q = 0; q < n; ++q) {
+                    if (members[m0 + q] >= L) return fail(GBRS_ERR_STATE, "a set member is no locus");
+                    fn(members[m0 + q], glist[off + 1 + q]);
+                }
+            }
+        }
+        return GBRS_OK;
+    };
+    std::vector<uint32_t> uses(L, 0u);
+    GBRS_TRY(walk([&](uint32_t l, uint32_t &) { ++uses[l]; }));
+    std::vector<uint8_t> owned(L, 0);
+    GBRS_TRY(walk([&](uint32_t l, uint32_t &w) {
+        w = l | (owned[l] ? 0u : GSLOT_OWNER) | (uses[l] == 1 ? GSLOT_DIRECT : 0u);
+        owned[l] = 1;
+    }));
+    GBRS_TRY(tl.gdest.alloc(gdest.size()));
+    GBRS_TRY(tl.gdest_b.alloc(std::max<size_t>(gdest_b.size(), 1)));
+    GBRS_TRY(tl.gdest_list.alloc(glist.size()));
+    GBRS_HIP_CHECK(hipMemcpy(tl.gdest.p, gdest.data(), gdest.size() * 4, hipMemcpyHostToDevice));
+    if (!gdest_b.empty()) GBRS_HIP_CHECK(hipMemcpy(tl.gdest_b.p, gdest_b.data(), gdest_b.size() * 4, hipMemcpyHostToDevice));
+    GBRS_HIP_CHECK(hipMemcpy(tl.gdest_list.p, glist.data(), glist.size() * 4, hipMemcpyHostToDevice));
+    tl.gather_slots = true;
+    return GBRS_OK;
+}
+
 int build_tile_layout(TileLayout &out, uint64_t R, uint64_t N, const uint32_t *ent_row, const uint64_t *col_ptr,
                       const double *count, hipStream_t s, const EmPlan &plan) {
     const uint32_t L_in = plan.tL, H = plan.tH;
diff --git a/gbrs_amd/csrc/em_plan.h b/gbrs_amd/csrc/em_plan.h
--- a/gbrs_amd/csrc/em_plan.h
+++ b/gbrs_amd/csrc/em_plan.h
@@ -32,6 +32,7 @@
     uint32_t resample_cut = 256;
     bool no_fused_mstep = false;
     bool no_float_check = false;
+    bool no_gather_mstep = false;
 };
 
 namespace em_env {
@@ -65,6 +66,7 @@
     at_least("GBRS_TUNING_RESAMPLE_CUT", 1, t.resample_cut);
     t.no_fused_mstep = integer("GBRS_TUNING_NO_FUSED_MSTEP").nonzero();
     t.no_float_check = integer("GBRS_TUNING_NO_FLOAT_CHECK").set;
+    t.no_gather_mstep = integer("GBRS_TUNING_NO_GATHER_MSTEP").nonzero();
     return t;
 }
 
@@ -124,6 +126,7 @@
     uint32_t lead_mask = ~0u;
     uint32_t resample_cut = 256;
     bool no_fused_mstep = false, no_float_check = false;
+    bool no_gather_mstep = false;
 };
 
 inline uint64_t em_tile_target(uint64_t places, unsigned side_by_side, uint32_t err_blocks, int forced) {
@@ -141,6 +144,7 @@
     p.side_by_side = (f & GBRS_EM_SIDE_BY_SIDE) ? 2u : 1u;
     p.no_fused_mstep = t.no_fused_mstep;
     p.no_float_check = t.no_float_check;
+    p.no_gather_mstep = t.no_gather_mstep;
     if ((f & GBRS_EM_RESAMPLE) && s.counts_given) p.resample_cut = t.resample_cut;
     p.tiled = !(f & GBRS_EM_LAYOUT_CSC) && s.H <= 16 && s.N < 0xFFFFFFFFull;
     p.tH = s.H;
diff --git a/gbrs_amd/csrc/em_step.h b/gbrs_amd/csrc/em_step.h
--- a/gbrs_amd/csrc/em_step.h
+++ b/gbrs_amd/csrc/em_step.h
@@ -81,4 +81,23 @@
     return r;
 }
 
+struct EmGatherShape {
+    bool no_heavy = true;
+    uint32_t n_tiles = 0, tile_waves = 0, msum_cap = 0;
+    bool posterior = false, resample = false, pair_mode = false;
+};
+
+inline bool em_gather_mstep(const EmStepShape &s, const EmGatherShape &g, EmPass pass, const EmTuning &t) {
+    if (pass != EmPass::Step || !s.tiled || s.no_tiles) return false;
+    const EmStepRoute r = em_step_route(s, pass);
+    if (r.estep != EmEstep::Tiles && r.estep != EmEstep::TilesOneWord) return false;
+    if (s.weighted) return false;
+    if (!(s.H == 1 || s.H == 2 || s.H == 4 || s.H == 8) || s.tH != s.H || s.view != 1) return false;
+    if (!s.no_long || !g.no_heavy) return false;
+    if (s.acc_handed_out) return false;
+    if (g.posterior || g.resample || g.pair_mode) return false;
+    if ((uint64_t)g.n_tiles * g.tile_waves > g.msum_cap) return false;
+    return !t.no_gather_mstep;
 }
+
+}
diff --git a/gbrs_amd/csrc/em_tiles.inc b/gbrs_amd/csrc/em_tiles.inc
--- a/gbrs_amd/csrc/em_tiles.inc
+++ b/gbrs_amd/csrc/em_tiles.inc
@@ -404,7 +404,89 @@
 #define GBRS_DIAG_PSTAMP(t, slot) do { } while (0)
 #endif
 
-template <int HT, bool WEIGHTED, bool ONES, bool DET = false, bool ONEWORD = false>
+struct GatherMember { double t, a, ln; };
+template <int H>
+__device__ __forceinline__ GatherMember gm_load(const GatherArgs &ga, const double *__restrict__ theta, uint32_t g, uint32_t h) {
+    const size_t i = (size_t)(g & GSLOT_LOCUS) * H + h;
+    GatherMember m;
+    m.t = theta[i];
+    m.a = ga.acc_old[i];
+    m.ln = ga.eff_len ? ga.eff_len[i] : 1.0;
+    return m;
+}
+template <int H>
+__device__ __forceinline__ double gm_total(double x) {
+    if (H >= 2) x += mstep_dpp<0xB1>(x);
+    if (H >= 4) x += mstep_dpp<0x4E>(x);
+    if (H >= 8) x += mstep_dpp<0x141>(x);
+    return x;
+}
+template <int H>
+__device__ __forceinline__ double gm_apply(const GatherArgs &ga, uint32_t g, uint32_t h, const GatherMember &m, bool live,
+                                           double &sum_old, double &sum_new) {
+    const uint32_t l = g & GSLOT_LOCUS;
+    const size_t i = (size_t)l * H + h;
+    const bool owner = (g & GSLOT_OWNER) != 0 && live;
+    double tn = m.t;
+    if (ga.pending) {
+        const double c = m.t * m.a;
+        tn = c / m.ln;
+        const double tp = gm_total<H>(m.t), tq = gm_total<H>(tn);
+        if (owner) {
+            ga.theta_new[i] = tn;
+            if (h == 0) {
+                ga.tot_prev[l] = tp;
+                ga.tot_new[l] = tq;
+            }
+            sum_old += m.t;
+            sum_new += tn;
+        }
+    }
+    if (owner && !(g & GSLOT_DIRECT)) ga.acc_next[i] = 0.0;
+    return tn;
+}
+
+template <int H, bool WEIGHTED>
+__device__ __forceinline__ void tile_gather_prologue(const TileHdr &th, uint32_t DH, const uint32_t *__restrict__ dict,
+                                                     const uint32_t *__restrict__ slot_dest, const double *__restrict__ theta,
+                                                     const SetArgs &sets, const GatherArgs &ga, bool live, int wave,
+                                                     double *__restrict__ s_theta) {
+    double sum_old = 0.0, sum_new = 0.0;
+    for (uint32_t i = threadIdx.x; i < DH; i += TILE_THREADS) {
+        const uint32_t j = i / H, h = i - j * H, p = th.dict_base + j;
+        const uint32_t e = dict[p], g = ga.gdest[p];
+        double tv;
+        if (sets.set_ptr == nullptr || !(e & (DICT_PAIR | DICT_SET))) {
+            tv = gm_apply<H>(ga, g, h, gm_load<H>(ga, theta, g, h), live, sum_old, sum_new);
+        } else if (e & DICT_PAIR) {
+            const uint32_t g2 = ga.gdest_b[p];
+            const GatherMember m0 = gm_load<H>(ga, theta, g, h), m1 = gm_load<H>(ga, theta, g2, h);
+            const double t0 = gm_apply<H>(ga, g, h, m0, live, sum_old, sum_new);
+            const double t1 = gm_apply<H>(ga, g2, h, m1, live, sum_old, sum_new);
+            tv = t0 + t1;
+        } else {
+            const uint32_t *gl = ga.gdest_list + (slot_dest[p] & ~SLOT_SET);
+            const uint32_t n = gl[0];
+            tv = 0.0;
+            for (uint32_t q = 1; q <= n; ++q) {
+                const uint32_t gq = gl[q];
+                tv += gm_apply<H>(ga, gq, h, gm_load<H>(ga, theta, gq, h), live, sum_old, sum_new);
+            }
+        }
+        constexpr uint32_t DP = theta_planar(H) ? lds_theta_doubles(WEIGHTED, H) / H : 0;
+        s_theta[theta_planar(H) ? (((h >> 1) * DP + j) << 1) + (h & 1u) : i] = tv;
+    }
+    if (ga.pending) {
+        sum_old = wave_sum_all(sum_old);
+        sum_new = wave_sum_all(sum_new);
+        if ((threadIdx.x & 63) == 0 && live) {
+            ga.msums[(size_t)blockIdx.x * TILE_WAVES + wave] = sum_old;
+            ga.msums[(size_t)ga.cap + (size_t)blockIdx.x * TILE_WAVES + wave] = sum_new;
+        }
+    }
+}
+
+template <int HT, bool WEIGHTED, bool ONES, bool DET = false, bool ONEWORD = false, bool GATHER = false>
 #if defined(GBRS_ESTEP_VGPR_CAP)
 __attribute__((amdgpu_num_vgpr(GBRS_ESTEP_VGPR_CAP)))
 #endif
@@ -414,7 +496,9 @@
                   const double *__restrict__ theta, double *__restrict__ partials,
                   const uint32_t *__restrict__ slot_dest, double *__restrict__ acc_direct,
                   EmScalars *__restrict__ sc, uint32_t n_tiles, ErrArgs ea, SetArgs sets,
-                  uint32_t lead_mask ) {
+                  uint32_t lead_mask ,
+                  GatherArgs ga ) {
+    static_assert(!GATHER || (HT > 0 && HT <= 8 && !WEIGHTED && !ONES && !DET), "the gather-side M-step: unweighted, 1-8 haplotypes");
     constexpr int LDS_ACC_DOUBLES = lds_acc_doubles(WEIGHTED, HT);
     __shared__ __attribute__((aligned(16))) double s_theta[lds_theta_doubles(WEIGHTED, HT)];
     __shared__ __attribute__((aligned(16))) double2 s_ftab[32];
@@ -485,6 +569,8 @@
 #endif
     for (uint32_t i = threadIdx.x; i < K * stride; i += TILE_THREADS) s_acc[i] = 0.0;
     GBRS_DIAG_STAMP(7);
+    if constexpr (GATHER) tile_gather_prologue<HT, WEIGHTED>(th, DH, dict, slot_dest, theta, sets, ga, stop_flag == 0, wave, s_theta);
+    else
     for (uint32_t i = threadIdx.x; i < DH; i += TILE_THREADS) {
         const uint32_t j = i / H, h = i - j * H;
         constexpr uint32_t DP = theta_planar(HT) ? lds_theta_doubles(WEIGHTED, HT) / (HT > 0 ? HT : 1) : 0;
@@ -641,6 +727,26 @@
         const uint32_t j = i / H, h = i - j * H;
         const uint32_t d = slot_dest[th.dict_base + j];
         const uint32_t d2 = sets.set_ptr ? sets.dest_b[th.dict_base + j] : 0u;
+        if constexpr (GATHER) {
+            const uint32_t g = ga.gdest[th.dict_base + j];
+            const uint32_t g2 = sets.set_ptr ? ga.gdest_b[th.dict_base + j] : 0u;
+            auto add = [&](uint32_t gq) {
+                double *dst = ga.acc_cur + (size_t)(gq & GSLOT_LOCUS) * H + h;
+                if (gq & GSLOT_DIRECT) *dst = a;
+                else atomicAdd(dst, a);
+            };
+            if (sets.set_ptr == nullptr || !(d & (SLOT_SET | SLOT_PAIR))) {
+                add(g);
+            } else if (d & SLOT_PAIR) {
+                add(g);
+                add(g2);
+            } else {
+                const uint32_t *gl = ga.gdest_list + (d & ~SLOT_SET);
+                const uint32_t n = gl[0];
+                for (uint32_t q = 1; q <= n; ++q) add(gl[q]);
+            }
+            continue;
+        }
         auto put = [&](uint32_t dq) {
             if (dq & SLOT_DIRECT) acc_direct[(size_t)(dq & ~SLOT_DIRECT) * H + h] = a;
             else partials[(size_t)dq * H + h] = a;
diff --git a/gbrs_amd/engine.py b/gbrs_amd/engine.py
--- a/gbrs_amd/engine.py
+++ b/gbrs_amd/engine.py
@@ -132,6 +132,11 @@
         _lib.check(_lib.load().gbrs_em_tile_cut(self._h, C.byref(passes), C.byref(words)))
         return int(passes.value), int(words.value)
 
+    def gather_mstep(self):
+        taken = C.c_uint32(0)
+        _lib.check(_lib.load().gbrs_em_gather_mstep(self._h, C.byref(taken)))
+        return bool(taken.value)
+
     def tile_shapes(self):
         n = int(self.info().num_tiles)
         batches, entries = np.zeros(n, np.uint32), np.zeros(n, np.uint32)
diff --git a/include/gbrs_hip.h b/include/gbrs_hip.h
--- a/include/gbrs_hip.h
+++ b/include/gbrs_hip.h
@@ -131,6 +131,7 @@
 int gbrs_em_info(gbrs_em_t *em, gbrs_em_info_t *info);
 int gbrs_em_fold_counts(gbrs_em_t *em, uint64_t *one_word_reads, uint64_t *two_word_reads);
 int gbrs_em_tile_cut(gbrs_em_t *em, uint32_t *passes, uint32_t *tile_words);
+int gbrs_em_gather_mstep(gbrs_em_t *em, uint32_t *taken);
 int gbrs_em_tile_shapes(gbrs_em_t *em, uint32_t *n_batches, uint32_t *dict_entries, uint64_t n);
 
 int gbrs_alignment_counts(uint64_t num_rows, uint32_t num_loci, uint32_t num_haps,
```

Measured after the change: 26620, median of 6. 9.5% higher.
